# kwai/blaze

Measured on NVIDIA H100. Metric: rows/sec on TPC-DS q1 hash-agg+filter at 1/2/4/8 H100; HBM GB/s vs 3.35 TB/s, higher is better.
Workload: dtype int64

## Files before the change

blaze_b200/csrc/agg_device.cuh:

```cuda
#pragma once
#include <cuda_runtime.h>
#include <stdint.h>

#include "kernels.cuh"

namespace b200q {

constexpr unsigned TAG_EMPTY = 0, TAG_LOCKED = 1;
constexpr unsigned FLAG_SLOT_LOCK = 1u << 15;

__device__ __forceinline__ unsigned long long ld_relaxed_u64(const unsigned long long* p) {
  unsigned long long v; asm volatile("ld.relaxed.gpu.global.u64 %0, [%1];" : "=l"(v) : "l"(p) : "memory"); return v;
}
__device__ __forceinline__ ulonglong2 ld_relaxed_v2u64(const unsigned long long* p) {
  ulonglong2 v; asm volatile("ld.relaxed.gpu.global.v2.u64 {%0,%1}, [%2];" : "=l"(v.x), "=l"(v.y) : "l"(p) : "memory"); return v;
}
__device__ __forceinline__ void st_release_u32(unsigned* p, unsigned v) { asm volatile("st.release.gpu.global.u32 [%0], %1;" ::"l"(p), "r"(v) : "memory"); }
__device__ __forceinline__ void st_relaxed_u64(unsigned long long* p, unsigned long long v) { asm volatile("st.relaxed.gpu.global.u64 [%0], %1;" ::"l"(p), "l"(v) : "memory"); }
__device__ __forceinline__ void red_add_u64(unsigned long long* p, unsigned long long v) { asm volatile("red.global.add.u64 [%0], %1;" ::"l"(p), "l"(v) : "memory"); }
__device__ __forceinline__ void red_add_f64(unsigned long long* p, double v) { asm volatile("red.global.add.f64 [%0], %1;" ::"l"(p), "d"(v) : "memory"); }
__device__ __forceinline__ void red_min_s64(unsigned long long* p, long long v) { asm volatile("red.global.min.s64 [%0], %1;" ::"l"(p), "l"(v) : "memory"); }
__device__ __forceinline__ void red_max_s64(unsigned long long* p, long long v) { asm volatile("red.global.max.s64 [%0], %1;" ::"l"(p), "l"(v) : "memory"); }
constexpr uint64_t AGG_HASH_SEED = 0x9E3779B97F4A7C15ULL;
__device__ __forceinline__ uint64_t mix64(uint64_t x) { x ^= x >> 33; x *= 0xff51afd7ed558ccdULL; x ^= x >> 33; x *= 0xc4ceb9fe1a85ec53ULL; x ^= x >> 33; return x; }
__device__ __forceinline__ unsigned lanemask_lt() { unsigned m; asm("mov.u32 %0, %%lanemask_lt;" : "=r"(m)); return m; }

__device__ __forceinline__ uint64_t agg_hash2(uint64_t k0, uint64_t k1, uint32_t knull) {
  return mix64((AGG_HASH_SEED ^ k0) + k1 * 0xD6E8FEB86659FD93ULL + (uint64_t)knull * 0xA0761D6478BD642FULL);
}
__device__ __forceinline__ uint64_t agg_hash_words(const uint64_t* kw, int nkw, uint32_t knull) {
  if (nkw <= 2) return agg_hash2(nkw > 0 ? kw[0] : 0, nkw > 1 ? kw[1] : 0, knull);
  uint64_t x = AGG_HASH_SEED ^ kw[0];
  for (int i = 1; i < nkw; i++) x = x * 0xD6E8FEB86659FD93ULL + kw[i];
  return mix64(x + (uint64_t)knull * 0xA0761D6478BD642FULL);
}

__device__ __forceinline__ void slot_mark(unsigned long long* key_entry, unsigned flags_seen, int vbit) {
  if (vbit != 0xFF && !((flags_seen >> vbit) & 1)) atomicOr((unsigned*)key_entry + 1, 1u << vbit);
}

__device__ __forceinline__ uint64_t agg_first_slot(uint64_t h, uint64_t capacity) { return __umulhi((unsigned)(h >> 32), (unsigned)capacity); }
__device__ __forceinline__ unsigned agg_tag(uint64_t h) { return (unsigned)h | 0x80000000u; }
__device__ __forceinline__ uint64_t agg_next_slot(uint64_t s, uint64_t capacity) { return s + 1 == capacity ? 0 : s + 1; }
constexpr uint64_t AGG_NO_SLOT = ~0ULL;

__device__ __forceinline__ uint64_t agg_find_or_insert(const AggLayout& lay, const AggTable& tab, const uint64_t* kw, uint32_t knull,
                                                       uint64_t h, unsigned* flags_out, bool* inserted) {
  const unsigned tag = agg_tag(h);
  uint64_t s = agg_first_slot(h, tab.capacity);
  while (true) {
    unsigned long long* ke = tab.keys + s * (uint64_t)lay.kstride;
    const unsigned long long hdr = ld_relaxed_u64(ke);
    const unsigned t = (unsigned)hdr;
    unsigned flags = (unsigned)(hdr >> 32);
    if (t == tag) {
      asm volatile("fence.acq_rel.gpu;" ::: "memory");
      bool eq = (flags >> 16) == knull;
      for (int i = 0; eq && i < lay.nkw; i++) eq = ld_relaxed_u64(ke + 1 + i) == kw[i];
      if (eq) { *flags_out = flags; return s; }
    } else if (t == TAG_EMPTY) {
      if (ld_relaxed_u64(tab.counters) >= tab.max_groups) return AGG_NO_SLOT;
      if (atomicCAS((unsigned*)ke, TAG_EMPTY, TAG_LOCKED) == TAG_EMPTY) {
        for (int i = 0; i < lay.nkw; i++) ke[1 + i] = kw[i];
        unsigned long long* ae = tab.accs + s * (uint64_t)lay.astride;
        for (int i = 0; i < lay.astride; i++) ae[i] = lay.init[i];
        flags = lay.init_flags | (knull << 16);
        ((unsigned*)ke)[1] = flags;
        st_release_u32((unsigned*)ke, tag);
        *inserted = true;
        *flags_out = flags;
        return s;
      }
      continue;
    } else if (t == TAG_LOCKED) {
      continue;
    }
    s = agg_next_slot(s, tab.capacity);
  }
}

}
```

blaze_b200/csrc/capi.cu:

```cuda
#include <algorithm>
#include <cstdio>
#include <cstdlib>
#include <cstring>
#include <functional>
#include <mutex>

#include "lz4_frame.h"
#include "parquet_meta.h"
#include "runtime.h"

namespace b200q {

static thread_local std::string g_last_error;

static std::string format_of(const DType& t) {
  switch (t.id) {
    case T_BOOL: return "b"; case T_INT8: return "c"; case T_INT16: return "s"; case T_INT32: return "i"; case T_INT64: return "l";
    case T_FLOAT32: return "f"; case T_FLOAT64: return "g"; case T_DATE32: return "tdD"; case T_TIMESTAMP_US: return "tsu:";
    case T_DECIMAL128: return "d:" + std::to_string(t.precision) + "," + std::to_string(t.scale);
    case T_BINARY: return "z"; case T_UTF8: return "u"; default: return "n";
  }
}
DType type_of_format(const char* f) {
  DType d; std::string s(f ? f : "");
// ... 455 lines not shown
      hc.values = d2h((const uint8_t*)dc.values->ptr + first, (size_t)(ho[n] - first));
      if (first) for (int64_t i = 0; i <= n; i++) ho[i] -= first;
    } else if (dc.type.id == T_BOOL) hc.values = d2h(dc.values->ptr, (size_t)(n + 7) / 8);
    else if (dc.type.id != T_NULL) hc.values = d2h(dc.values->ptr, (size_t)n * dc.type.byte_width());
    hb.cols.push_back(hc);
  }
  B200Q_CUDA(cudaStreamSynchronize(cx.stream));
  return hb;
}

struct ArrayPriv {
  std::shared_ptr<HostBlock> block;
  std::vector<DevMemP> dev;
  std::vector<const void*> buffers;
  std::vector<ArrowArray> children; std::vector<ArrowArray*> child_ptrs;
};
static void release_array(ArrowArray* a) {
  if (!a || !a->release) return;
  auto* p = (ArrayPriv*)a->private_data;
  for (auto& c : p->children) if (c.release) c.release(&c);
  delete p; a->release = nullptr;
}
static int64_t count_nulls(const uint8_t* bits, int64_t off, int64_t n) {
  int64_t set = 0;
  for (int64_t i = 0; i < n; i++) set += (bits[(off + i) >> 3] >> ((off + i) & 7)) & 1;
  return n - set;
}
static void export_host_slice(const HostBatch& hb, int64_t off, int64_t len, ArrowArray* out) {
  auto* top = new ArrayPriv(); top->block = hb.block;
  memset(out, 0, sizeof(*out));
  out->length = len; out->null_count = 0; out->offset = 0; out->n_buffers = 1;
  top->buffers.push_back(nullptr); out->buffers = top->buffers.data();
  top->children.resize(hb.cols.size()); top->child_ptrs.resize(hb.cols.size());
  for (size_t i = 0; i < hb.cols.size(); i++) {
    const HostColumn& hc = hb.cols[i];
    auto* cp = new ArrayPriv(); cp->block = hb.block;
    ArrowArray& c = top->children[i]; memset(&c, 0, sizeof(c));
    c.length = len; c.offset = off;
    c.null_count = hc.validity ? count_nulls((const uint8_t*)hc.validity, off, len) : 0;
    if (hc.type.id == T_NULL) { c.null_count = len; c.n_buffers = 0; }
    else if (hc.type.is_varlen()) { cp->buffers = {hc.validity, hc.offsets, hc.values}; c.n_buffers = 3; }
    else { cp->buffers = {hc.validity, hc.values}; c.n_buffers = 2; }
    c.buffers = cp->buffers.data(); c.release = release_array; c.private_data = cp;
    top->child_ptrs[i] = &c;
  }
  out->n_children = (int64_t)hb.cols.size(); out->children = top->child_ptrs.data();
  out->release = release_array; out->private_data = top;
}
void export_device(DevBatch& db, int device, ArrowDeviceArray* out) {
  auto* top = new ArrayPriv();
  memset(out, 0, sizeof(*out));
  ArrowArray& a = out->array;
  a.length = db.num_rows; a.n_buffers = 1; top->buffers.push_back(nullptr); a.buffers = top->buffers.data();
  top->children.resize(db.cols.size()); top->child_ptrs.resize(db.cols.size());
  for (size_t i = 0; i < db.cols.size(); i++) {
    DevColumn& dc = db.cols[i];
    auto* cp = new ArrayPriv();
    ArrowArray& c = top->children[i]; memset(&c, 0, sizeof(c));
    c.length = db.num_rows; c.offset = dc.offset; c.null_count = dc.validity ? -1 : 0;
    const void* v = dc.validity ? dc.validity->ptr : nullptr;
    if (dc.validity) cp->dev.push_back(dc.validity);
    if (dc.values) cp->dev.push_back(dc.values);
    if (dc.offsets) cp->dev.push_back(dc.offsets);
    if (dc.type.id == T_NULL) { c.n_buffers = 0; c.null_count = db.num_rows; }
    else if (dc.type.is_varlen()) { cp->buffers = {v, dc.offsets->ptr, dc.values->ptr}; c.n_buffers = 3; }
    else { cp->buffers = {v, dc.values ? dc.values->ptr : nullptr}; c.n_buffers = 2; }
    c.buffers = cp->buffers.data(); c.release = release_array; c.private_data = cp;
    top->child_ptrs[i] = &c;
  }
  a.n_children = (int64_t)db.cols.size(); a.children = top->child_ptrs.data();
  a.release = release_array; a.private_data = top;
  out->device_id = device; out->device_type = ARROW_DEVICE_CUDA; out->sync_event = nullptr;
}

static void conf_defaults(b200q_conf* c) {
  memset(c, 0, sizeof(*c));
  c->struct_size = sizeof(b200q_conf);
  c->batch_size = 10000;
  c->suggested_batch_mem_size = 8388608;
  c->partial_agg_skipping_enable = 1;
  c->partial_agg_skipping_ratio = 0.999;
  c->partial_agg_skipping_min_rows = 20000;
  c->staging_rows = 1 << 20;
  c->agg_initial_groups = 1 << 19;
  c->max_launch_rows = 1 << 27;
  c->partial_state_columnar = 0;
  c->force_generic_kernels = 0;
  c->agg_dense_keys = 1;
  c->agg_hot_key_cache = 1;
}

}

#define B200Q_STR2(x) #x
#define B200Q_STR(x) B200Q_STR2(x)

extern "C" {

int32_t b200q_version(void) { return 100; }
const char* b200q_build_info(void) { return "blaze_b200 hot path: Filter/Project/HashAgg, sm_90a, CUDA " B200Q_STR(CUDART_VERSION); }
const char* b200q_last_error(void) { return g_last_error.c_str(); }
int32_t b200q_device_count(void) { int n = 0; if (cudaGetDeviceCount(&n) != cudaSuccess) { cudaGetLastError(); return 0; } return n; }

b200q_status b200q_conf_init(b200q_conf* conf) {
  if (!conf) return fail(B200Q_ERR_INVALID_ARG, "conf is null");
  conf_defaults(conf); return B200Q_OK;
}

b200q_status b200q_plan_explain(const uint8_t* plan, size_t plan_len, int32_t plan_kind, char* buf, size_t cap, size_t* needed) {
  return guarded(nullptr, [&] {
    PlanP p = decode_plan(plan, plan_len, plan_kind);
    std::string s = explain_plan(p);
    if (needed) *needed = s.size() + 1;
    if (buf && cap) { const size_t n = std::min(cap - 1, s.size()); memcpy(buf, s.data(), n); buf[n] = 0; }
  });
}

b200q_status b200q_op_create(const uint8_t* plan, size_t plan_len, int32_t plan_kind, const struct ArrowSchema* input_schema,
                             const b200q_conf* conf, int32_t device, b200q_op** out) {
  if (!out) return fail(B200Q_ERR_INVALID_ARG, "out is null");
  *out = nullptr;
  b200q_op* op = nullptr;
  b200q_status st = guarded(nullptr, [&] {
    PlanP p = decode_plan(plan, plan_len, plan_kind);
    int ndev = 0;
    if (cudaGetDeviceCount(&ndev) != cudaSuccess || ndev == 0) { cudaGetLastError(); throw ExecError(B200Q_ERR_NO_DEVICE, "no CUDA device is visible: the sm_90a kernels cannot run and there is no CPU fallback"); }
    if (device < 0 || device >= ndev) throw ExecError(B200Q_ERR_INVALID_ARG, "invalid device ordinal");
    op = new b200q_op();
    op->plan = p; op->cx.device = device;
    conf_defaults(&op->cx.conf);
    if (conf) { const size_t n = std::min<size_t>(conf->struct_size ? conf->struct_size : sizeof(b200q_conf), sizeof(b200q_conf)); memcpy(&op->cx.conf, conf, n); op->cx.conf.struct_size = sizeof(b200q_conf); }
    if (op->cx.conf.batch_size <= 0) op->cx.conf.batch_size = 10000;
    if (op->cx.conf.max_launch_rows <= 0) op->cx.conf.max_launch_rows = 1 << 27;
    if (op->cx.conf.agg_initial_groups <= 0) op->cx.conf.agg_initial_groups = 1 << 19;
    B200Q_CUDA(cudaSetDevice(device));
    {
      cudaMemPool_t pool; unsigned long long keep = ~0ULL;
      if (cudaDeviceGetDefaultMemPool(&pool, device) == cudaSuccess) cudaMemPoolSetAttribute(pool, cudaMemPoolAttrReleaseThreshold, &keep);
    }
    op->stream_ref = stream_ref_create(device);
    op->cx.stream = op->stream_ref->s;
    B200Q_CUDA(cudaEventCreate(&op->cx.ev0)); B200Q_CUDA(cudaEventCreate(&op->cx.ev1));
    build_pipeline(op);
    const PlanNode* leaf = op->plan.get();
    while (leaf->input) leaf = leaf->input.get();
    if (leaf->leaf_kind == "IpcReader") op->ipc = make_ipc_source(op->cx, op->in_schema, op->stages[0]->used_input_cols);
    if (input_schema) {
      if (input_schema->n_children != (int64_t)op->in_schema.fields.size()) throw PlanError(B200Q_ERR_INVALID_ARG, "input_schema does not match the plan leaf: column count");
      for (int64_t i = 0; i < input_schema->n_children; i++)
        if (type_of_format(input_schema->children[i]->format) != op->in_schema.fields[i].type)
          throw PlanError(B200Q_ERR_INVALID_ARG, "input_schema does not match the plan leaf: type of column " + std::to_string(i));
    }
  });
  if (st != B200Q_OK) { if (op) { op->stages.clear(); delete op; } return st; }
  *out = op;
  return B200Q_OK;
}

b200q_status b200q_op_input_schema(b200q_op* op, struct ArrowSchema* out) {
  if (!op || !out) return fail(B200Q_ERR_INVALID_ARG, "null argument");
  return guarded(nullptr, [&] { export_schema(op->in_schema, out); });
}
b200q_status b200q_op_output_schema(b200q_op* op, struct ArrowSchema* out) {
  if (!op || !out) return fail(B200Q_ERR_INVALID_ARG, "null argument");
  return guarded(nullptr, [&] { export_schema(op->out_schema, out); });
}

b200q_status b200q_op_push(b200q_op* op, struct ArrowArray* batch) {
  if (!op) return fail(B200Q_ERR_INVALID_ARG, "op is null");
  b200q_status st = guarded(op, [&] {
    if (op->finished) throw ExecError(B200Q_ERR_STATE, "push after finish");
    if (op->ipc) throw ExecError(B200Q_ERR_STATE, "an op whose leaf is an IpcReaderExecNode takes its input through b200q_op_push_ipc");
    B200Q_CUDA(cudaSetDevice(op->cx.device));
    validate_host_batch(op, batch);
    poll_pending(op, false);
    op->cx.m.input_rows += batch->length; op->cx.m.input_batches++;
    if (batch->length == 0) return;
    const std::vector<int>& used = op->stages[0]->used_input_cols;
    const int64_t srows = op->cx.conf.staging_rows;
    if (srows > 0 && batch->length < srows / 2) { staging_append(op, batch); return; }
    if (op->staging_ready) staging_flush(op);
    DevBatch db = import_direct(op, batch, used);
    PendingRelease pr; pr.arr = *batch; batch->release = nullptr;
    B200Q_CUDA(cudaEventCreateWithFlags(&pr.ev, cudaEventDisableTiming));
    B200Q_CUDA(cudaEventRecord(pr.ev, op->cx.stream));
    op->pending.push_back(pr);
    run_stages(op, db, 0);
  });
  if (batch && batch->release) batch->release(batch);
  return st;
}

b200q_status b200q_op_push_ipc(b200q_op* op, const uint8_t* data, size_t len) {
  if (!op) return fail(B200Q_ERR_INVALID_ARG, "op is null");
  return guarded(op, [&] {
    if (op->finished) throw ExecError(B200Q_ERR_STATE, "push after finish");
    if (!op->ipc) throw ExecError(B200Q_ERR_STATE, "push_ipc: the op's leaf is not an IpcReaderExecNode");
    if (!data && len) throw ExecError(B200Q_ERR_INVALID_ARG, "push_ipc: null data");
    B200Q_CUDA(cudaSetDevice(op->cx.device));
    poll_pending(op, false);
    op->ipc->push(op->cx, data, len, [&](DevBatch& b) { run_stages(op, b, 0); });
  });
}

b200q_status b200q_op_push_device(b200q_op* op, struct ArrowDeviceArray* dbatch) {
  if (!op) return fail(B200Q_ERR_INVALID_ARG, "op is null");
  b200q_status st = guarded(op, [&] {
    if (op->finished) throw ExecError(B200Q_ERR_STATE, "push after finish");
    if (op->ipc) throw ExecError(B200Q_ERR_STATE, "an op whose leaf is an IpcReaderExecNode takes its input through b200q_op_push_ipc");
    if (!dbatch) throw ExecError(B200Q_ERR_INVALID_ARG, "null batch");
    if (dbatch->device_type != ARROW_DEVICE_CUDA || dbatch->device_id != op->cx.device) throw ExecError(B200Q_ERR_INVALID_ARG, "push_device: batch is not on this op's CUDA device");
    B200Q_CUDA(cudaSetDevice(op->cx.device));
    ArrowArray* batch = &dbatch->array;
    validate_host_batch(op, batch);
    poll_pending(op, false);
    if (op->staging_ready) staging_flush(op);
    if (dbatch->sync_event) B200Q_CUDA(cudaStreamWaitEvent(op->cx.stream, *(cudaEvent_t*)dbatch->sync_event, 0));
    op->cx.m.input_rows += batch->length; op->cx.m.input_batches++;
    if (batch->length == 0) return;
    DevBatch db; db.num_rows = batch->length; db.cols.resize(op->in_schema.fields.size());
    for (size_t i = 0; i < db.cols.size(); i++) {
      const ArrowArray* c = batch->children[i]; DevColumn& dc = db.cols[i];
      dc.type = op->in_schema.fields[i].type; dc.offset = c->offset + batch->offset;
      const size_t huge = (size_t)1 << 60;
      if (c->n_buffers > 0 && c->buffers[0] && c->null_count != 0) dc.validity = DevMem::borrow(c->buffers[0], huge, nullptr);
      if (dc.type.is_varlen()) { dc.offsets = DevMem::borrow(c->buffers[1], huge, nullptr); dc.values = DevMem::borrow(c->buffers[2], huge, nullptr); }
      else if (c->n_buffers > 1 && c->buffers[1]) dc.values = DevMem::borrow(c->buffers[1], huge, nullptr);
    }
    PendingRelease pr; pr.arr = *batch;
    B200Q_CUDA(cudaEventCreateWithFlags(&pr.ev, cudaEventDisableTiming));
    batch->release = nullptr;
    op->pending.push_back(pr);
    const cudaEvent_t ev = pr.ev;
    try { run_stages(op, db, 0); } catch (...) { cudaEventRecord(ev, op->cx.stream); throw; }
    B200Q_CUDA(cudaEventRecord(ev, op->cx.stream));
  });
  if (dbatch && dbatch->array.release) dbatch->array.release(&dbatch->array);
  return st;
}

b200q_status b200q_op_finish(b200q_op* op) {
  if (!op) return fail(B200Q_ERR_INVALID_ARG, "op is null");
  return guarded(op, [&] {
    if (op->finished) return;
    B200Q_CUDA(cudaSetDevice(op->cx.device));
    {
      const PlanNode* leaf = op->plan.get();
      while (leaf->input) leaf = leaf->input.get();
      if (leaf->kind == N_LEAF && leaf->leaf_kind == "ParquetScan") {
        if (op->cx.m.input_batches) throw ExecError(B200Q_ERR_STATE, "an op whose leaf is a ParquetScanExecNode takes no pushed batches");
        run_parquet_scan(op->cx, *leaf, [&](DevBatch& b) { run_stages(op, b, 0); });
      }
    }
    if (op->ipc) op->ipc->flush(op->cx, [&](DevBatch& b) { run_stages(op, b, 0); });
    if (op->staging_ready) staging_flush(op);
    for (size_t i = 0; i < op->stages.size(); i++) {
      std::vector<DevBatch> outs;
      op->cx.cur_stage = (int)i;
      op->stages[i]->finish(op->cx, outs);
      for (auto& o : outs) {
        if (i + 1 < op->stages.size()) run_stages(op, o, i + 1);
        else { op->cx.m.output_rows += o.num_rows; op->out_queue.push_back(std::move(o)); }
      }
    }
    B200Q_CUDA(cudaStreamSynchronize(op->cx.stream));
    poll_pending(op, true);
    op->finished = true;
  });
}

b200q_status b200q_op_pull(b200q_op* op, struct ArrowArray* out, int32_t* has_batch) {
  if (!op || !out || !has_batch) return fail(B200Q_ERR_INVALID_ARG, "null argument");
  *has_batch = 0;
  return guarded(op, [&] {
    B200Q_CUDA(cudaSetDevice(op->cx.device));
    if (!op->has_cur_host) {
      if (op->out_queue.empty()) return;
      op->cur_host = to_host(op, op->out_queue.front());
      op->out_queue.pop_front();
      op->has_cur_host = true;
    }
    HostBatch& hb = op->cur_host;
    const int64_t len = std::min<int64_t>(op->cx.conf.batch_size, hb.num_rows - hb.cursor);
    export_host_slice(hb, hb.cursor, len, out);
    hb.cursor += len;
    if (hb.cursor >= hb.num_rows) { op->has_cur_host = false; op->cur_host = HostBatch(); }
    op->cx.m.output_batches++;
    *has_batch = 1;
  });
}

b200q_status b200q_op_pull_device(b200q_op* op, struct ArrowDeviceArray* out, int32_t* has_batch) {
  if (!op || !out || !has_batch) return fail(B200Q_ERR_INVALID_ARG, "null argument");
  *has_batch = 0;
  return guarded(op, [&] {
    if (op->has_cur_host) throw ExecError(B200Q_ERR_STATE, "pull_device while a host batch is partially pulled");
    if (op->out_queue.empty()) return;
    B200Q_CUDA(cudaSetDevice(op->cx.device));
    B200Q_CUDA(cudaStreamSynchronize(op->cx.stream));
    export_device(op->out_queue.front(), op->cx.device, out);
    op->out_queue.pop_front();
    op->cx.m.output_batches++;
    *has_batch = 1;
  });
}

b200q_status b200q_op_sync(b200q_op* op) {
// ... 143 lines not shown
```

blaze_b200/csrc/kernels_fast.cu:

```cuda
#include <algorithm>
#include <cstdlib>
#include <cuda_runtime.h>
#include <stdint.h>

#include "agg_device.cuh"
#include "kernels_fast.cuh"

namespace b200q {

constexpr int FA_BLOCK = 256;

__device__ __forceinline__ uint64_t make_evict_first_policy() {
  uint64_t pol; asm volatile("createpolicy.fractional.L2::evict_first.b64 %0, 1.0;" : "=l"(pol)); return pol;
}
__device__ __forceinline__ long long ld_stream_s64(const long long* p) {
  long long v; const uint64_t pol = make_evict_first_policy();
  asm volatile("ld.global.nc.L1::no_allocate.L2::cache_hint.s64 %0, [%1], %2;" : "=l"(v) : "l"(p), "l"(pol)); return v;
}
__device__ __forceinline__ bool col_valid(const DevCol& c, long long i) {
  if (!c.validity) return true;
  const unsigned long long bi = (unsigned long long)i + c.bit_offset;
  return (__ldg(c.validity + (bi >> 3)) >> (bi & 7)) & 1;
}
__device__ __forceinline__ long long col_load_int(const DevCol& c, int phys, long long i) {
// ... 191 lines not shown
#pragma unroll
    for (int u = 0; u < U; u++) {
      unsigned long long di;
      const bool in = dense_index<NK>(fs, k0[u], k1[u], di) && alive[u] && !(meta[u] & 3u);
      const unsigned pk = in ? ((unsigned)di | ((meta[u] & 0xCu) << 26)) : 0xFFFFFFFFu;
#pragma unroll
      for (int t = 0; t < G; t++) {
        const unsigned opk = __shfl_sync(0xffffffffu, pk, t, G);
        const unsigned long long ov0 = add0 ? __shfl_sync(0xffffffffu, v0[u], t, G) : 0ULL;
        const unsigned long long ov1 = add1 ? __shfl_sync(0xffffffffu, v1[u], t, G) : 0ULL;
        const bool live = opk != 0xFFFFFFFFu;
        unsigned long long val;
        switch (wkind) {
          case DW_ONE: val = 1; break;
          case DW_ADD0: val = ov0; break;
          case DW_ADD1: val = ov1; break;
          case DW_VALID0: val = (opk >> 28) & 1u; break;
          case DW_VALID1: val = (opk >> 29) & 1u; break;
          default: val = 0; break;
        }
        red_add_u64(live ? fs.dense_tab + (uint64_t)(opk & IDX_MASK) * G + q : sink, live ? val : 0ULL);
      }
      const bool fb = alive[u] && !in;
      if (__any_sync(0xffffffffu, fb)) {
        bool inserted = false;
        if (fb) {
          uint64_t kw[2] = {(uint64_t)k0[u], NK == 2 ? (uint64_t)k1[u] : 0ULL};
          const unsigned knull = meta[u] & 3u;
          unsigned fl = 0;
          const uint64_t si = agg_find_or_insert(lay, tab, kw, knull, agg_hash2(kw[0], kw[1], knull), &fl, &inserted);
          if (si == AGG_NO_SLOT) { const unsigned long long at = atomicAdd(tab.counters + 1, 1ULL); tab.deferred[at] = (uint32_t)((unit0 + u) * 32 + lane); }
          else {
            unsigned long long* const p = tab.accs + si * (uint64_t)lay.astride;
            unsigned long long* const ke = tab.keys + si * (uint64_t)lay.kstride;
            if (meta[u] & 4u) { red_add_u64(p + fs.acc[0].word, add0 ? v0[u] : 1ULL); slot_mark(ke, fl, fs.acc[0].vbit); }
            if (NACC == 2 && (meta[u] & 8u)) { red_add_u64(p + fs.acc[1].word, add1 ? v1[u] : 1ULL); slot_mark(ke, fl, fs.acc[1].vbit); }
          }
        }
        const unsigned bl = __ballot_sync(0xffffffffu, inserted);
        if (lane == 0 && bl) atomicAdd(tab.counters, (unsigned long long)__popc(bl));
      }
    }
  }
}

constexpr int HC_LINES = 1024;
template <int NACC, int NK, int G>
__global__ void __launch_bounds__(FA_BLOCK) agg_dense_hot_kernel(const ColTable cols, const FastSpec fs, const AggLayout lay, const AggTable tab,
                                                                 long long row_begin, long long n) {
  constexpr int U = 4;
  constexpr unsigned IDX_MASK = 0x0FFFFFFFu;
  __shared__ unsigned long long c_key[HC_LINES];
  __shared__ unsigned c_acc[HC_LINES * G * 2];
  for (int i = threadIdx.x; i < HC_LINES; i += FA_BLOCK) c_key[i] = 0;
  for (int i = threadIdx.x; i < HC_LINES * G * 2; i += FA_BLOCK) c_acc[i] = 0;
  __syncthreads();
  const unsigned lane = threadIdx.x & 31, q = lane & (G - 1);
  const long long gwarp = (long long)blockIdx.x * (FA_BLOCK / 32) + (threadIdx.x >> 5), nwarps = (long long)gridDim.x * (FA_BLOCK / 32);
  const long long nunits = (n + 31) / 32;
  const bool add0 = fs.acc[0].kind == FAST_ACC_ADD, add1 = NACC == 2 && fs.acc[1].kind == FAST_ACC_ADD;
  auto word_kind = [&](int m) {
    const int src = fs.dense_word_src[m];
    return src == -1 ? DW_ONE : src == -2 ? DW_ZERO : src >= 2 ? DW_ONE : src == 0 ? (add0 ? DW_ADD0 : DW_ONE) : (add1 ? DW_ADD1 : DW_ONE);
  };
  int wk[G];
#pragma unroll
  for (int m = 0; m < G; m++) wk[m] = word_kind(m);
  const int wkind = word_kind((int)q);
  unsigned long long* const sink = warp_sink(fs, gwarp, lane);

  for (long long unit0 = gwarp * U; unit0 < nunits; unit0 += nwarps * U) {
    long long k0[U], k1[U]; unsigned long long v0[U], v1[U]; bool alive[U];
#pragma unroll
    for (int u = 0; u < U; u++) {
      const long long rel = (unit0 + u) * 32 + lane, row = row_begin + rel;
      alive[u] = rel < n; k0[u] = 0; k1[u] = 0; v0[u] = 0; v1[u] = 0;
      if (!alive[u]) continue;
      k0[u] = ld_stream_vec((const long long*)cols.col[fs.key_col[0]].values + row, (i64xG<1>*)nullptr).v[0];
      if (NK == 2) k1[u] = ld_stream_vec((const long long*)cols.col[fs.key_col[1]].values + row, (i64xG<1>*)nullptr).v[0];
      if (add0) v0[u] = (unsigned long long)ld_stream_vec((const long long*)cols.col[fs.acc[0].col].values + row, (i64xG<1>*)nullptr).v[0];
      if (add1) v1[u] = (unsigned long long)ld_stream_vec((const long long*)cols.col[fs.acc[1].col].values + row, (i64xG<1>*)nullptr).v[0];
    }
    for (int f = 0; f < fs.nfilt; f++) {
      const long long* fcol = (const long long*)cols.col[fs.filt[f].col].values + row_begin;
#pragma unroll
      for (int u = 0; u < U; u++) {
        const long long rel = (unit0 + u) * 32 + lane;
        if (alive[u]) alive[u] = cmp_apply(fs.filt[f].op, ld_stream_vec(fcol + rel, (i64xG<1>*)nullptr).v[0], fs.filt[f].lit);
      }
    }
#pragma unroll
    for (int u = 0; u < U; u++) {
      unsigned long long di;
      const bool in = dense_index<NK>(fs, k0[u], k1[u], di) && alive[u];
      bool cached = false;
      if (in) {
        const unsigned line = (unsigned)((di * 0x9E3779B97F4A7C15ULL) >> 54);
        const unsigned long long mine = di + 1;
        unsigned long long cur = *(volatile unsigned long long*)&c_key[line];
        if (cur == 0) { cur = atomicCAS(&c_key[line], 0ULL, mine); if (cur == 0) cur = mine; }
        if (cur == mine) {
          cached = true;
          unsigned* const e = c_acc + line * (G * 2);
#pragma unroll
          for (int m = 0; m < G; m++) {
            if (wk[m] == DW_ONE) smem_add64(e + 2 * m, 1ULL);
            else if (wk[m] == DW_ADD0) smem_add64(e + 2 * m, v0[u]);
            else if (wk[m] == DW_ADD1) smem_add64(e + 2 * m, v1[u]);
          }
        }
      }
      const unsigned pk = (in && !cached) ? (unsigned)di : 0xFFFFFFFFu;
#pragma unroll
      for (int t = 0; t < G; t++) {
        const unsigned opk = __shfl_sync(0xffffffffu, pk, t, G);
        const unsigned long long ov0 = add0 ? __shfl_sync(0xffffffffu, v0[u], t, G) : 0ULL;
        const unsigned long long ov1 = add1 ? __shfl_sync(0xffffffffu, v1[u], t, G) : 0ULL;
        const bool live = opk != 0xFFFFFFFFu;
        const unsigned long long val = wkind == DW_ONE ? 1ULL : wkind == DW_ADD0 ? ov0 : wkind == DW_ADD1 ? ov1 : 0ULL;
        red_add_u64(live ? fs.dense_tab + (uint64_t)(opk & IDX_MASK) * G + q : sink, live ? val : 0ULL);
      }
      const bool fb = alive[u] && !in;
      if (__any_sync(0xffffffffu, fb)) {
        bool inserted = false;
        if (fb) {
          uint64_t kw[2] = {(uint64_t)k0[u], NK == 2 ? (uint64_t)k1[u] : 0ULL};
          unsigned fl = 0;
          const uint64_t si = agg_find_or_insert(lay, tab, kw, 0, agg_hash2(kw[0], kw[1], 0), &fl, &inserted);
          if (si == AGG_NO_SLOT) { const unsigned long long at = atomicAdd(tab.counters + 1, 1ULL); tab.deferred[at] = (uint32_t)((unit0 + u) * 32 + lane); }
          else {
            unsigned long long* const p = tab.accs + si * (uint64_t)lay.astride;
            unsigned long long* const ke = tab.keys + si * (uint64_t)lay.kstride;
            red_add_u64(p + fs.acc[0].word, add0 ? v0[u] : 1ULL); slot_mark(ke, fl, fs.acc[0].vbit);
            if (NACC == 2) { red_add_u64(p + fs.acc[1].word, add1 ? v1[u] : 1ULL); slot_mark(ke, fl, fs.acc[1].vbit); }
          }
        }
        const unsigned bl = __ballot_sync(0xffffffffu, inserted);
        if (lane == 0 && bl) atomicAdd(tab.counters, (unsigned long long)__popc(bl));
      }
    }
  }
  __syncthreads();
  for (int line = threadIdx.x; line < HC_LINES; line += FA_BLOCK) {
    const unsigned long long key = c_key[line];
    if (!key) continue;
#pragma unroll
    for (int m = 0; m < G; m++) {
      const unsigned long long val = (unsigned long long)c_acc[(line * G + m) * 2] | ((unsigned long long)c_acc[(line * G + m) * 2 + 1] << 32);
      if (val) red_add_u64(fs.dense_tab + (key - 1) * G + m, val);
    }
  }
}

__global__ void __launch_bounds__(256) key_skew_hist_kernel(const DevCol c0, const DevCol c1, int phys0, int phys1, int nkeys, long long n, unsigned* hist) {
  for (long long i = blockIdx.x * (long long)blockDim.x + threadIdx.x; i < n; i += (long long)gridDim.x * blockDim.x) {
    if (!col_valid(c0, i) || (nkeys == 2 && !col_valid(c1, i))) continue;
    const uint64_t h = agg_hash2((uint64_t)col_load_int(c0, phys0, i), nkeys == 2 ? (uint64_t)col_load_int(c1, phys1, i) : 0ULL, 0);
    atomicAdd(hist + (h >> 48), 1u);
  }
}
__global__ void __launch_bounds__(256) key_skew_max_kernel(unsigned* hist) {
  unsigned mx = 0;
  for (int i = blockIdx.x * blockDim.x + threadIdx.x; i < 65536; i += gridDim.x * blockDim.x) mx = max(mx, hist[i]);
#pragma unroll
  for (int d = 16; d > 0; d >>= 1) mx = max(mx, __shfl_xor_sync(0xffffffffu, mx, d));
  if ((threadIdx.x & 31) == 0) atomicMax(hist + 65536, mx);
}

constexpr int LH_BLOCK = 128, LH_U = 4, LH_QCAP = 32 * (LH_U + 1);
template <int NK, bool TYPED> struct LhQueue {
  unsigned long long k0[LH_QCAP]; unsigned long long k1[NK == 2 ? LH_QCAP : 1]; unsigned long long v0[LH_QCAP], v1[LH_QCAP];
  unsigned idx[LH_QCAP], tag[LH_QCAP], row[LH_QCAP];
  uint8_t meta[TYPED ? LH_QCAP : 1];
};
enum { LH_HIT = 0, LH_AGAIN = 1, LH_NEW = 2, LH_IDLE = 3 };
constexpr unsigned LH_META_PLAIN = 0xC;

template <int NK>
__device__ __forceinline__ int lh_eval(const AggTable& tab, int ks, unsigned cap, ulonglong2 hk, unsigned tag, unsigned knull, unsigned long long k0,
                                       unsigned long long k1, unsigned& idx, unsigned& flags) {
  const unsigned t = (unsigned)hk.x;
  if (t == tag) {
    bool hit = (unsigned)(hk.x >> 48) == knull && hk.y == k0;
    if (NK == 2 && hit) hit = ld_relaxed_u64(tab.keys + (uint64_t)idx * ks + 2) == k1;
    if (hit) { flags = (unsigned)(hk.x >> 32); return LH_HIT; }
  } else if (t == TAG_EMPTY) return LH_NEW;
  else if (t == TAG_LOCKED) return LH_AGAIN;
  idx = idx + 1 == cap ? 0 : idx + 1;
  return LH_AGAIN;
}

template <int NK, int NACC, bool TYPED>
__device__ __forceinline__ void lh_finish(const FastSpec& fs, const AggLayout& lay, const AggTable& tab, LhQueue<NK, TYPED>& q, int& count, unsigned lane,
                                          unsigned long long* sink, bool has_v1, int st, unsigned idx, unsigned flags, unsigned tag, unsigned meta,
                                          unsigned long long k0, unsigned long long k1, unsigned long long v0, unsigned long long v1, unsigned row) {
  constexpr unsigned NONE = 0xFFFFFFFFu;
  if (__any_sync(0xffffffffu, st == LH_NEW)) {
    bool inserted = false;
    if (st == LH_NEW) {
      uint64_t kw[2] = {k0, NK == 2 ? k1 : 0ULL};
      const unsigned knull = TYPED ? (meta & 3u) : 0u;
      const uint64_t si = agg_find_or_insert(lay, tab, kw, knull, agg_hash2(k0, NK == 2 ? k1 : 0ULL, knull), &flags, &inserted);
      if (si == AGG_NO_SLOT) { const unsigned long long at = atomicAdd(tab.counters + 1, 1ULL); tab.deferred[at] = row; st = LH_IDLE; }
      else { idx = (unsigned)si; st = LH_HIT; }
    }
    const unsigned b = __ballot_sync(0xffffffffu, inserted);
    if (lane == 0 && b) atomicAdd(tab.counters, (unsigned long long)__popc(b));
  }
  const bool odd = lane & 1;
  const int as = lay.astride, w0 = fs.acc[0].word, w1 = NACC == 2 ? fs.acc[1].word : 0;
  const unsigned mi = st == LH_HIT ? idx : NONE;
  unsigned long long* const mine = mi != NONE ? tab.accs + (uint64_t)mi * as + w0 : sink;
  const unsigned long long mv = mi != NONE ? v0 : 0ULL;
  if (NACC == 1) red_add_u64(mine, mv);
  else {
    const unsigned pi = __shfl_xor_sync(0xffffffffu, mi, 1);
    const unsigned long long pv1 = has_v1 ? __shfl_xor_sync(0xffffffffu, v1, 1) : 1ULL;
    unsigned long long* const theirs = pi != NONE ? tab.accs + (uint64_t)pi * as + w1 : sink;
    const unsigned long long tv = pi != NONE ? pv1 : 0ULL;
    red_add_u64(odd ? theirs : mine, odd ? tv : mv);
    red_add_u64(odd ? mine : theirs, odd ? mv : tv);
  }
  if (mi != NONE) {
    unsigned long long* ke = tab.keys + (uint64_t)mi * lay.kstride;
    if (!TYPED || (meta & 4u)) slot_mark(ke, flags, fs.acc[0].vbit);
    if (NACC == 2 && (!TYPED || (meta & 8u))) slot_mark(ke, flags, fs.acc[1].vbit);
  }
  const unsigned m = __ballot_sync(0xffffffffu, st == LH_AGAIN);
  if (m) {
    if (st == LH_AGAIN) {
      const int at = count + __popc(m & ((1u << lane) - 1));
      q.k0[at] = k0; if (NK == 2) q.k1[at] = k1; q.v0[at] = v0; q.v1[at] = v1; q.idx[at] = idx; q.tag[at] = tag; q.row[at] = row;
      if (TYPED) q.meta[at] = (uint8_t)meta;
    }
    count += __popc(m);
  }
}

template <int NK, int NACC, bool TYPED>
__device__ __forceinline__ void lh_drain(const FastSpec& fs, const AggLayout& lay, const AggTable& tab, LhQueue<NK, TYPED>& q, int& count, unsigned lane,
                                         unsigned long long* sink, bool has_v1) {
  const int nb = count < 32 ? count : 32;
  __syncwarp();
  count -= nb;
  const bool act = (int)lane < nb; const int e = count + (act ? lane : 0);
  const unsigned long long k0 = q.k0[e], k1 = NK == 2 ? q.k1[e] : 0ULL, v0 = q.v0[e], v1 = q.v1[e];
  unsigned idx = q.idx[e], flags = 0; const unsigned tag = q.tag[e], row = q.row[e], meta = TYPED ? q.meta[e] : LH_META_PLAIN;
  __syncwarp();
  int st = LH_IDLE;
  if (act) st = lh_eval<NK>(tab, lay.kstride, (unsigned)tab.capacity, ld_relaxed_v2u64(tab.keys + (uint64_t)idx * lay.kstride), tag, TYPED ? (meta & 3u) : 0u, k0, k1, idx, flags);
  lh_finish<NK, NACC, TYPED>(fs, lay, tab, q, count, lane, sink, has_v1, st, idx, flags, tag, meta, k0, k1, v0, v1, row);
}

template <int NK, int NACC, bool TYPED>
__global__ void __launch_bounds__(LH_BLOCK, TYPED ? 4 : 6) agg_lean_hash_kernel(const ColTable cols, const FastSpec fs, const AggLayout lay, const AggTable tab,
                                                                                long long row_begin, long long n) {
  constexpr int U = LH_U;
  __shared__ LhQueue<NK, TYPED> queues[LH_BLOCK / 32];
  LhQueue<NK, TYPED>& q = queues[threadIdx.x >> 5];
  int count = 0;
  const unsigned lane = threadIdx.x & 31;
  const long long gwarp = (long long)blockIdx.x * (LH_BLOCK / 32) + (threadIdx.x >> 5), nwarps = (long long)gridDim.x * (LH_BLOCK / 32);
  const long long nunits = (n + 31) / 32;
  const bool add0 = fs.acc[0].kind == FAST_ACC_ADD, add1 = NACC == 2 && fs.acc[1].kind == FAST_ACC_ADD;
  const long long* kcol0 = (const long long*)cols.col[fs.key_col[0]].values + row_begin;
  const long long* kcol1 = NK == 2 ? (const long long*)cols.col[fs.key_col[1]].values + row_begin : nullptr;
  const long long* vcol0 = add0 ? (const long long*)cols.col[fs.acc[0].col].values + row_begin : nullptr;
  const long long* vcol1 = add1 ? (const long long*)cols.col[fs.acc[1].col].values + row_begin : nullptr;
  unsigned long long* const sink = warp_sink(fs, gwarp, lane);
  const unsigned cap = (unsigned)tab.capacity; const int ks = lay.kstride;

  for (long long unit0 = gwarp * U; unit0 < nunits; unit0 += nwarps * U) {
    unsigned long long k0[U], k1[U], v0[U], v1[U]; bool alive[U]; unsigned meta[U];
#pragma unroll
    for (int u = 0; u < U; u++) {
      const long long rel = (unit0 + u) * 32 + lane;
      alive[u] = rel < n; meta[u] = LH_META_PLAIN;
      if (!TYPED) {
        k0[u] = alive[u] ? (unsigned long long)ld_stream_vec(kcol0 + rel, (i64xG<1>*)nullptr).v[0] : 0;
        k1[u] = (NK == 2 && alive[u]) ? (unsigned long long)ld_stream_vec(kcol1 + rel, (i64xG<1>*)nullptr).v[0] : 0;
        v0[u] = (vcol0 && alive[u]) ? (unsigned long long)ld_stream_vec(vcol0 + rel, (i64xG<1>*)nullptr).v[0] : 1ULL;
        v1[u] = (vcol1 && alive[u]) ? (unsigned long long)ld_stream_vec(vcol1 + rel, (i64xG<1>*)nullptr).v[0] : 1ULL;
      } else {
        k0[u] = 0; k1[u] = 0; v0[u] = 1; v1[u] = 1;
        if (alive[u]) {
          const long long row = row_begin + rel;
          { const DevCol& c = cols.col[fs.key_col[0]]; if (col_valid(c, row)) k0[u] = (unsigned long long)col_load_int(c, fs.key_phys[0], row); else meta[u] |= 1u; }
          if (NK == 2) { const DevCol& c = cols.col[fs.key_col[1]]; if (col_valid(c, row)) k1[u] = (unsigned long long)col_load_int(c, fs.key_phys[1], row); else meta[u] |= 2u; }
          if (fs.acc[0].col >= 0) {
            const DevCol& c = cols.col[fs.acc[0].col];
            if (!col_valid(c, row)) { meta[u] &= ~4u; v0[u] = 0; } else if (add0) v0[u] = (unsigned long long)col_load_int(c, fs.acc[0].phys, row);
          }
          if (NACC == 2 && fs.acc[1].col >= 0) {
            const DevCol& c = cols.col[fs.acc[1].col];
            if (!col_valid(c, row)) { meta[u] &= ~8u; v1[u] = 0; } else if (add1) v1[u] = (unsigned long long)col_load_int(c, fs.acc[1].phys, row);
          }
        }
      }
    }
    for (int f = 0; f < fs.nfilt; f++) {
      if (!TYPED) {
        const long long* fcol = (const long long*)cols.col[fs.filt[f].col].values + row_begin;
#pragma unroll
        for (int u = 0; u < U; u++) {
          const long long rel = (unit0 + u) * 32 + lane;
          const long long x = rel < n ? ld_stream_vec(fcol + rel, (i64xG<1>*)nullptr).v[0] : 0;
          alive[u] = alive[u] && cmp_apply(fs.filt[f].op, x, fs.filt[f].lit);
        }
      } else {
        const DevCol& c = cols.col[fs.filt[f].col];
#pragma unroll
        for (int u = 0; u < U; u++) {
          const long long row = row_begin + (unit0 + u) * 32 + lane;
          if (alive[u]) alive[u] = col_valid(c, row) && cmp_apply(fs.filt[f].op, col_load_int(c, fs.filt[f].phys, row), fs.filt[f].lit);
        }
      }
    }
    unsigned idx[U], tag[U]; ulonglong2 hk[U];
#pragma unroll
// ... 25 lines not shown
  for (unsigned i = threadIdx.x; i < 2 * nwords; i += FA_BLOCK) s_tab[i] = 0;
  __syncthreads();
  const unsigned lane = threadIdx.x & 31;
  const long long gwarp = (long long)blockIdx.x * (FA_BLOCK / 32) + (threadIdx.x >> 5), nwarps = (long long)gridDim.x * (FA_BLOCK / 32);
  const long long nunits = (n + 31) / 32;
  const bool add0 = fs.acc[0].kind == FAST_ACC_ADD, add1 = NACC == 2 && fs.acc[1].kind == FAST_ACC_ADD;

  for (long long unit0 = gwarp * U; unit0 < nunits; unit0 += nwarps * U) {
    long long k[U], k1[U]; unsigned long long v0[U], v1[U]; bool alive[U]; unsigned meta[U];
#pragma unroll
    for (int u = 0; u < U; u++) {
      const long long rel = (unit0 + u) * 32 + lane, row = row_begin + rel;
      alive[u] = rel < n; meta[u] = 0xC; k[u] = 0; k1[u] = 0; v0[u] = 1; v1[u] = 1;
      if (!alive[u]) continue;
      if (!TYPED) {
        k[u] = ld_stream_vec((const long long*)cols.col[fs.key_col[0]].values + row, (i64xG<1>*)nullptr).v[0];
        if (NK == 2) k1[u] = ld_stream_vec((const long long*)cols.col[fs.key_col[1]].values + row, (i64xG<1>*)nullptr).v[0];
        if (add0) v0[u] = (unsigned long long)ld_stream_vec((const long long*)cols.col[fs.acc[0].col].values + row, (i64xG<1>*)nullptr).v[0];
        if (add1) v1[u] = (unsigned long long)ld_stream_vec((const long long*)cols.col[fs.acc[1].col].values + row, (i64xG<1>*)nullptr).v[0];
      } else {
        { const DevCol& c = cols.col[fs.key_col[0]]; if (col_valid(c, row)) k[u] = col_load_int(c, fs.key_phys[0], row); else meta[u] |= 1u; }
        if (NK == 2) { const DevCol& c = cols.col[fs.key_col[1]]; if (col_valid(c, row)) k1[u] = col_load_int(c, fs.key_phys[1], row); else meta[u] |= 2u; }
        if (fs.acc[0].col >= 0) {
          const DevCol& c = cols.col[fs.acc[0].col];
          if (!col_valid(c, row)) { meta[u] &= ~4u; v0[u] = 0; } else if (add0) v0[u] = (unsigned long long)col_load_int(c, fs.acc[0].phys, row);
        }
        if (NACC == 2 && fs.acc[1].col >= 0) {
          const DevCol& c = cols.col[fs.acc[1].col];
          if (!col_valid(c, row)) { meta[u] &= ~8u; v1[u] = 0; } else if (add1) v1[u] = (unsigned long long)col_load_int(c, fs.acc[1].phys, row);
        }
      }
    }
    for (int f = 0; f < fs.nfilt; f++) {
      const DevCol& c = cols.col[fs.filt[f].col];
#pragma unroll
      for (int u = 0; u < U; u++) {
        const long long row = row_begin + (unit0 + u) * 32 + lane;
        if (!alive[u]) continue;
        if (!TYPED) alive[u] = cmp_apply(fs.filt[f].op, ld_stream_vec((const long long*)c.values + row, (i64xG<1>*)nullptr).v[0], fs.filt[f].lit);
        else alive[u] = col_valid(c, row) && cmp_apply(fs.filt[f].op, col_load_int(c, fs.filt[f].phys, row), fs.filt[f].lit);
      }
    }
#pragma unroll
    for (int u = 0; u < U; u++) {
      unsigned long long idx;
      const bool in = dense_index<NK>(fs, k[u], k1[u], idx) && alive[u] && !(meta[u] & 3u);
      if (in) {
        unsigned* const e = s_tab + 2 * (unsigned)idx * G;
#pragma unroll
        for (int m = 0; m < 4; m++) {
          if (m >= G) break;
          const int src = fs.dense_word_src[m];
          if (src == -1) smem_add64(e + 2 * m, 1ULL);
          else if (src == 0) { if (meta[u] & 4u) smem_add64(e + 2 * m, v0[u]); }
          else if (src == 1 && NACC == 2) { if (meta[u] & 8u) smem_add64(e + 2 * m, v1[u]); }
          else if (src >= 2) { if (meta[u] & (4u << (src - 2))) smem_add64(e + 2 * m, 1ULL); }
        }
      }
      const bool fb = alive[u] && !in;
      if (__any_sync(0xffffffffu, fb)) {
        bool inserted = false;
        if (fb) {
          uint64_t kw[2] = {(uint64_t)k[u], NK == 2 ? (uint64_t)k1[u] : 0ULL};
          const unsigned knull = meta[u] & 3u;
          unsigned fl = 0;
          const uint64_t si = agg_find_or_insert(lay, tab, kw, knull, agg_hash2(kw[0], kw[1], knull), &fl, &inserted);
          if (si == AGG_NO_SLOT) { const unsigned long long at = atomicAdd(tab.counters + 1, 1ULL); tab.deferred[at] = (uint32_t)((unit0 + u) * 32 + lane); }
          else {
            unsigned long long* const p = tab.accs + si * (uint64_t)lay.astride;
            unsigned long long* const ke = tab.keys + si * (uint64_t)lay.kstride;
            if (meta[u] & 4u) { red_add_u64(p + fs.acc[0].word, v0[u]); slot_mark(ke, fl, fs.acc[0].vbit); }
            if (NACC == 2 && (meta[u] & 8u)) { red_add_u64(p + fs.acc[1].word, v1[u]); slot_mark(ke, fl, fs.acc[1].vbit); }
          }
        }
        const unsigned b = __ballot_sync(0xffffffffu, inserted);
        if (lane == 0 && b) atomicAdd(tab.counters, (unsigned long long)__popc(b));
      }
    }
  }
  __syncthreads();
  for (unsigned w = threadIdx.x; w < nwords; w += FA_BLOCK) {
    const unsigned long long val = (unsigned long long)s_tab[2 * w] | ((unsigned long long)s_tab[2 * w + 1] << 32);
    if (val) red_add_u64(fs.dense_tab + w, val);
  }
}

static int fast_grid(int64_t ntiles) {
  int dev = 0, sms = 132; cudaGetDevice(&dev); cudaDeviceGetAttribute(&sms, cudaDevAttrMultiProcessorCount, dev);
  const int64_t cap = (int64_t)sms * 8;
  return (int)(ntiles < cap ? (ntiles < 1 ? 1 : ntiles) : cap);
}

int launch_agg_fast_update(const ColTable& cols, const FastSpec& fs, const AggLayout& lay, const AggTable& tab, int64_t row_begin, int64_t n, cudaStream_t s) {
  if (n <= 0) return 0;
  const int dg = fs.dense ? fs.dense_stride : 0;
  if (dg && fs.dense_cap * (unsigned long long)dg <= (unsigned long long)DS_MAX_WORDS) {
    const int g = (int)std::max<int64_t>(1, std::min<int64_t>((n + FA_BLOCK * 4 - 1) / (FA_BLOCK * 4), (int64_t)fast_grid(1 << 30) / 8 * 3));
#define B200Q_DS(NACC, TYPED, NK) agg_dense_smem_kernel<NACC, TYPED, NK><<<g, FA_BLOCK, 0, s>>>(cols, fs, lay, tab, row_begin, n)
    if (fs.nkeys == 1) {
      if (fs.lean) { if (fs.nacc == 2) B200Q_DS(2, false, 1); else B200Q_DS(1, false, 1); } else { if (fs.nacc == 2) B200Q_DS(2, true, 1); else B200Q_DS(1, true, 1); }
    } else {
      if (fs.lean) { if (fs.nacc == 2) B200Q_DS(2, false, 2); else B200Q_DS(1, false, 2); } else { if (fs.nacc == 2) B200Q_DS(2, true, 2); else B200Q_DS(1, true, 2); }
    }
#undef B200Q_DS
    return 1;
  }
  if (dg && fs.lean && fs.hot_cache) {
    const int g = fast_grid((n + 32 * 8 * 4 - 1) / (32 * 8 * 4));
#define B200Q_HC(NACC, NK, G) agg_dense_hot_kernel<NACC, NK, G><<<g, FA_BLOCK, 0, s>>>(cols, fs, lay, tab, row_begin, n)
    if (fs.nkeys == 1) {
      if (fs.nacc == 2) { if (dg == 2) B200Q_HC(2, 1, 2); else B200Q_HC(2, 1, 4); } else { if (dg == 2) B200Q_HC(1, 1, 2); else B200Q_HC(1, 1, 4); }
    } else {
      if (fs.nacc == 2) { if (dg == 2) B200Q_HC(2, 2, 2); else B200Q_HC(2, 2, 4); } else { if (dg == 2) B200Q_HC(1, 2, 2); else B200Q_HC(1, 2, 4); }
    }
#undef B200Q_HC
    return 1;
  }
  if (dg && fs.lean && fs.nkeys == 1 && fs.nfilt == 0) {
    const int u = dg == 2 ? 4 : 2;
    const int g = fast_grid((n + 32 * 8 * u - 1) / (32 * 8 * u));
#define B200Q_LD(NACC, G) agg_lean_dense_kernel<NACC, G, 1><<<g, FA_BLOCK, 0, s>>>(cols, fs, lay, tab, row_begin, n)
    if (fs.nacc == 2) { if (dg == 2) B200Q_LD(2, 2); else B200Q_LD(2, 4); } else { if (dg == 2) B200Q_LD(1, 2); else B200Q_LD(1, 4); }
#undef B200Q_LD
    return 1;
  }
  if (dg && fs.nfcol >= 0) {
    if (fs.filt_never) return 0;
    return launch_agg_tile_dense(cols, fs, lay, tab, row_begin, n, s);
  }
  if (dg) {
    const int g = fast_grid((n + 32 * 8 * 4 - 1) / (32 * 8 * 4));
#define B200Q_DR(NACC, NK, G) do { if (fs.lean) agg_dense_row_kernel<NACC, NK, G, false><<<g, FA_BLOCK, 0, s>>>(cols, fs, lay, tab, row_begin, n); \
                                   else agg_dense_row_kernel<NACC, NK, G, true><<<g, FA_BLOCK, 0, s>>>(cols, fs, lay, tab, row_begin, n); } while (0)
    if (fs.nkeys == 1) {
      if (fs.nacc == 2) { if (dg == 2) B200Q_DR(2, 1, 2); else B200Q_DR(2, 1, 4); } else { if (dg == 2) B200Q_DR(1, 1, 2); else B200Q_DR(1, 1, 4); }
    } else {
      if (fs.nacc == 2) { if (dg == 2) B200Q_DR(2, 2, 2); else B200Q_DR(2, 2, 4); } else { if (dg == 2) B200Q_DR(1, 2, 2); else B200Q_DR(1, 2, 4); }
    }
#undef B200Q_DR
    return 1;
  }
  if (!dg) {
    const int64_t tiles = (n + 32 * (LH_BLOCK / 32) * LH_U - 1) / (32 * (LH_BLOCK / 32) * LH_U);
    const int g = (int)std::max<int64_t>(1, std::min<int64_t>(tiles, (int64_t)fast_grid(1 << 30) / 8 * (fs.lean ? 6 : 4)));
#define B200Q_LH(NK, NACC, TYPED) agg_lean_hash_kernel<NK, NACC, TYPED><<<g, LH_BLOCK, 0, s>>>(cols, fs, lay, tab, row_begin, n)
    if (fs.lean) { if (fs.nkeys == 1) { if (fs.nacc == 2) B200Q_LH(1, 2, false); else B200Q_LH(1, 1, false); } else { if (fs.nacc == 2) B200Q_LH(2, 2, false); else B200Q_LH(2, 1, false); } }
    else { if (fs.nkeys == 1) { if (fs.nacc == 2) B200Q_LH(1, 2, true); else B200Q_LH(1, 1, true); } else { if (fs.nacc == 2) B200Q_LH(2, 2, true); else B200Q_LH(2, 1, true); } }
#undef B200Q_LH
    return 1;
  }
  return 0;
}

__global__ void __launch_bounds__(256) key_range_kernel(const DevCol col, int phys, long long n, long long* out ) {
  long long mn = INT64_MAX, mx = INT64_MIN; unsigned long long cnt = 0;
  for (long long i = blockIdx.x * (long long)blockDim.x + threadIdx.x; i < n; i += (long long)gridDim.x * blockDim.x) {
    if (!col_valid(col, i)) continue;
    const long long v = col_load_int(col, phys, i);
    mn = v < mn ? v : mn; mx = v > mx ? v : mx; cnt++;
  }
#pragma unroll
  for (int d = 16; d > 0; d >>= 1) {
    const long long a = __shfl_xor_sync(0xffffffffu, mn, d), b = __shfl_xor_sync(0xffffffffu, mx, d);
    mn = a < mn ? a : mn; mx = b > mx ? b : mx; cnt += __shfl_xor_sync(0xffffffffu, cnt, d);
  }
  if ((threadIdx.x & 31) == 0) { atomicMin(out, mn); atomicMax(out + 1, mx); atomicAdd((unsigned long long*)out + 2, cnt); }
}
int launch_key_skew_probe(const DevCol* key_cols, const uint8_t* phys, int nkeys, int64_t n, unsigned* d_hist, cudaStream_t s) {
  key_skew_hist_kernel<<<fast_grid((n + 2047) / 2048), 256, 0, s>>>(key_cols[0], key_cols[nkeys == 2 ? 1 : 0], phys[0], phys[nkeys == 2 ? 1 : 0], nkeys, n, d_hist);
  key_skew_max_kernel<<<32, 256, 0, s>>>(d_hist);
  return 2;
}
int launch_key_range(const DevCol& col, int phys, int64_t n, long long* d_out, cudaStream_t s) {
  key_range_kernel<<<fast_grid((n + 2047) / 2048), 256, 0, s>>>(col, phys, n, d_out);
  return 1;
}

__device__ __forceinline__ void dense_store(const EmitCol& c, unsigned long long at, uint64_t lo, bool valid) {
  if (c.valid_bytes) c.valid_bytes[at] = valid ? 1 : 0;
  switch (c.phys) {
    case PH_BOOL: ((uint8_t*)c.values)[at] = lo != 0; break;
    case PH_I8: ((int8_t*)c.values)[at] = (int8_t)lo; break;
    case PH_I16: ((int16_t*)c.values)[at] = (int16_t)lo; break;
    case PH_I32: ((int32_t*)c.values)[at] = (int32_t)lo; break;
    default: ((uint64_t*)c.values)[at] = lo; break;
  }
}
__global__ void __launch_bounds__(256) agg_emit_dense_kernel(const FastSpec fs, const EmitTable emit, const DenseEmitMap map, unsigned long long* out_count) {
  const unsigned lane = threadIdx.x & 31;
  const uint64_t stride = (uint64_t)gridDim.x * blockDim.x;
  const uint64_t rounds = (fs.dense_cap + stride - 1) / stride;
  for (uint64_t it = 0; it < rounds; it++) {
    const uint64_t i = it * stride + blockIdx.x * (uint64_t)blockDim.x + threadIdx.x;
    const uint64_t pe = fs.nkeys == 2 && fs.dense_key0_minor ? dense_entry2(fs, i / fs.dense_r1, i % fs.dense_r1) : i;
    const unsigned long long* e = fs.dense_tab + pe * fs.dense_stride;
    const bool occ = i < fs.dense_cap && e[fs.dense_presence_word] != 0;
    const unsigned m = __ballot_sync(0xffffffffu, occ);
    if (!m) continue;
    unsigned long long base = 0;
    if (lane == 0) base = atomicAdd(out_count, (unsigned long long)__popc(m));
    base = __shfl_sync(0xffffffffu, base, 0);
    if (!occ) continue;
    const unsigned long long at = base + __popc(m & lanemask_lt());
    for (int c = 0; c < emit.ncols; c++) {
      const EmitCol ec = emit.col[c];
      if (ec.kind == EMIT_KEY) {
        const long long kv = fs.nkeys == 1 ? fs.dense_base + (long long)i
                           : ec.key == 0 ? fs.dense_base + (long long)(i / fs.dense_r1) : fs.dense_base1 + (long long)(i % fs.dense_r1);
        dense_store(ec, at, (uint64_t)kv, true);
      }
      else {
        const int w = map.word[c], vw = map.valid_word[c];
        const bool valid = vw == 0xFF ? true : e[vw] != 0;
        dense_store(ec, at, valid ? e[w] : 0, valid);
      }
    }
  }
}
int launch_agg_emit_dense(const FastSpec& fs, const EmitTable& emit, const DenseEmitMap& map, unsigned long long* d_out_count, cudaStream_t s) {
  agg_emit_dense_kernel<<<fast_grid(((int64_t)fs.dense_cap + 255) / 256), 256, 0, s>>>(fs, emit, map, d_out_count);
  return 1;
}

__global__ void __launch_bounds__(256) dense_count_kernel(const FastSpec fs, unsigned long long* out) {
  unsigned long long c = 0;
  for (uint64_t i = blockIdx.x * (uint64_t)blockDim.x + threadIdx.x; i < fs.dense_cap; i += (uint64_t)gridDim.x * blockDim.x)
    c += fs.dense_tab[i * fs.dense_stride + fs.dense_presence_word] != 0;
#pragma unroll
  for (int d = 16; d > 0; d >>= 1) c += __shfl_xor_sync(0xffffffffu, c, d);
  if ((threadIdx.x & 31) == 0 && c) atomicAdd(out, c);
}
int launch_dense_count(const FastSpec& fs, unsigned long long* d_out, cudaStream_t s) {
  dense_count_kernel<<<fast_grid(((int64_t)fs.dense_cap + 255) / 256), 256, 0, s>>>(fs, d_out);
  return 1;
}

}
```

blaze_b200/csrc/kernels_fast.cuh:

```cuda
#pragma once
#include <cstddef>

#include "kernels.cuh"

namespace b200q {

enum FastAccKind : uint8_t { FAST_ACC_ADD = 0, FAST_ACC_COUNT = 1 };

struct FilterInterval { int8_t col; uint8_t phys; uint8_t _pad[6]; long long lo; unsigned long long span; };

struct FastSpec {
  int32_t nkeys, nacc, nfilt, dense;
  int32_t lean, hot_cache;
  int8_t key_col[2]; uint8_t key_phys[2];
  struct { uint8_t kind; int8_t col; uint8_t phys; uint8_t vbit; uint8_t word; uint8_t _pad[3]; } acc[2];
  struct { int8_t col; uint8_t phys; uint8_t op; uint8_t _pad[5]; long long lit; } filt[4];
  int32_t nfcol;
  int32_t filt_never;
  FilterInterval frange[2];
  long long dense_base;
  unsigned long long dense_cap;
  long long dense_base1;
  unsigned long long dense_r1, dense_cap0;
  unsigned long long* dense_tab;
  int8_t dense_stride;
  int8_t dense_word_src[4];
  uint8_t dense_presence_word;
  uint8_t dense_key0_minor;
  uint8_t _pad1;
  unsigned long long* sink;
};
constexpr int FAST_SINK_WARPS = 4096;

struct DenseEmitMap { uint8_t word[EMIT_MAX_COLS]; uint8_t valid_word[EMIT_MAX_COLS]; };

__device__ __forceinline__ unsigned long long dense_entry2(const FastSpec& fs, unsigned long long d0, unsigned long long d1) {
  return fs.dense_key0_minor ? d1 * fs.dense_cap0 + d0 : d0 * fs.dense_r1 + d1;
}
template <int NK>
__device__ __forceinline__ bool dense_index_of(const FastSpec& fs, long long k0, long long k1, unsigned long long& idx) {
  const unsigned long long d0 = (unsigned long long)(k0 - fs.dense_base);
  if (NK == 1) { idx = d0; return d0 < fs.dense_cap; }
  const unsigned long long d1 = (unsigned long long)(k1 - fs.dense_base1);
  idx = dense_entry2(fs, d0, d1);
  return d0 < fs.dense_cap0 && d1 < fs.dense_r1;
}

enum TileFlavour : uint8_t { TF_ADD_U64 = 0, TF_ADD_F64 = 1, TF_MIN_S64 = 2 };
__host__ __device__ constexpr unsigned long long tile_identity(int flavour) {
  return flavour == TF_MIN_S64 ? 0x7FFFFFFFFFFFFFFFULL : flavour == TF_ADD_F64 ? 0x8000000000000000ULL : 0ULL;
}
enum TileArgCvt : uint8_t { TC_NONE = 0, TC_I2F = 1 , TC_ORDER = 2  };
enum TileRecon : uint8_t { TR_COPY = 0 , TR_NOT = 1 ,
                           TR_F2I = 2 , TR_DEC3 = 3  };
struct TileWord {
  uint8_t srcsel;
  uint8_t sh;
  uint8_t gate;
  uint8_t _pad[5];
  unsigned long long msk, inv, cst;
};
struct TileAggSpec {
  int32_t nkeys, nargs, nfcol, filt_never, nacc, G, flavour, arg_is_dec;
  int8_t key_col[2]; uint8_t key_phys[2];
  int8_t arg_col[2]; uint8_t arg_phys[2]; uint8_t arg_cvt[2]; uint8_t arg_values[2];
  FilterInterval frange[2];
  long long dense_base, dense_base1;
  unsigned long long dense_cap, dense_r1, dense_cap0;
  unsigned long long* dense_tab;
  unsigned long long* sink;
  unsigned long long dec_mul;
  TileWord word[8];
  uint8_t presence_word, dec_word , _pad2[6];
  struct { int8_t arg; uint8_t recon; uint8_t w0; uint8_t valid_word; uint8_t lay_acc; uint8_t _pad[3]; } acc[4];
};
static_assert(sizeof(FastSpec) == 232 && offsetof(FastSpec, frange) == 120, "FastSpec layout");
static_assert(sizeof(TileAggSpec) == 456 && offsetof(TileAggSpec, frange) == 48, "TileAggSpec layout");

int launch_agg_tile_wide(const ColTable& cols, const TileAggSpec& ts, const AggLayout& lay, const AggTable& tab, int64_t row_begin, int64_t n, cudaStream_t s);
int launch_tile_wide_init(const TileAggSpec& ts, cudaStream_t s);
int launch_tile_wide_count(const TileAggSpec& ts, unsigned long long* d_out, cudaStream_t s);
int launch_tile_wide_normalise(const TileAggSpec& ts, cudaStream_t s);
int launch_tile_wide_emit(const TileAggSpec& ts, const AggLayout& lay, const EmitTable& emit, unsigned long long* d_out_count, cudaStream_t s);

int launch_agg_tile_dense(const ColTable& cols, const FastSpec& fs, const AggLayout& lay, const AggTable& tab, int64_t row_begin, int64_t n, cudaStream_t s);
int launch_agg_fast_update(const ColTable& cols, const FastSpec& fs, const AggLayout& lay, const AggTable& tab, int64_t row_begin, int64_t n, cudaStream_t s);
int launch_key_skew_probe(const DevCol* key_cols, const uint8_t* phys, int nkeys, int64_t n, unsigned* d_hist , cudaStream_t s);
int launch_key_range(const DevCol& col, int phys, int64_t n, long long* d_out, cudaStream_t s);
int launch_agg_emit_dense(const FastSpec& fs, const EmitTable& emit, const DenseEmitMap& map, unsigned long long* d_out_count, cudaStream_t s);
int launch_dense_count(const FastSpec& fs, unsigned long long* d_out, cudaStream_t s);

}
```

blaze_b200/csrc/kernels_tile.cu:

```cuda
#include <cuda_runtime.h>
#include <stdint.h>

#include <algorithm>

#include "agg_device.cuh"
#include "emit_device.cuh"
#include "kernels_fast.cuh"

namespace b200q {

constexpr int TL_BLOCK = 256, TL_WARPS = TL_BLOCK / 32, TL_ROWS = 128;

__device__ __forceinline__ uint64_t tl_policy_evict_first() {
  uint64_t pol; asm volatile("createpolicy.fractional.L2::evict_first.b64 %0, 1.0;" : "=l"(pol)); return pol;
}
__device__ __forceinline__ void tl_ld_b64(const long long* p, unsigned on, uint64_t pol, long long& v) {
  asm volatile("{\n\t.reg .pred q;\n\tsetp.ne.u32 q, %2, 0;\n\t@q ld.global.nc.L1::no_allocate.L2::cache_hint.b64 %0, [%1], %3;\n\t}"
               : "+l"(v) : "l"(p), "r"(on), "l"(pol));
}
__device__ __forceinline__ void tl_ld_v2b64(const long long* p, unsigned on, uint64_t pol, long long& a, long long& b) {
  asm volatile("{\n\t.reg .pred q;\n\tsetp.ne.u32 q, %3, 0;\n\t@q ld.global.nc.L1::no_allocate.L2::cache_hint.v2.b64 {%0,%1}, [%2], %4;\n\t}"
               : "+l"(a), "+l"(b) : "l"(p), "r"(on), "l"(pol));
}
__device__ __forceinline__ void tl_ld_b32(const int* p, unsigned on, uint64_t pol, int& v) {
// ... 227 lines not shown
  const bool a16 = ((uintptr_t)c.values & 15) == 0;
#pragma unroll
  for (int j = 0; j < 4; j++) {
    lo[j] = 0; hi[j] = 0;
    if (a16) tl_ld_v2b64(p + 64 * j, (ld >> j) & 1u, pol, lo[j], hi[j]);
    else { tl_ld_b64(p + 64 * j, (ld >> j) & 1u, pol, lo[j]); tl_ld_b64(p + 64 * j + 1, (ld >> j) & 1u, pol, hi[j]); }
  }
}

__device__ __forceinline__ unsigned long long tw_convert(long long v, int cvt) {
  if (cvt == TC_I2F) return f64_bits(__ll2double_rn(v));
  if (cvt == TC_ORDER) return (unsigned long long)total_order_key((uint64_t)v);
  return (unsigned long long)v;
}

__device__ __forceinline__ void tw_slot_update(const AggLayout& lay, const TileAggSpec& ts, unsigned long long* ke, unsigned long long* ae, unsigned flags,
                                               unsigned long long x0, unsigned long long x1, bool valid0, bool valid1) {
  for (int a = 0; a < ts.nacc; a++) {
    const AccOp op = lay.acc[ts.acc[a].lay_acc];
    const int arg = ts.acc[a].arg;
    const bool valid = arg < 0 ? true : (arg == 0 ? valid0 : valid1);
    if (!valid) continue;
    const unsigned long long x = arg == 1 ? x1 : x0;
    unsigned long long* w = ae + op.word;
    switch (op.kind) {
      case ACC_ADD_I64: red_add_u64(w, x); break;
      case ACC_ADD_F64: red_add_f64(w, as_f64(x)); break;
      case ACC_ADD_DEC: { const unsigned long long old = atomicAdd(w, x0); red_add_u64(w + 1, x1 + ((old + x0) < old ? 1ULL : 0ULL)); break; }
      case ACC_COUNT: red_add_u64(w, 1ULL); break;
      case ACC_MIN_I64: case ACC_MIN_F64: red_min_s64(w, (long long)x); break;
      default: red_max_s64(w, (long long)x); break;
    }
    slot_mark(ke, flags, op.vbit);
  }
}

template <int NK, int NF, int G, int FLAV>
__global__ void __launch_bounds__(TL_BLOCK, TW_MIN_CTAS(NK, NF)) agg_tile_wide_kernel(const ColTable cols, const TileAggSpec ts, const AggLayout lay, const AggTable tab, long long row_begin, long long n) {
  constexpr unsigned IDX_MASK = 0x0FFFFFFFu, ALWAYS = 1u << 30, FULL = 0xffffffffu;
  __shared__ TileQueue queues[TL_WARPS];
  TileQueue& q = queues[threadIdx.x >> 5];
  const unsigned lane = threadIdx.x & 31, qw = lane & (G - 1);
  const long long gwarp = (long long)blockIdx.x * TL_WARPS + (threadIdx.x >> 5), nwarps = (long long)gridDim.x * TL_WARPS;
  const long long ntiles = (n + TL_ROWS - 1) / TL_ROWS;
  const TileWord tw = ts.word[qw];
  const bool use1 = tw.srcsel == 1, use_c = tw.srcsel == 2;
  const unsigned long long noop = tw_noop<FLAV>();
  unsigned long long* const sink = ts.sink + ((gwarp & (FAST_SINK_WARPS - 1)) << 2) + (lane & 3);
  const uint64_t pol = tl_policy_evict_first();
  const bool dec = ts.arg_is_dec != 0;

  long long f[NF > 0 ? NF : 1][4]; unsigned fv[NF > 0 ? NF : 1];
  tl_load_filters<NF>(cols, ts.frange, row_begin, gwarp * TL_ROWS + lane, n, pol, f, fv);
  for (long long tile = gwarp; tile < ntiles; tile += nwarps) {
    const long long rel0 = tile * TL_ROWS + lane, row0 = row_begin + rel0;
    const unsigned alive = tl_pass<NF>(ts.frange, f, fv, tl_rows_in(rel0, n));
    long long k0[4], k1[4], a0[4], a1[4]; unsigned kv0, kv1 = 0xF, av0 = 0xF, av1 = 0xF;
    tl_column<NF>(cols, ts.frange, f, fv, ts.key_col[0], ts.key_phys[0], row0, alive, true, pol, k0, kv0);
    if (NK == 2) tl_column<NF>(cols, ts.frange, f, fv, ts.key_col[1], ts.key_phys[1], row0, alive, true, pol, k1, kv1);
    else { k1[0] = k1[1] = k1[2] = k1[3] = 0; }
    a0[0] = a0[1] = a0[2] = a0[3] = 0; a1[0] = a1[1] = a1[2] = a1[3] = 0;
    if (dec) {
      tl_load_dec(cols.col[ts.arg_col[0]], row0, alive, pol, a0, a1, av0); av1 = av0;
      if (ts.dec_mul != 1) {
#pragma unroll
        for (int j = 0; j < 4; j++) { const i128_t v = mk128((uint64_t)a0[j], (uint64_t)a1[j]) * (i128_t)ts.dec_mul; a0[j] = (long long)lo64(v); a1[j] = (long long)hi64(v); }
      }
    }
    else {
      if (ts.nargs > 0) tl_column<NF>(cols, ts.frange, f, fv, ts.arg_col[0], ts.arg_phys[0], row0, alive, ts.arg_values[0] != 0, pol, a0, av0);
      if (ts.nargs > 1) tl_column<NF>(cols, ts.frange, f, fv, ts.arg_col[1], ts.arg_phys[1], row0, alive, ts.arg_values[1] != 0, pol, a1, av1);
    }
    tl_load_filters<NF>(cols, ts.frange, row_begin, rel0 + nwarps * TL_ROWS, n, pol, f, fv);
    const unsigned knull = (~kv0 | (NK == 2 ? ~kv1 : 0u)) & 0xFu;
    int total = 0; unsigned fb = 0;
#pragma unroll
    for (int j = 0; j < 4; j++) {
      const unsigned long long d0 = (unsigned long long)(k0[j] - ts.dense_base), d1 = (unsigned long long)(k1[j] - ts.dense_base1);
      const unsigned long long di = NK == 1 ? d0 : d0 * ts.dense_r1 + d1;
      const bool inr = NK == 1 ? d0 < ts.dense_cap : (d0 < ts.dense_cap0 && d1 < ts.dense_r1);
      const bool live = (alive >> j) & 1u;
      const bool in = inr && live && !((knull >> j) & 1u);
      fb |= (unsigned)(live && !in) << j;
      const unsigned m = __ballot_sync(FULL, in);
      if (in) {
        const int at = total + __popc(m & lanemask_lt());
        q.idx[at] = (unsigned)di | (((av0 >> j) & 1u) << 28) | (((av1 >> j) & 1u) << 29) | ALWAYS;
        q.v0[at] = dec ? (unsigned long long)a0[j] : tw_convert(a0[j], ts.arg_cvt[0]);
        q.v1[at] = dec ? (unsigned long long)a1[j] : tw_convert(a1[j], ts.arg_cvt[1]);
      }
      total += __popc(m);
    }
    __syncwarp();
    for (int e0 = 0; e0 < total; e0 += 32 / G) {
      const int e = e0 + (int)(lane / G);
      const bool live = e < total;
      const int er = live ? e : 0;
      const unsigned pk = q.idx[er];
      const unsigned long long x = use1 ? q.v1[er] : q.v0[er];
      unsigned long long val = use_c ? tw.cst : (((x >> tw.sh) & tw.msk) ^ tw.inv);
      const bool on = live && ((pk >> tw.gate) & 1u);
      val = on ? val : noop;
      tw_red<FLAV>(live ? ts.dense_tab + (uint64_t)(pk & IDX_MASK) * G + qw : sink, val);
    }
    __syncwarp();
    if (__any_sync(FULL, fb != 0)) {
#pragma unroll
      for (int j = 0; j < 4; j++) {
        bool inserted = false;
        if ((fb >> j) & 1u) {
          const unsigned kn = ((~kv0 >> j) & 1u) | (NK == 2 ? (((~kv1 >> j) & 1u) << 1) : 0u);
          uint64_t kw[2] = {(kn & 1u) ? 0ULL : (uint64_t)k0[j], (NK == 2 && !(kn & 2u)) ? (uint64_t)k1[j] : 0ULL};
          unsigned fl = 0;
          const uint64_t si = agg_find_or_insert(lay, tab, kw, kn, agg_hash2(kw[0], kw[1], kn), &fl, &inserted);
          if (si == AGG_NO_SLOT) { const unsigned long long at = atomicAdd(tab.counters + 1, 1ULL); tab.deferred[at] = (uint32_t)(rel0 + 32 * j); }
          else tw_slot_update(lay, ts, tab.keys + si * (uint64_t)lay.kstride, tab.accs + si * (uint64_t)lay.astride, fl,
                              dec ? (unsigned long long)a0[j] : tw_convert(a0[j], ts.arg_cvt[0]), dec ? (unsigned long long)a1[j] : tw_convert(a1[j], ts.arg_cvt[1]),
                              (av0 >> j) & 1u, (av1 >> j) & 1u);
        }
        const unsigned bl = __ballot_sync(FULL, inserted);
        if (lane == 0 && bl) atomicAdd(tab.counters, (unsigned long long)__popc(bl));
      }
    }
  }
}

int launch_agg_tile_wide(const ColTable& cols, const TileAggSpec& ts, const AggLayout& lay, const AggTable& tab, int64_t row_begin, int64_t n, cudaStream_t s) {
  if (n <= 0 || ts.filt_never) return 0;
  const int64_t units = ((n + TL_ROWS - 1) / TL_ROWS + TL_WARPS - 1) / TL_WARPS;
#define B200Q_TW(NK, NF, G_, FL) do { auto k_ = agg_tile_wide_kernel<NK, NF, G_, FL>; k_<<<tile_grid(k_, units), TL_BLOCK, 0, s>>>(cols, ts, lay, tab, row_begin, n); } while (0)
#define B200Q_TW_FL(NK, NF, G_) do { if (ts.flavour == TF_ADD_U64) B200Q_TW(NK, NF, G_, TF_ADD_U64); else if (ts.flavour == TF_ADD_F64) B200Q_TW(NK, NF, G_, TF_ADD_F64); else B200Q_TW(NK, NF, G_, TF_MIN_S64); } while (0)
#define B200Q_TW_G(NK, NF) do { if (ts.G == 2) B200Q_TW_FL(NK, NF, 2); else if (ts.G == 4) B200Q_TW_FL(NK, NF, 4); else B200Q_TW_FL(NK, NF, 8); } while (0)
#define B200Q_TW_NF(NK) do { if (ts.nfcol == 0) B200Q_TW_G(NK, 0); else if (ts.nfcol == 1) B200Q_TW_G(NK, 1); else B200Q_TW_G(NK, 2); } while (0)
  if (ts.nkeys == 1) B200Q_TW_NF(1); else B200Q_TW_NF(2);
#undef B200Q_TW_NF
#undef B200Q_TW_G
#undef B200Q_TW_FL
#undef B200Q_TW
  return 1;
}

__global__ void __launch_bounds__(256) tile_wide_fill_kernel(unsigned long long* tab, unsigned long long nwords, unsigned long long v) {
  for (unsigned long long i = blockIdx.x * (unsigned long long)blockDim.x + threadIdx.x; i < nwords; i += (unsigned long long)gridDim.x * blockDim.x) tab[i] = v;
}
int launch_tile_wide_init(const TileAggSpec& ts, cudaStream_t s) {
  const unsigned long long nwords = ts.dense_cap * (unsigned long long)ts.G;
  tile_wide_fill_kernel<<<tile_grid(tile_wide_fill_kernel, (int64_t)((nwords + 8191) / 8192)), 256, 0, s>>>(ts.dense_tab, nwords, tile_identity(ts.flavour));
  return 1;
}
__device__ __forceinline__ bool tw_marked(const TileAggSpec& ts, unsigned long long w) {
  return ts.flavour == TF_MIN_S64 ? w == 0 : ts.flavour == TF_ADD_F64 ? as_f64(w) != 0.0 : w != 0;
}
__device__ __forceinline__ bool tw_present(const TileAggSpec& ts, const unsigned long long* e) { return tw_marked(ts, e[ts.presence_word]); }
__global__ void __launch_bounds__(256) tile_wide_count_kernel(const TileAggSpec ts, unsigned long long* out) {
  unsigned long long c = 0;
  for (uint64_t i = blockIdx.x * (uint64_t)blockDim.x + threadIdx.x; i < ts.dense_cap; i += (uint64_t)gridDim.x * blockDim.x) c += tw_present(ts, ts.dense_tab + i * ts.G);
#pragma unroll
  for (int d = 16; d > 0; d >>= 1) c += __shfl_xor_sync(0xffffffffu, c, d);
  if ((threadIdx.x & 31) == 0 && c) atomicAdd(out, c);
}
int launch_tile_wide_count(const TileAggSpec& ts, unsigned long long* d_out, cudaStream_t s) {
  tile_wide_count_kernel<<<tile_grid(tile_wide_count_kernel, ((int64_t)ts.dense_cap + 16383) / 16384), 256, 0, s>>>(ts, d_out);
  return 1;
}
__global__ void __launch_bounds__(256) tile_wide_normalise_kernel(const TileAggSpec ts) {
  for (uint64_t i = blockIdx.x * (uint64_t)blockDim.x + threadIdx.x; i < ts.dense_cap; i += (uint64_t)gridDim.x * blockDim.x) {
    unsigned long long* e = ts.dense_tab + i * ts.G + ts.dec_word;
    unsigned long long w0 = e[0], w1 = e[1], w2 = e[2];
    w1 += w0 >> 32; w0 &= 0xFFFFFFFFULL; w2 += w1 >> 32; w1 &= 0xFFFFFFFFULL;
    e[0] = w0; e[1] = w1; e[2] = w2;
  }
}
int launch_tile_wide_normalise(const TileAggSpec& ts, cudaStream_t s) {
  if (ts.dec_word == 0xFF) return 0;
  tile_wide_normalise_kernel<<<tile_grid(tile_wide_normalise_kernel, ((int64_t)ts.dense_cap + 16383) / 16384), 256, 0, s>>>(ts);
  return 1;
}
__global__ void __launch_bounds__(256) tile_wide_emit_kernel(const TileAggSpec ts, const AggLayout lay, const EmitTable emit, unsigned long long* out_count) {
  const unsigned lane = threadIdx.x & 31;
  const uint64_t stride = (uint64_t)gridDim.x * blockDim.x;
  const uint64_t rounds = (ts.dense_cap + stride - 1) / stride;
  for (uint64_t it = 0; it < rounds; it++) {
    const uint64_t i = it * stride + blockIdx.x * (uint64_t)blockDim.x + threadIdx.x;
    const unsigned long long* e = ts.dense_tab + i * ts.G;
    const bool occ = i < ts.dense_cap && tw_present(ts, e);
    const unsigned m = __ballot_sync(0xffffffffu, occ);
    if (!m) continue;
    unsigned long long base = 0;
    if (lane == 0) base = atomicAdd(out_count, (unsigned long long)__popc(m));
    base = __shfl_sync(0xffffffffu, base, 0);
    if (!occ) continue;
    const unsigned long long at = base + __popc(m & lanemask_lt());
    unsigned long long ke[4] = {0, 0, 0, 0}, slot[16];
    ke[lay.key_word[0]] = (unsigned long long)(ts.nkeys == 1 ? ts.dense_base + (long long)i : ts.dense_base + (long long)(i / ts.dense_r1));
    if (ts.nkeys == 2) ke[lay.key_word[1]] = (unsigned long long)(ts.dense_base1 + (long long)(i % ts.dense_r1));
#pragma unroll
    for (int w = 0; w < 16; w++) slot[w] = 0;
    unsigned flags = 0;
    for (int a = 0; a < ts.nacc; a++) {
      const AccOp op = lay.acc[ts.acc[a].lay_acc];
      const unsigned long long d = e[ts.acc[a].w0];
      switch (ts.acc[a].recon) {
        case TR_COPY: slot[op.word] = d; break;
        case TR_NOT: slot[op.word] = ~d; break;
        case TR_F2I: slot[op.word] = (unsigned long long)__double2ll_rn(as_f64(d)); break;
        default: {
          const unsigned long long w0 = d, w1 = e[ts.acc[a].w0 + 1], w2 = e[ts.acc[a].w0 + 2];
          const unsigned long long c1 = w1 + (w0 >> 32);
          slot[op.word] = (w0 & 0xFFFFFFFFULL) | (c1 << 32); slot[op.word + 1] = w2 + (c1 >> 32);
          break;
        }
      }
      const uint8_t vw = ts.acc[a].valid_word;
      const bool valid = vw == 0xFF ? true : tw_marked(ts, e[vw]);
      if (op.vbit != 0xFF && valid) flags |= 1u << op.vbit;
    }
    emit_row_columns(emit, at, ke, slot, flags);
  }
}
int launch_tile_wide_emit(const TileAggSpec& ts, const AggLayout& lay, const EmitTable& emit, unsigned long long* d_out_count, cudaStream_t s) {
  tile_wide_emit_kernel<<<tile_grid(tile_wide_emit_kernel, ((int64_t)ts.dense_cap + 16383) / 16384), 256, 0, s>>>(ts, lay, emit, d_out_count);
  return 1;
}

}
```

blaze_b200/csrc/stages.cu:

```cuda
#include <algorithm>
#include <chrono>
#include <cstdlib>
#include <cstring>
#include <mutex>
#include <unordered_map>

#include "runtime.h"
#include "kernels_fast.cuh"

namespace b200q {

static std::mutex g_stream_mu;
static std::unordered_map<cudaStream_t, std::weak_ptr<StreamRef>> g_streams;

StreamRef::~StreamRef() {
  { std::lock_guard<std::mutex> l(g_stream_mu); g_streams.erase(s); }
  if (s) { cudaSetDevice(device); cudaStreamSynchronize(s); cudaStreamDestroy(s); }
}
std::shared_ptr<StreamRef> stream_ref_create(int device) {
  auto r = std::make_shared<StreamRef>(); r->device = device;
  B200Q_CUDA(cudaStreamCreateWithFlags(&r->s, cudaStreamNonBlocking));
  std::lock_guard<std::mutex> l(g_stream_mu); g_streams[r->s] = r;
  return r;
}
std::shared_ptr<StreamRef> stream_ref_lookup(cudaStream_t s) {
  std::lock_guard<std::mutex> l(g_stream_mu);
  auto it = g_streams.find(s);
  return it == g_streams.end() ? nullptr : it->second.lock();
}

DevMem::~DevMem() {
  if (owned && ptr) {
    if (stream_keep) { cudaSetDevice(stream_keep->device); cudaFreeAsync(ptr, stream_keep->s); }
    else cudaFree(ptr);
  }
}
DevMemP DevMem::alloc(size_t bytes, cudaStream_t s, bool zero) {
  auto m = std::make_shared<DevMem>();
  m->bytes = bytes; m->stream = s; m->owned = true; m->stream_keep = stream_ref_lookup(s);
  if (bytes == 0) bytes = 16;
  {
    const cudaError_t e = cudaMallocAsync(&m->ptr, bytes, s);
    if (e == cudaErrorMemoryAllocation) {
      cudaGetLastError(); m->ptr = nullptr; m->owned = false;
      throw ExecError(B200Q_ERR_UNSUPPORTED, "out of HBM: a device allocation of " + std::to_string(bytes) + " bytes failed; this task must fall back to the host path");
    }
    B200Q_CUDA(e);
  }
  if (zero) B200Q_CUDA(cudaMemsetAsync(m->ptr, 0, bytes, s));
  return m;
}
DevMemP DevMem::borrow(const void* p, size_t bytes, std::shared_ptr<void> owner) {
  auto m = std::make_shared<DevMem>();
  m->ptr = const_cast<void*>(p); m->bytes = bytes; m->owned = false; m->owner = std::move(owner);
  return m;
}

static inline size_t bitmap_bytes(int64_t n) { return (size_t)((n + 31) / 32) * 4; }

DevCol dev_col_of(const DevColumn& c) {
  DevCol d{};
  const int w = c.type.byte_width();
  d.values = c.values ? (const uint8_t*)c.values->ptr + (size_t)c.offset * (size_t)w : nullptr;
  if (c.type.is_varlen()) d.offsets = c.offsets ? (const int32_t*)c.offsets->ptr + c.offset : nullptr;
  d.validity = c.validity ? (const uint8_t*)c.validity->ptr : nullptr;
  d.bit_offset = (uint32_t)c.offset;
  if (c.offset > 0xFFFFFFFFLL) throw ExecError(B200Q_ERR_UNSUPPORTED, "column offset beyond 2^32 rows");
  return d;
}

static DevMemP upload_program(const CompiledProgram& cp, cudaStream_t s) {
  DevMemP d = DevMem::alloc(sizeof(VmProgram), s);
  const VmProgram p = relocated_program(cp, d->ptr);
  B200Q_CUDA(cudaMemcpyAsync(d->ptr, &p, sizeof(VmProgram), cudaMemcpyHostToDevice, s));
  B200Q_CUDA(cudaStreamSynchronize(s));
  return d;
}

static void check_device_error_flags(int flags) {
  if (flags & 1) throw ExecError(B200Q_ERR_EXECUTION, "Arrow error: Divide by zero error");
  if (flags & 2) throw ExecError(B200Q_ERR_EXECUTION, "Arrow error: Arithmetic overflow");
  if (flags & 4) throw ExecError(B200Q_ERR_EXECUTION, "corrupted accumulator row in the Binary agg buffer column");
}

class FilterProjectStage : public Stage {
  CompiledProgram cp_;
  DevMemP d_prog_;
  bool has_filters_;
  bool identity_ = false;
  bool lean_possible_ = false;
  LeanFpSpec lean_{};
  std::vector<int> out_src_, vm_out_;
  bool varlen_ = false;
  int sel_out_ = -1;

  int slot_of(int col_index) const { for (size_t i = 0; i < cp_.used_cols.size(); i++) if (cp_.used_cols[i] == col_index) return (int)i; return -1; }
  static bool is_i64(const DType& t) { return t.id == T_INT64 || t.id == T_TIMESTAMP_US; }

  void detect_lean(const std::vector<ExprP>& filters, const std::vector<ExprP>& outs) {
    lean_possible_ = false;
    if (filters.size() > 4 || outs.size() > 8 || outs.empty() || cp_.used_cols.empty() || cp_.used_cols.size() > 4) return;
    LeanFpSpec sp{}; sp.nfilt = (int)filters.size(); sp.nout = (int)outs.size();
    for (size_t f = 0; f < filters.size(); f++) {
      const ExprP& p = filters[f];
      if (p->kind != E_BINARY || p->op < OP_EQ || p->op > OP_GE) return;
      ExprP l = p->children[0], r = p->children[1]; int op = p->op - OP_EQ;
      if (l->kind == E_LITERAL && r->kind == E_COLUMN) { std::swap(l, r); static const int flip[] = {CMP_EQ, CMP_NE, CMP_GT, CMP_GE, CMP_LT, CMP_LE}; op = flip[op]; }
      if (l->kind != E_COLUMN || r->kind != E_LITERAL || r->lit_null || !is_i64(l->type) || !is_i64(r->type)) return;
      const int s = slot_of(l->col_index); if (s < 0 || s > 127) return;
      sp.filt[f].col = (int8_t)s; sp.filt[f].op = (uint8_t)op; sp.filt[f].lit = (long long)r->lit_lo;
    }
    for (size_t o = 0; o < outs.size(); o++) {
      const ExprP& e = outs[o];
      if (!is_i64(e->type)) return;
      if (e->kind == E_COLUMN) { const int s = slot_of(e->col_index); if (s < 0 || s > 127) return; sp.out[o].kind = 0; sp.out[o].a = (int8_t)s; sp.out[o].b = -1; continue; }
      if (e->kind != E_BINARY || (e->op != OP_PLUS && e->op != OP_MINUS && e->op != OP_MUL)) return;
      const ExprP &l = e->children[0], &r = e->children[1];
      if (l->kind != E_COLUMN || !is_i64(l->type)) return;
      const int sa = slot_of(l->col_index); if (sa < 0 || sa > 127) return;
      sp.out[o].kind = (uint8_t)(e->op == OP_PLUS ? 1 : e->op == OP_MINUS ? 2 : 3); sp.out[o].a = (int8_t)sa;
      if (r->kind == E_COLUMN && is_i64(r->type)) { const int sb = slot_of(r->col_index); if (sb < 0 || sb > 127) return; sp.out[o].b = (int8_t)sb; }
      else if (r->kind == E_LITERAL && !r->lit_null && is_i64(r->type)) { sp.out[o].b = -1; sp.out[o].lit = (long long)r->lit_lo; }
      else return;
    }
    lean_ = sp; lean_possible_ = true;
  }

 public:
  FilterProjectStage(OpContext& cx, const SchemaDef& in, const std::vector<ExprP>& filters, const std::vector<ExprP>& outs, const SchemaDef& out) {
    in_schema = in; out_schema = out;
    has_filters_ = !filters.empty();
    identity_ = !has_filters_ && outs.size() == in.fields.size();
    for (size_t i = 0; identity_ && i < outs.size(); i++) identity_ = outs[i]->kind == E_COLUMN && outs[i]->col_index == (int)i && outs[i]->type == in.fields[i].type;
    std::vector<ExprP> vm_outs;
    for (const ExprP& o : outs) {
      ExprP e = o;
      while ((e->kind == E_TRY_CAST || e->kind == E_CAST) && e->children[0]->type == e->type) e = e->children[0];
      if (!e->type.is_varlen()) { out_src_.push_back(-1); vm_out_.push_back((int)vm_outs.size()); vm_outs.push_back(o); continue; }
      if (e->kind != E_COLUMN)
        throw PlanError(B200Q_ERR_UNSUPPORTED, "ProjectExec: " + explain_expr(o) + " produces a " + e->type.str() + " value; only " + e->type.str() + " column references are on the hot path");
      out_src_.push_back(e->col_index); vm_out_.push_back(-1);
    }
    varlen_ = vm_outs.size() != outs.size();
    if (varlen_ && has_filters_) sel_out_ = (int)vm_outs.size();
    cp_ = compile_program(filters, vm_outs, has_filters_, sel_out_);
    used_input_cols = cp_.used_cols;
    for (int c : out_src_) if (c >= 0 && std::find(used_input_cols.begin(), used_input_cols.end(), c) == used_input_cols.end()) used_input_cols.push_back(c);
    if (!cx.conf.force_generic_kernels && !varlen_ && !cp_.has_strings) detect_lean(filters, outs);
    d_prog_ = upload_program(cp_, cx.stream);
  }

  void push(OpContext& cx, DevBatch& in, std::vector<DevBatch>& outs) override {
    const int64_t n = in.num_rows;
    if (n == 0) return;
    if (n > 0x7FFFFFFFLL) throw ExecError(B200Q_ERR_UNSUPPORTED, "batches above 2^31-1 rows must be split by the caller");
    if (identity_) {
      bool plain = true;
      auto ours = [](const DevMemP& m) { return !m || m->owned || m->owner; };
      for (auto& c : in.cols) plain = plain && c.offset == 0 && ours(c.values) && ours(c.validity) && ours(c.offsets);
      if (plain) { outs.push_back(in); return; }
    }
    ColTable ct{};
    for (size_t i = 0; i < cp_.used_cols.size(); i++) ct.col[i] = dev_col_of(in.cols[cp_.used_cols[i]]);
    OutTable ot{};
    DevBatch ob;
    for (size_t i = 0; i < cp_.outs.size(); i++) {
      const OutDesc& od = cp_.outs[i];
      DevColumn c; c.type = od.type;
      const bool is_bool = od.type.id == T_BOOL;
      c.values = is_bool ? DevMem::alloc(bitmap_bytes(n), cx.stream, true) : DevMem::alloc((size_t)n * od.type.byte_width(), cx.stream);
      if (od.nullable) c.validity = DevMem::alloc(bitmap_bytes(n), cx.stream, true);
      ot.values[i] = c.values->ptr; ot.validity[i] = c.validity ? (uint32_t*)c.validity->ptr : nullptr; ot.phys[i] = phys_of(od.type);
      ob.cols.push_back(c);
    }
    DevMemP sel;
    if (sel_out_ >= 0) { sel = DevMem::alloc((size_t)n * 4, cx.stream); ot.values[sel_out_] = sel->ptr; ot.validity[sel_out_] = nullptr; ot.phys[sel_out_] = PH_SEL; }
    bool lean = lean_possible_;
    for (size_t i = 0; lean && i < cp_.used_cols.size(); i++) lean = ct.col[i].validity == nullptr;
    DevMemP scratch = DevMem::alloc(32, cx.stream, true);
    DevMemP status;
    B200Q_CUDA(cudaEventRecord(cx.ev0, cx.stream));
    if (lean) {
      for (auto& c : ob.cols) if (c.validity) B200Q_CUDA(cudaMemsetAsync(c.validity->ptr, 0xFF, c.validity->bytes, cx.stream));
      if (has_filters_) status = DevMem::alloc((size_t)filter_project_lean_scratch_bytes(n), cx.stream, true);
      long long* outp[8]; for (size_t i = 0; i < cp_.outs.size(); i++) outp[i] = (long long*)ot.values[i];
      cx.m.launches += launch_filter_project_lean(ct, (int)cp_.used_cols.size(), lean_, outp, n, status ? status->ptr : nullptr, (unsigned long long*)scratch->ptr, cx.stream);
      cx.m.fast_launches++;
    } else {
      if (has_filters_) status = DevMem::alloc((size_t)filter_project_num_tiles(n) * 8, cx.stream, true);
      cx.m.launches += launch_filter_project((const VmProgram*)d_prog_->ptr, ct, ot, (int)cp_.outs.size(), n, has_filters_,
                                             status ? (unsigned long long*)status->ptr : nullptr, (unsigned long long*)scratch->ptr, cx.stream);
    }
    B200Q_CUDA(cudaEventRecord(cx.ev1, cx.stream));
    B200Q_CUDA(cudaGetLastError());
    unsigned long long h[4];
    B200Q_CUDA(cudaMemcpyAsync(h, scratch->ptr, 32, cudaMemcpyDeviceToHost, cx.stream));
    B200Q_CUDA(cudaStreamSynchronize(cx.stream));
    { float ms = 0; B200Q_CUDA(cudaEventElapsedTime(&ms, cx.ev0, cx.ev1)); cx.m.gpu_ms += ms; if (cx.cur_stage == 0) { cx.m.hot_ms += ms; cx.m.hot_rows += n; cx.m.hot_launches++; } }
    check_device_error_flags((int)h[2]);
    ob.num_rows = (int64_t)h[1];
    if (ob.num_rows == 0) return;
    if (!varlen_) { outs.push_back(std::move(ob)); return; }
    DevBatch res; res.num_rows = ob.num_rows;
    for (size_t i = 0; i < out_src_.size(); i++) res.cols.push_back(out_src_[i] < 0 ? ob.cols[(size_t)vm_out_[i]] : DevColumn());
    gather_varlen(cx, in, sel ? (const uint32_t*)sel->ptr : nullptr, res);
    outs.push_back(std::move(res));
  }

  void gather_varlen(OpContext& cx, const DevBatch& in, const uint32_t* sel, DevBatch& res) {
    const int64_t m = res.num_rows;
    auto ours = [](const DevMemP& p) { return !p || p->owned || p->owner; };
    struct Job { size_t out; DevCol src; };
    std::vector<Job> jobs;
    for (size_t i = 0; i < out_src_.size(); i++) {
      if (out_src_[i] < 0) continue;
      const DevColumn& c = in.cols[(size_t)out_src_[i]];
      if (!sel && c.offset == 0 && ours(c.values) && ours(c.offsets) && ours(c.validity)) { res.cols[i] = c; continue; }
      jobs.push_back(Job{i, dev_col_of(c)});
    }
    if (jobs.empty()) return;
    const size_t nj = jobs.size();
    DevMemP totals = DevMem::alloc(nj * 8, cx.stream, true);
    std::vector<DevMemP> keep;
    for (size_t j = 0; j < nj; j++) {
      DevColumn& o = res.cols[jobs[j].out];
      const DevColumn& c = in.cols[(size_t)out_src_[jobs[j].out]];
      o.type = c.type;
      o.offsets = DevMem::alloc((size_t)(m + 1) * 4, cx.stream);
      if (c.validity && out_schema.fields[jobs[j].out].nullable) o.validity = DevMem::alloc(bitmap_bytes(m), cx.stream);
      DevMemP lengths = DevMem::alloc((size_t)m * 4 + 16, cx.stream), sums = DevMem::alloc((size_t)scan_num_blocks(m) * 4 + 16, cx.stream);
      cx.m.launches += launch_varlen_lengths(jobs[j].src, sel, m, (int32_t*)lengths->ptr, o.validity ? (uint32_t*)o.validity->ptr : nullptr,
                                             (unsigned long long*)totals->ptr + j, cx.stream);
      cx.m.launches += launch_exclusive_scan_i32((const int32_t*)lengths->ptr, (int32_t*)o.offsets->ptr, m, (int32_t*)sums->ptr, cx.stream);
      keep.push_back(lengths); keep.push_back(sums);
    }
    std::vector<unsigned long long> bytes(nj);
    B200Q_CUDA(cudaMemcpyAsync(bytes.data(), totals->ptr, nj * 8, cudaMemcpyDeviceToHost, cx.stream));
    B200Q_CUDA(cudaStreamSynchronize(cx.stream));
    for (size_t j = 0; j < nj; j++) {
      DevColumn& o = res.cols[jobs[j].out];
      if (bytes[j] > 0x7FFFFFFFULL) throw ExecError(B200Q_ERR_UNSUPPORTED, "a " + o.type.str() + " output column of one batch exceeds 2 GiB (32-bit Arrow offsets); push smaller batches");
      o.values = DevMem::alloc((size_t)bytes[j], cx.stream);
      cx.m.launches += launch_varlen_copy(jobs[j].src, sel, m, (const int32_t*)o.offsets->ptr, (uint8_t*)o.values->ptr, cx.stream);
    }
    B200Q_CUDA(cudaGetLastError());
  }
  void finish(OpContext&, std::vector<DevBatch>&) override {}
};

std::unique_ptr<Stage> make_filter_project_stage(OpContext& cx, const SchemaDef& in_schema, const std::vector<ExprP>& filters,
                                                 const std::vector<ExprP>& outs, const SchemaDef& out_schema) {
  return std::unique_ptr<Stage>(new FilterProjectStage(cx, in_schema, filters, outs, out_schema));
}

class ExpandStage : public Stage {
  std::vector<std::unique_ptr<FilterProjectStage>> sets_;
 public:
  ExpandStage(OpContext& cx, const SchemaDef& in, const std::vector<ExprP>& filters, const std::vector<std::vector<ExprP>>& projections, const SchemaDef& out) {
    in_schema = in; out_schema = out;
    for (auto& p : projections) {
      sets_.emplace_back(new FilterProjectStage(cx, in, filters, p, out));
      for (int c : sets_.back()->used_input_cols) if (std::find(used_input_cols.begin(), used_input_cols.end(), c) == used_input_cols.end()) used_input_cols.push_back(c);
    }
    std::sort(used_input_cols.begin(), used_input_cols.end());
  }
  void push(OpContext& cx, DevBatch& in, std::vector<DevBatch>& outs) override { for (auto& s : sets_) s->push(cx, in, outs); }
  void finish(OpContext&, std::vector<DevBatch>&) override {}
};

std::unique_ptr<Stage> make_expand_stage(OpContext& cx, const SchemaDef& in_schema, const std::vector<ExprP>& filters,
                                         const std::vector<std::vector<ExprP>>& projections, const SchemaDef& out_schema) {
  return std::unique_ptr<Stage>(new ExpandStage(cx, in_schema, filters, projections, out_schema));
}

static uint64_t host_mix64(uint64_t x) { x ^= x >> 33; x *= 0xff51afd7ed558ccdULL; x ^= x >> 33; x *= 0xc4ceb9fe1a85ec53ULL; x ^= x >> 33; return x; }

StateCols state_columns_of(const AggDef& a) {
  StateCols s; DType i64; i64.id = T_INT64;
  const uint8_t value_kind = a.data_type.id == T_BOOL ? FZ_BOOL : FZ_PRIM;
  switch (a.fn) {
    case AGG_COUNT: s.fields.push_back(FieldDef{a.field_name, i64, false}); s.frozen = {FZ_COUNT}; break;
    case AGG_AVG:
      s.fields.push_back(FieldDef{a.field_name + "#sum", a.data_type, true});
      s.fields.push_back(FieldDef{a.field_name + "#count", i64, false});
      s.frozen = {FZ_PRIM, FZ_COUNT};
      break;
    case AGG_FIRST: {
      DType i8; i8.id = T_INT8;
      s.fields.push_back(FieldDef{a.field_name, a.data_type, true});
      s.fields.push_back(FieldDef{a.field_name + "#flag", i8, false});
      s.frozen = {value_kind, FZ_BOOL};
      break;
    }
    default: s.fields.push_back(FieldDef{a.field_name, a.data_type, true}); s.frozen = {value_kind}; break;
  }
  return s;
}

static bool cast_may_fail(const DType& f, const DType& t) {
  if (f == t) return false;
  auto ii = [](const DType& d) { return d.is_integer() || d.id == T_DATE32 || d.id == T_TIMESTAMP_US || d.id == T_BOOL; };
  if (ii(f) && ii(t)) return t.int_bits() < f.int_bits();
  if (ii(f) && t.is_float()) return false;
  if (f.is_float() && (t.is_float() || t.is_integer() || t.id == T_BOOL)) return false;
  return true;
}
static bool can_be_null(const ExprP& e) {
  switch (e->kind) {
    case E_COLUMN: return e->nullable;
    case E_LITERAL: return e->lit_null || e->type.id == T_NULL;
    case E_BINARY:
      if (e->op == OP_AND || e->op == OP_OR) return e->nullable;
      return can_be_null(e->children[0]) || can_be_null(e->children[1]);
    case E_IS_NULL: case E_IS_NOT_NULL: return false;
    case E_NOT: case E_NEGATIVE: return can_be_null(e->children[0]);
    case E_CAST: case E_TRY_CAST: return can_be_null(e->children[0]) || cast_may_fail(e->children[0]->type, e->type);
    default: return true;
  }
}

static bool same_expr(const ExprP& a, const ExprP& b) {
  if (a == b) return true;
  if (a->kind != b->kind || a->type != b->type || a->children.size() != b->children.size()) return false;
  if (a->kind == E_COLUMN) return a->col_index == b->col_index;
  if (a->kind == E_LITERAL) return a->lit_null == b->lit_null && a->lit_lo == b->lit_lo && a->lit_hi == b->lit_hi && a->lit_str == b->lit_str;
  if (a->kind == E_STR_MATCH && (a->str_match != b->str_match || a->lit_str != b->lit_str)) return false;
  if (a->kind == E_BINARY && a->op != b->op) return false;
  if (a->kind == E_SCALAR_FN && a->name != b->name) return false;
  if (a->kind == E_IN_LIST && a->negated != b->negated) return false;
  if (a->kind == E_CASE && (a->case_has_base != b->case_has_base || a->case_has_else != b->case_has_else)) return false;
  for (size_t i = 0; i < a->children.size(); i++) if (!same_expr(a->children[i], b->children[i])) return false;
  return true;
}
static ExprP strip_noop_casts(ExprP e) {
  while ((e->kind == E_CAST || e->kind == E_TRY_CAST) && !cast_may_fail(e->children[0]->type, e->type)) {
    const DType &f = e->children[0]->type, &t = e->type;
    const bool same_repr = (f == t) || (f.is_intlike() && t.is_intlike());
    if (!same_repr) break;
    e = e->children[0];
  }
  return e;
}

static bool is_null_literal(ExprP e) {
  while (e->kind == E_CAST || e->kind == E_TRY_CAST) e = e->children[0];
  return e->kind == E_LITERAL && (e->lit_null || e->type.id == T_NULL);
}
static bool const_key(const ExprP& e0, bool& null, uint64_t& lo, uint64_t& hi) {
  if (is_null_literal(e0)) { null = true; lo = hi = 0; return true; }
  const ExprP e = strip_noop_casts(e0);
  if (e->kind != E_LITERAL || !(e->type.is_intlike() || e->type.is_decimal())) return false;
  null = false; lo = e->lit_lo; hi = e->lit_hi;
  return true;
}

class PinnedSlots {
  std::mutex mu_; std::vector<unsigned long long*> free_; 
 public:
  unsigned long long* get() {
    std::lock_guard<std::mutex> l(mu_);
    if (free_.empty()) {
      unsigned long long* page = nullptr;
      B200Q_CUDA(cudaMallocHost((void**)&page, 4096));
      for (int i = 0; i < 4096 / 32; i++) free_.push_back(page + i * 4);
    }
    unsigned long long* p = free_.back(); free_.pop_back(); return p;
  }
  void put(unsigned long long* p) { std::lock_guard<std::mutex> l(mu_); free_.push_back(p); }
};
static PinnedSlots& pinned_slots() { static PinnedSlots* p = new PinnedSlots(); return *p; }

class AggStage : public Stage {
  PlanNode node_;
  std::vector<ExprP> filters_;
  std::vector<ExprP> vm_outs_;
  CompiledProgram cp_;
  DevMemP d_prog_;
  AggLayout lay_{};
  bool merge_mode_ = false, columnar_ = false, final_ = false;
  int n_in_ = 0;
  std::vector<FieldDef> merge_state_fields_;
  std::vector<uint8_t> merge_state_kinds_;
  uint64_t rows_pushed_ = 0;
  int first_state_col_ = 0;
  int nsets_ = 1;
  std::vector<AggSetDesc> sets_;
  DevMemP d_sets_;

  DevMemP keys_, accs_, counters_, deferred_[2];
  uint64_t capacity_ = 0;
  int64_t deferred_cap_ = 0;
  int64_t ngroups_ = 0;

  bool fast_ok_ = false, dense_possible_ = false, dense_decided_ = false;
  bool acc_arg_nullable_[2] = {true, true};
  FastSpec fs_{};
  DenseEmitMap dmap_{};
  DevMemP dense_tab_, sink_;
  bool wide_possible_ = false;
  TileAggSpec ws_{};
  int64_t wide_rows_since_norm_ = 0;

  struct EmitSpec { EmitCol ec; FieldDef field; bool frozen_count = false, frozen_bool = false; };
  std::vector<EmitSpec> emit_;
  std::vector<FrozenField> frozen_fields_;

  int add_out(const ExprP& e) {
    ExprP s = strip_noop_casts(e);
    for (size_t i = 0; i < vm_outs_.size(); i++) if (same_expr(vm_outs_[i], s)) return (int)i;
    if (nsets_ > 1 && (int)vm_outs_.size() >= VM_MAX_OUT)
      throw PlanError(B200Q_ERR_UNSUPPORTED, "ExpandExec below AggExec: the grouping sets need more than " + std::to_string(VM_MAX_OUT) + " distinct key and argument expressions (VM_MAX_OUT)");
    vm_outs_.push_back(s);
    return (int)vm_outs_.size() - 1;
  }

  static uint8_t frozen_width(const DType& t) { return (uint8_t)t.byte_width(); }

 public:
  AggStage(OpContext& cx, const SchemaDef& in, const std::vector<ExprP>& filters, const PlanNode& agg,
           const std::vector<ExprP>& group_exprs, const std::vector<std::vector<ExprP>>& agg_args, const std::vector<AggSetExprs>& sets) : node_(agg), filters_(filters) {
    in_schema = in; out_schema = agg.schema;
    n_in_ = (int)in.fields.size();
    merge_mode_ = agg.need_partial_merge; final_ = agg.need_final_merge;
    columnar_ = cx.conf.partial_state_columnar != 0;
    if (agg.exec_mode != 0 && !agg.group_exprs.empty()) {
    }
    if ((int)group_exprs.size() > AGG_MAX_KEYS) throw PlanError(B200Q_ERR_UNSUPPORTED, "more than 8 grouping columns");
    if (merge_mode_ && !filters.empty()) throw PlanError(B200Q_ERR_UNSUPPORTED, "Filter fused below a merge-mode aggregate");
    const bool multi = sets.size() > 1;
    if (multi) {
      if ((int)sets.size() > AGG_MAX_SETS)
        throw PlanError(B200Q_ERR_UNSUPPORTED, "ExpandExec below AggExec: " + std::to_string(sets.size()) + " projections exceed the limit of " + std::to_string(AGG_MAX_SETS) + " grouping sets (AGG_MAX_SETS)");
      if (merge_mode_) throw PlanError(B200Q_ERR_UNSUPPORTED, "ExpandExec fused below a merge-mode aggregate");
      nsets_ = (int)sets.size();
      sets_.resize(nsets_);
      for (auto& d : sets_) { memset(&d, 0, sizeof(d)); memset(d.acc_arg, AGG_NO_ARG, sizeof(d.acc_arg)); }
    }

    for (auto& a : agg.aggs)
      if (a.mode != MODE_PARTIAL) {
        const StateCols sc = state_columns_of(a);
        for (size_t k = 0; k < sc.fields.size(); k++) { merge_state_fields_.push_back(sc.fields[k]); merge_state_kinds_.push_back(sc.frozen[k]); }
      }
    if (merge_mode_) {
      if (columnar_) {
        first_state_col_ = n_in_ - (int)merge_state_fields_.size();
        if (first_state_col_ < (int)0) throw PlanError(B200Q_ERR_INVALID_PLAN, "columnar partial state: input has too few columns");
        for (size_t k = 0; k < merge_state_fields_.size(); k++)
          if (in.fields[first_state_col_ + k].type != merge_state_fields_[k].type)
            throw PlanError(B200Q_ERR_INVALID_PLAN, "columnar partial state: column " + in.fields[first_state_col_ + k].name + " has type " +
                                                        in.fields[first_state_col_ + k].type.str() + ", expected " + merge_state_fields_[k].type.str());
      } else {
        first_state_col_ = n_in_;
        if (in.fields.empty() || in.fields.back().type.id != T_BINARY)
          throw PlanError(B200Q_ERR_INVALID_PLAN, "merge-mode aggregate: the last input column must be the Binary agg buffer column (agg_ctx.rs:280)");
      }
    }

    lay_.nkeys = (int)group_exprs.size();
    int word = 1;
    for (int k = 0; k < lay_.nkeys; k++) {
      const ExprP& g = group_exprs[k];
      if (!multi) {
        lay_.key_out[k] = (uint8_t)add_out(g);
        if (lay_.key_out[k] != k) throw PlanError(B200Q_ERR_UNSUPPORTED, "duplicate grouping expressions");
      } else lay_.key_out[k] = AGG_KEY_CONST;
      lay_.key_word[k] = (uint8_t)word; lay_.key_nwords[k] = g->type.is_decimal() ? 2 : 1;
      word += lay_.key_nwords[k];
    }
    for (int s = 0; multi && s < nsets_; s++)
      for (int k = 0; k < lay_.nkeys; k++) {
        AggSetDesc& d = sets_[s];
        bool null = false; uint64_t lo = 0, hi = 0;
        if (const_key(sets[s].group_exprs[k], null, lo, hi)) {
          d.key_out[k] = AGG_KEY_CONST;
          if (null) d.key_null |= 1u << k;
          else { d.key_const[lay_.key_word[k] - 1] = lo; if (lay_.key_nwords[k] == 2) d.key_const[lay_.key_word[k]] = hi; }
        } else d.key_out[k] = (uint8_t)add_out(sets[s].group_exprs[k]);
      }
    lay_.nkw = word - 1;
    const int key_entry_words = word;
    word = 0;
    for (int i = 0; i < AGG_MAX_SLOT_WORDS; i++) lay_.init[i] = 0;
    lay_.init_flags = 0;
    int vbits = 0, state_k = 0;
    auto new_vbit = [&]() { if (vbits >= 15) throw PlanError(B200Q_ERR_UNSUPPORTED, "too many nullable accumulators in one aggregate"); return (uint8_t)vbits++; };
    auto state_col_expr = [&](const FieldDef& f) {
      auto e = std::make_shared<Expr>(); e->kind = E_COLUMN; e->col_index = first_state_col_ + state_k++; e->name = f.name; e->type = f.type; e->nullable = f.nullable;
      return ExprP(e);
    };
    auto add_acc = [&](AccKind kind, int nwords, uint8_t vbit, const std::vector<int>& args, uint64_t init_lo, uint64_t init_hi) {
      if (lay_.nacc >= AGG_MAX_ACC) throw PlanError(B200Q_ERR_UNSUPPORTED, "too many accumulators in one aggregate");
      if (word + nwords > AGG_MAX_SLOT_WORDS) throw PlanError(B200Q_ERR_UNSUPPORTED, "aggregate state too wide for one table slot");
      AccOp& a = lay_.acc[lay_.nacc++];
      a.kind = kind; a.word = (uint8_t)word; a.vbit = vbit; a.nargs = (uint8_t)args.size();
      for (size_t i = 0; i < args.size() && i < 4; i++) a.arg_out[i] = (uint8_t)args[i];
      lay_.init[word] = init_lo; if (nwords == 2) lay_.init[word + 1] = init_hi;
      const int w = word; word += nwords; return w;
    };
    int first_oword[2] = {-1, -1}, first_flag_out = -1;
    auto new_oword = [&]() {
      if (word + 1 > AGG_MAX_SLOT_WORDS) throw PlanError(B200Q_ERR_UNSUPPORTED, "aggregate state too wide for one table slot");
      lay_.init[word] = ~0ULL; return word++;
    };

    for (int k = 0; k < lay_.nkeys; k++) {
      EmitSpec es{}; es.ec.kind = EMIT_KEY; es.ec.phys = phys_of(group_exprs[k]->type); es.ec.word = lay_.key_word[k]; es.ec.key = (uint8_t)k; es.ec.vbit = 0xFF;
      es.field = agg.schema.fields[k];
      emit_.push_back(es);
    }

    for (size_t ai = 0; ai < agg.aggs.size(); ai++) {
      const AggDef& a = agg.aggs[ai];
      const bool partial = a.mode == MODE_PARTIAL;
      const DType& dt = a.data_type;
      if ((a.fn == AGG_MIN || a.fn == AGG_MAX) && dt.id == T_BOOL) throw PlanError(B200Q_ERR_UNSUPPORTED, "min/max over boolean is not on the hot path");
      int sum_word = -1, cnt_word = -1; uint8_t sum_vbit = 0xFF;
      if (a.fn == AGG_FIRST || a.fn == AGG_FIRST_IGNORES_NULL) {
        const bool ign = a.fn == AGG_FIRST_IGNORES_NULL;
        const StateCols sc = state_columns_of(a);
        std::vector<int> args;
        bool value_nullable = true;
        std::vector<int> set_o(nsets_, -1);
        if (partial && !multi) { args.push_back(add_out(agg_args[ai][0])); value_nullable = can_be_null(agg_args[ai][0]); }
        else if (partial) {
          value_nullable = false;
          for (int s = 0; s < nsets_; s++) {
            const ExprP& e = sets[s].agg_args[ai][0];
            if (is_null_literal(e)) { value_nullable = true; continue; }
            set_o[s] = add_out(e); value_nullable = value_nullable || can_be_null(e);
          }
          int o = 0; for (int s = nsets_ - 1; s >= 0; s--) if (set_o[s] >= 0) o = set_o[s];
          args.push_back(o);
        } else {
          args.push_back(add_out(state_col_expr(sc.fields[0])));
          if (!ign) {
            const ExprP flag = state_col_expr(sc.fields[1]);
            if (first_flag_out < 0) first_flag_out = add_out(flag);
            args.push_back(first_flag_out);
          }
        }
        const uint8_t vbit = (!ign && value_nullable) ? new_vbit() : (uint8_t)0xFF;
        const int nwords = dt.is_decimal() ? 2 : 1;
        const int vw = add_acc(ign ? ACC_FIRST_VALID : ACC_FIRST, nwords, vbit, args, 0, 0);
        AccOp& op = lay_.acc[lay_.nacc - 1];
        op.nwords = (uint8_t)nwords;
        int ow;
        if (!ign) { if (first_oword[partial] < 0) first_oword[partial] = new_oword(); ow = first_oword[partial]; }
        else ow = new_oword();
        op.oword = (uint8_t)ow;
        for (int s = 0; multi && s < nsets_; s++) {
          if (set_o[s] >= 0) sets_[s].acc_arg[lay_.nacc - 1][0] = (uint8_t)set_o[s];
          else if (ign) sets_[s].acc_skip |= 1u << (lay_.nacc - 1);
        }
        auto first_spec = [&](const FieldDef& f, EmitKind kind) {
          EmitSpec es{}; es.ec.kind = kind; es.ec.phys = phys_of(f.type); es.ec.word = (uint8_t)vw; es.ec.word2 = (uint8_t)ow; es.ec.vbit = vbit; es.field = f; return es;
        };
        if (final_) emit_.push_back(first_spec(agg.schema.fields[lay_.nkeys + ai], EMIT_FIRST_VALUE));
        else {
          emit_.push_back(first_spec(sc.fields[0], EMIT_FIRST_VALUE)); emit_.back().frozen_bool = sc.frozen[0] == FZ_BOOL;
          if (!ign) { emit_.push_back(first_spec(sc.fields[1], EMIT_FIRST_FLAG)); emit_.back().frozen_bool = true; }
        }
        continue;
      }
      if (a.fn != AGG_COUNT) {
        ExprP arg;
        if (partial) { arg = agg_args[ai][0]; }
        else { arg = state_col_expr(state_columns_of(a).fields[0]); }
        std::vector<int> set_o(nsets_, -1);
        bool set_nullable = false;
        for (int s = 0; multi && s < nsets_; s++) {
          const ExprP& e = sets[s].agg_args[ai][0];
          if (is_null_literal(e)) { set_nullable = true; continue; }
          set_o[s] = add_out(e); set_nullable = set_nullable || can_be_null(e);
        }
        int o = 0;
        if (!multi) o = add_out(arg);
        else for (int s = nsets_ - 1; s >= 0; s--) if (set_o[s] >= 0) o = set_o[s];
        const bool nullable_arg = (multi ? set_nullable : can_be_null(arg)) || lay_.nkeys == 0;
        const uint8_t vbit = nullable_arg ? new_vbit() : (uint8_t)0xFF;
        AccKind kind; int nwords = 1; uint64_t ilo = 0, ihi = 0;
        if (a.fn == AGG_SUM || a.fn == AGG_AVG) {
          if (dt.is_decimal()) { kind = ACC_ADD_DEC; nwords = 2; }
          else if (dt.id == T_FLOAT64) { kind = ACC_ADD_F64; ilo = 0x8000000000000000ULL; }
          else if (dt.is_integer()) kind = ACC_ADD_I64;
          else throw PlanError(B200Q_ERR_UNSUPPORTED, "sum/avg accumulating at " + dt.str() + " is not on the hot path");
        } else {
          const bool mn = a.fn == AGG_MIN;
          if (dt.is_decimal()) { kind = mn ? ACC_MIN_DEC : ACC_MAX_DEC; nwords = 2; ilo = mn ? ~0ULL : 0ULL; ihi = mn ? 0x7FFFFFFFFFFFFFFFULL : 0x8000000000000000ULL; }
          else if (dt.is_float()) { kind = mn ? ACC_MIN_F64 : ACC_MAX_F64; ilo = mn ? 0x7FFFFFFFFFFFFFFFULL : 0x8000000000000000ULL; }
          else if (dt.is_intlike()) { kind = mn ? ACC_MIN_I64 : ACC_MAX_I64; ilo = mn ? 0x7FFFFFFFFFFFFFFFULL : 0x8000000000000000ULL; }
          else throw PlanError(B200Q_ERR_UNSUPPORTED, "min/max over " + dt.str() + " is not on the hot path");
        }
        sum_word = add_acc(kind, nwords, vbit, {o}, ilo, ihi); sum_vbit = vbit;
        for (int s = 0; multi && s < nsets_; s++) {
          if (set_o[s] < 0) sets_[s].acc_skip |= 1u << (lay_.nacc - 1);
          else sets_[s].acc_arg[lay_.nacc - 1][0] = (uint8_t)set_o[s];
        }
      }
      if (a.fn == AGG_COUNT || a.fn == AGG_AVG) {
        if (multi) {
          std::vector<std::vector<int>> set_args(nsets_);
          std::vector<bool> skip(nsets_, false);
          for (int s = 0; s < nsets_; s++) {
            const auto& srcs = a.fn == AGG_AVG ? std::vector<ExprP>{sets[s].agg_args[ai][0]} : sets[s].agg_args[ai];
            for (auto& e : srcs) {
              if (is_null_literal(e)) skip[s] = true;
              else if (can_be_null(e)) set_args[s].push_back(add_out(e));
            }
            if (set_args[s].size() > 4) throw PlanError(B200Q_ERR_UNSUPPORTED, "count over more than 4 nullable arguments");
          }
          cnt_word = add_acc(ACC_COUNT, 1, 0xFF, set_args[0], 0, 0);
          for (int s = 0; s < nsets_; s++) {
            if (skip[s]) { sets_[s].acc_skip |= 1u << (lay_.nacc - 1); continue; }
            for (size_t i = 0; i < set_args[s].size(); i++) sets_[s].acc_arg[lay_.nacc - 1][i] = (uint8_t)set_args[s][i];
          }
        } else if (partial) {
          std::vector<int> args;
          const auto& srcs = a.fn == AGG_AVG ? std::vector<ExprP>{agg_args[ai][0]} : agg_args[ai];
          for (auto& e : srcs) if (can_be_null(e)) args.push_back(add_out(e));
          if (args.size() > 4) throw PlanError(B200Q_ERR_UNSUPPORTED, "count over more than 4 nullable arguments");
          cnt_word = add_acc(ACC_COUNT, 1, 0xFF, args, 0, 0);
        } else {
          const auto sc = state_columns_of(a);
          const int o = add_out(state_col_expr(sc.fields.back()));
          cnt_word = add_acc(ACC_ADD_I64, 1, 0xFF, {o}, 0, 0);
        }
      }
      auto value_spec = [&](const FieldDef& f, int w, uint8_t vbit, bool order_key) {
        EmitSpec es{}; es.ec.kind = EMIT_ACC_VALUE; es.ec.phys = phys_of(f.type); es.ec.word = (uint8_t)w; es.ec.vbit = vbit; es.ec.is_order_key = order_key; es.field = f; return es;
      };
      const bool order_key = (a.fn == AGG_MIN || a.fn == AGG_MAX) && dt.is_float();
      if (final_) {
        const FieldDef& of = agg.schema.fields[lay_.nkeys + ai];
        if (a.fn == AGG_COUNT) emit_.push_back(value_spec(of, cnt_word, 0xFF, false));
        else if (a.fn == AGG_AVG) {
          EmitSpec es{}; es.field = of; es.ec.word = (uint8_t)sum_word; es.ec.word2 = (uint8_t)cnt_word; es.ec.vbit = sum_vbit;
          if (dt.is_decimal()) { es.ec.kind = EMIT_AVG_DEC; es.ec.phys = PH_DEC128; }
          else { es.ec.kind = EMIT_AVG_F64; es.ec.phys = PH_F64; es.ec.sum_is_f64 = dt.id == T_FLOAT64; }
          emit_.push_back(es);
        } else emit_.push_back(value_spec(of, sum_word, sum_vbit, order_key));
      } else {
        const auto sc = state_columns_of(a);
        if (a.fn == AGG_COUNT) { emit_.push_back(value_spec(sc.fields[0], cnt_word, 0xFF, false)); emit_.back().frozen_count = true; }
        else {
          emit_.push_back(value_spec(sc.fields[0], sum_word, sum_vbit, order_key));
          if (a.fn == AGG_AVG) { emit_.push_back(value_spec(sc.fields[1], cnt_word, 0xFF, false)); emit_.back().frozen_count = true; }
        }
      }
    }
    if (lay_.nkeys == 0 && lay_.nacc == 0) throw PlanError(B200Q_ERR_UNSUPPORTED, "aggregate without groupings and aggregates");
    auto stride_of = [](int words) { return words <= 1 ? 1 : words <= 2 ? 2 : words <= 4 ? 4 : (words + 3) & ~3; };
    lay_.kstride = std::max(2, stride_of(key_entry_words));
    lay_.astride = stride_of(std::max(word, 1));
    if (lay_.kstride > AGG_MAX_SLOT_WORDS || lay_.astride > AGG_MAX_SLOT_WORDS) throw PlanError(B200Q_ERR_UNSUPPORTED, "aggregate state too wide for one table slot");

    if (!final_ && columnar_) {
      out_schema.fields.resize(lay_.nkeys);
      for (size_t i = lay_.nkeys; i < emit_.size(); i++) out_schema.fields.push_back(emit_[i].field);
    }

    cp_ = compile_program(filters_, vm_outs_, false);
    lay_.nouts = (int)cp_.outs.size();
    int ow = 0;
    for (size_t i = 0; i < cp_.outs.size(); i++) { lay_.out_word[i] = (uint8_t)ow; ow += cp_.outs[i].slots; }
    if (ow > AGG_MAX_ROW_WORDS) {
      if (multi) throw PlanError(B200Q_ERR_UNSUPPORTED, "ExpandExec below AggExec: the grouping sets need " + std::to_string(ow) + " key/argument words per row, more than " + std::to_string(AGG_MAX_ROW_WORDS) + " (AGG_MAX_ROW_WORDS)");
      throw PlanError(B200Q_ERR_UNSUPPORTED, "too many key/argument words per row");
    }
    for (int c : cp_.used_cols) if (c < n_in_) used_input_cols.push_back(c);
    if (merge_mode_ && !columnar_) used_input_cols.push_back(n_in_ - 1);
    std::sort(used_input_cols.begin(), used_input_cols.end());
    used_input_cols.erase(std::unique(used_input_cols.begin(), used_input_cols.end()), used_input_cols.end());
    d_prog_ = upload_program(cp_, cx.stream);
    if (multi) {
      d_sets_ = DevMem::alloc(sizeof(AggSetDesc) * sets_.size(), cx.stream);
      B200Q_CUDA(cudaMemcpyAsync(d_sets_->ptr, sets_.data(), sizeof(AggSetDesc) * sets_.size(), cudaMemcpyHostToDevice, cx.stream));
    }

    if (!cp_.has_strings && !multi) {
      detect_fast(cx);
      if (!fast_ok_) detect_wide(cx);
    }

    if (!final_) {
      for (size_t i = lay_.nkeys; i < emit_.size(); i++) {
        FrozenField f{}; const FieldDef& fd = emit_[i].field;
        f.kind = emit_[i].frozen_count ? FZ_COUNT : emit_[i].frozen_bool ? FZ_BOOL : FZ_PRIM; f.width = frozen_width(fd.type); f.phys = phys_of(fd.type);
        frozen_fields_.push_back(f);
      }
    }

    capacity_ = std::max<uint64_t>(1ULL << 20, (uint64_t)((double)std::max<int64_t>(cx.conf.agg_initial_groups, 1) * AGG_SLOTS_PER_GROUP));
    if (capacity_ >= (1ULL << 32)) throw PlanError(B200Q_ERR_UNSUPPORTED, "agg_initial_groups too large");
    alloc_table(cx, capacity_, keys_, accs_, counters_);
    if (lay_.nkeys == 0) seed_global_group(cx);
    B200Q_CUDA(cudaStreamSynchronize(cx.stream));
    cx.m.table_capacity = (int64_t)capacity_;
  }


  int prog_col_slot(int col_index) const {
    for (size_t i = 0; i < cp_.used_cols.size(); i++) if (cp_.used_cols[i] == col_index) return (int)i;
    return -1;
  }
  static bool int_phys(const DType& t) { return t.is_intlike(); }
  bool has_first() const { for (int j = 0; j < lay_.nacc; j++) if (acc_is_first(lay_.acc[j].kind)) return true; return false; }

  bool parse_keys_and_conjuncts(FastSpec& fs) const {
    if (lay_.nkeys < 1 || lay_.nkeys > 2 || filters_.size() > 4) return false;
    fs.nkeys = lay_.nkeys; fs.nfilt = (int)filters_.size();
    for (int k = 0; k < lay_.nkeys; k++) {
      const ExprP& e = vm_outs_[lay_.key_out[k]];
      if (e->kind != E_COLUMN || !int_phys(e->type) || lay_.key_nwords[k] != 1) return false;
      const int s = prog_col_slot(e->col_index); if (s < 0 || s > 127) return false;
      fs.key_col[k] = (int8_t)s; fs.key_phys[k] = phys_of(e->type);
    }
    for (size_t f = 0; f < filters_.size(); f++) {
      const ExprP& p = filters_[f];
      if (p->kind != E_BINARY || p->op < OP_EQ || p->op > OP_GE) return false;
      ExprP l = strip_noop_casts(p->children[0]), r = strip_noop_casts(p->children[1]);
      int op = p->op - OP_EQ;
      if (l->kind == E_LITERAL && r->kind == E_COLUMN) { std::swap(l, r); static const int flip[] = {CMP_EQ, CMP_NE, CMP_GT, CMP_GE, CMP_LT, CMP_LE}; op = flip[op]; }
      if (l->kind != E_COLUMN || r->kind != E_LITERAL || r->lit_null || !int_phys(l->type) || !int_phys(r->type)) return false;
      const int s = prog_col_slot(l->col_index); if (s < 0 || s > 127) return false;
      fs.filt[f].col = (int8_t)s; fs.filt[f].phys = phys_of(l->type); fs.filt[f].op = (uint8_t)op; fs.filt[f].lit = (long long)r->lit_lo;
    }
    merge_conjuncts(fs);
    return true;
  }

  void detect_fast(OpContext& cx) {
    fast_ok_ = false;
    if (cx.conf.force_generic_kernels || has_first()) return;
    if (lay_.nacc < 1 || lay_.nacc > 2) return;
    FastSpec fs{};
    if (!parse_keys_and_conjuncts(fs)) return;
    fs.nacc = lay_.nacc;
    for (int j = 0; j < lay_.nacc; j++) {
      const AccOp& a = lay_.acc[j];
      fs.acc[j].vbit = a.vbit; fs.acc[j].word = a.word; fs.acc[j].col = -1; fs.acc[j].phys = PH_I64;
      if (a.kind == ACC_ADD_I64) {
        const ExprP& e = vm_outs_[a.arg_out[0]];
        if (e->kind != E_COLUMN || !int_phys(e->type)) return;
        const int s = prog_col_slot(e->col_index); if (s < 0 || s > 127) return;
        fs.acc[j].kind = FAST_ACC_ADD; fs.acc[j].col = (int8_t)s; fs.acc[j].phys = phys_of(e->type);
        acc_arg_nullable_[j] = e->nullable;
      } else if (a.kind == ACC_COUNT && a.nargs <= 1) {
        fs.acc[j].kind = FAST_ACC_COUNT;
        if (a.nargs == 1) {
          const ExprP& e = vm_outs_[a.arg_out[0]];
          if (e->kind != E_COLUMN || !(e->type.is_intlike() || e->type.is_float() || e->type.is_decimal())) return;
          const int s = prog_col_slot(e->col_index); if (s < 0 || s > 127) return;
          fs.acc[j].col = (int8_t)s; fs.acc[j].phys = phys_of(e->type);
        }
      } else return;
    }
    if (lay_.nacc == 2 && lay_.acc[0].word / 4 != lay_.acc[1].word / 4) return;
    sink_ = DevMem::alloc((size_t)FAST_SINK_WARPS * 32, cx.stream, true);
    fs.sink = (unsigned long long*)sink_->ptr;
    fs_ = fs; fast_ok_ = true;
    dense_possible_ = cx.conf.agg_dense_keys != 0;
    if (dense_possible_) {
      for (size_t c = 0; c < emit_.size(); c++) {
        const EmitCol& ec = emit_[c].ec;
        if (ec.kind == EMIT_KEY) continue;
        bool found = false; for (int i = 0; i < lay_.nacc; i++) found |= fs_.acc[i].word == ec.word;
        if (ec.kind != EMIT_ACC_VALUE || ec.is_order_key || !found) { dense_possible_ = false; break; }
      }
    }
    if (dense_possible_) dense_possible_ = dense_layout();
  }

  static void merge_conjuncts(FastSpec& fs) {
    fs.nfcol = 0; fs.filt_never = 0;
    long long lo[2] = {INT64_MIN, INT64_MIN}, hi[2] = {INT64_MAX, INT64_MAX}; bool never = false;
    for (int f = 0; f < fs.nfilt; f++) {
      int c = -1;
      for (int i = 0; i < fs.nfcol; i++) if (fs.frange[i].col == fs.filt[f].col) c = i;
      if (c < 0) { if (fs.nfcol == 2) { fs.nfcol = -1; return; } c = fs.nfcol++; fs.frange[c].col = fs.filt[f].col; fs.frange[c].phys = fs.filt[f].phys; }
      const long long lit = fs.filt[f].lit;
      switch (fs.filt[f].op) {
        case CMP_EQ: lo[c] = std::max(lo[c], lit); hi[c] = std::min(hi[c], lit); break;
        case CMP_LT: if (lit == INT64_MIN) never = true; else hi[c] = std::min(hi[c], lit - 1); break;
        case CMP_LE: hi[c] = std::min(hi[c], lit); break;
        case CMP_GT: if (lit == INT64_MAX) never = true; else lo[c] = std::max(lo[c], lit + 1); break;
        case CMP_GE: lo[c] = std::max(lo[c], lit); break;
        default: fs.nfcol = -1; return;
      }
    }
    for (int c = 0; c < fs.nfcol; c++) {
      if (lo[c] > hi[c]) never = true;
      fs.frange[c].lo = lo[c]; fs.frange[c].span = (unsigned long long)hi[c] - (unsigned long long)lo[c];
    }
    fs.filt_never = never ? 1 : 0;
  }

  void detect_wide(OpContext& cx) {
    wide_possible_ = false;
    if (cx.conf.force_generic_kernels || !cx.conf.agg_dense_keys || has_first()) return;
    if (lay_.nacc < 1 || lay_.nacc > 4) return;
    TileAggSpec ts{};
    {
      FastSpec fs{};
      if (!parse_keys_and_conjuncts(fs) || fs.nfcol < 0) return;
      ts.nkeys = fs.nkeys; ts.nfcol = fs.nfcol; ts.filt_never = fs.filt_never;
      for (int k = 0; k < 2; k++) { ts.key_col[k] = fs.key_col[k]; ts.key_phys[k] = fs.key_phys[k]; ts.frange[k] = fs.frange[k]; }
    }
    ts.nacc = lay_.nacc; ts.dec_word = 0xFF;
    bool any_f64 = false, any_min = false, any_int = false;
    for (int j = 0; j < lay_.nacc; j++) {
      switch (lay_.acc[j].kind) {
        case ACC_ADD_F64: any_f64 = true; break;
        case ACC_MIN_I64: case ACC_MAX_I64: case ACC_MIN_F64: case ACC_MAX_F64: any_min = true; break;
        case ACC_ADD_I64: case ACC_ADD_DEC: any_int = true; break;
        case ACC_COUNT: break;
        default: return;
      }
    }
    if ((int)any_f64 + (int)any_min + (int)any_int > 1) return;
    ts.flavour = any_f64 ? TF_ADD_F64 : any_min ? TF_MIN_S64 : TF_ADD_U64;
    const unsigned long long ONE = ts.flavour == TF_ADD_F64 ? 0x3FF0000000000000ULL : ts.flavour == TF_MIN_S64 ? 0ULL : 1ULL;
    const unsigned long long NOOP = tile_identity(ts.flavour);
    struct ArgInfo { int col_index; int cvt; bool nullable; bool values; };
    std::vector<ArgInfo> args; std::vector<ExprP> arg_cols;
    unsigned long long dec_mul = 1; bool dec_mul_seen = false;
    auto arg_of = [&](const ExprP& e0, int want_cvt, bool values, bool dec) -> int {
      ExprP e = strip_noop_casts(e0); int cvt = TC_NONE;
      const bool nullable = can_be_null(e0);
      if ((e->kind == E_CAST || e->kind == E_TRY_CAST)) {
        const ExprP& c = e->children[0];
        if (c->kind == E_COLUMN && c->type.is_intlike() && e->type.id == T_FLOAT64) { cvt = TC_I2F; e = c; }
        else if (c->kind == E_COLUMN && c->type.is_decimal() && e->type.is_decimal() && e->type.scale >= c->type.scale && e->type.scale - c->type.scale <= 18 &&
                 (int)e->type.precision - (int)c->type.precision >= (int)e->type.scale - (int)c->type.scale) {
          unsigned long long mul = 1; for (int i = c->type.scale; i < e->type.scale; i++) mul *= 10ULL;
          if (dec_mul_seen && dec_mul != mul) return -1;
          dec_mul = mul; dec_mul_seen = true; e = c;
        }
        else return -1;
      }
      if (e->kind != E_COLUMN) return -1;
      if (!values) { for (size_t i = 0; i < args.size(); i++) if (args[i].col_index == e->col_index) { args[i].nullable = args[i].nullable || nullable; return (int)i; } }
      if (values) {
        if (dec) { if (!e->type.is_decimal()) return -1; }
        else if (want_cvt == TC_ORDER) { if (e->type.id != T_FLOAT64 || cvt != TC_NONE) return -1; cvt = TC_ORDER; }
        else if (ts.flavour == TF_ADD_F64) { if (!(e->type.id == T_FLOAT64 && cvt == TC_NONE) && cvt != TC_I2F) return -1; }
        else if (!e->type.is_intlike() || cvt != TC_NONE) return -1;
      }
      for (size_t i = 0; i < args.size(); i++)
        if (args[i].col_index == e->col_index && (!values || !args[i].values || args[i].cvt == cvt)) { args[i].nullable = args[i].nullable || nullable; if (values && !args[i].values) { args[i].values = true; args[i].cvt = cvt; } return (int)i; }
      if (args.size() == 2) return -1;
      args.push_back(ArgInfo{e->col_index, cvt, nullable, values}); arg_cols.push_back(e);
      return (int)args.size() - 1;
    };
    int acc_arg[4] = {-1, -1, -1, -1};
    for (int j = 0; j < lay_.nacc; j++) {
      const AccOp& a = lay_.acc[j];
      if (a.kind == ACC_COUNT) { if (a.nargs > 1) return; if (a.nargs == 1) { acc_arg[j] = arg_of(vm_outs_[a.arg_out[0]], TC_NONE, false, false); if (acc_arg[j] < 0) return; } continue; }
      const bool dec = a.kind == ACC_ADD_DEC, order = a.kind == ACC_MIN_F64 || a.kind == ACC_MAX_F64;
      acc_arg[j] = arg_of(vm_outs_[a.arg_out[0]], order ? TC_ORDER : TC_NONE, true, dec);
      if (acc_arg[j] < 0) return;
      if (dec) { if ((ts.arg_is_dec && acc_arg[j] != 0) || acc_arg[j] != 0) return; ts.arg_is_dec = 1; }
    }
    if (ts.arg_is_dec && args.size() > 1) return;
    ts.nargs = (int)args.size(); ts.dec_mul = dec_mul;
    for (size_t i = 0; i < args.size(); i++) {
      const int s = prog_col_slot(args[i].col_index); if (s < 0 || s > 127) return;
      const DType& t = arg_cols[i]->type;
      if (args[i].values && !ts.arg_is_dec && !(t.is_intlike() || t.id == T_FLOAT64)) return;
      ts.arg_col[i] = (int8_t)s; ts.arg_phys[i] = t.id == T_FLOAT64 ? (uint8_t)PH_I64 : phys_of(t); ts.arg_cvt[i] = (uint8_t)args[i].cvt; ts.arg_values[i] = args[i].values ? 1 : 0;
    }
    int w = 0;
    auto constant_word = [&](unsigned long long cst, int gate) { TileWord tw{}; tw.srcsel = 2; tw.gate = (uint8_t)gate; tw.cst = cst; return tw; };
    ts.presence_word = 0; ts.word[w++] = constant_word(ONE, 30);
    int valid_word[2] = {-1, -1};
    for (size_t i = 0; i < args.size(); i++) if (args[i].nullable) { valid_word[i] = w; ts.word[w++] = constant_word(ONE, 28 + (int)i); }
    for (int j = 0; j < lay_.nacc; j++) {
      const AccOp& a = lay_.acc[j]; const int arg = acc_arg[j];
      auto& out = ts.acc[j]; out.arg = (int8_t)arg; out.lay_acc = (uint8_t)j; out.valid_word = 0xFF; out.recon = TR_COPY;
      if (a.kind == ACC_COUNT) {
        if (ts.flavour == TF_MIN_S64) return;
        out.w0 = (uint8_t)(arg >= 0 && valid_word[arg] >= 0 ? valid_word[arg] : 0);
        out.recon = ts.flavour == TF_ADD_F64 ? TR_F2I : TR_COPY;
        continue;
      }
      if (a.vbit != 0xFF) { if (valid_word[arg] < 0) return; out.valid_word = (uint8_t)valid_word[arg]; }
      if (w + (a.kind == ACC_ADD_DEC ? 3 : 1) > 8) return;
      out.w0 = (uint8_t)w;
      TileWord tw{}; tw.srcsel = (uint8_t)arg; tw.gate = (uint8_t)(28 + arg); tw.msk = ~0ULL;
      if (a.kind == ACC_ADD_DEC) {
        ts.dec_word = (uint8_t)w; out.recon = TR_DEC3;
        TileWord lo = tw; lo.srcsel = 0; lo.msk = 0xFFFFFFFFULL; ts.word[w++] = lo;
        TileWord mid = lo; mid.sh = 32; ts.word[w++] = mid;
        TileWord hi = tw; hi.srcsel = 1; ts.word[w++] = hi;
      } else {
        if (a.kind == ACC_MAX_I64 || a.kind == ACC_MAX_F64) { tw.inv = ~0ULL; out.recon = TR_NOT; }
        ts.word[w++] = tw;
      }
    }
    if (w > 8) return;
    ts.G = w <= 2 ? 2 : w <= 4 ? 4 : 8;
    for (; w < ts.G; w++) ts.word[w] = constant_word(NOOP, 30);
    sink_ = DevMem::alloc((size_t)FAST_SINK_WARPS * 32, cx.stream);
    { std::vector<unsigned long long> fill((size_t)FAST_SINK_WARPS * 4, NOOP); B200Q_CUDA(cudaMemcpyAsync(sink_->ptr, fill.data(), fill.size() * 8, cudaMemcpyHostToDevice, cx.stream)); B200Q_CUDA(cudaStreamSynchronize(cx.stream)); }
    ts.sink = (unsigned long long*)sink_->ptr;
    ws_ = ts; wide_possible_ = true;
  }

  struct DenseRange { long long base[2] = {0, 0}; uint64_t span[2] = {1, 1}; uint64_t entries = 1; bool hot = false; };
  bool dense_range(OpContext& cx, const ColTable& ct, int64_t n, int nkeys, const int8_t* key_col, const uint8_t* key_phys, int entry_words,
                   bool probe_skew, DenseRange& dr) {
    const int64_t sample = std::min<int64_t>(n, 1 << 22);
    DevMemP d = DevMem::alloc(64, cx.stream);
    { const long long init[8] = {INT64_MAX, INT64_MIN, 0, INT64_MAX, INT64_MIN, 0, 0, 0};
      B200Q_CUDA(cudaMemcpyAsync(d->ptr, init, 64, cudaMemcpyHostToDevice, cx.stream)); }
    for (int k = 0; k < nkeys; k++) cx.m.launches += launch_key_range(ct.col[key_col[k]], key_phys[k], sample, (long long*)d->ptr + 3 * k, cx.stream);
    DevMemP hist;
    if (probe_skew) {
      hist = DevMem::alloc((65536 + 1) * 4, cx.stream, true);
      DevCol kc[2] = {ct.col[key_col[0]], ct.col[key_col[nkeys == 2 ? 1 : 0]]};
      cx.m.launches += launch_key_skew_probe(kc, key_phys, nkeys, sample, (unsigned*)hist->ptr, cx.stream);
    }
    long long hr[6] = {0}; unsigned mx = 0;
    B200Q_CUDA(cudaMemcpyAsync(hr, d->ptr, 48, cudaMemcpyDeviceToHost, cx.stream));
    if (probe_skew) B200Q_CUDA(cudaMemcpyAsync(&mx, (unsigned*)hist->ptr + 65536, 4, cudaMemcpyDeviceToHost, cx.stream));
    B200Q_CUDA(cudaStreamSynchronize(cx.stream));
    long long nonnull = 0;
    for (int k = 0; k < nkeys; k++) {
      const long long* h = hr + 3 * k;
      if (h[2] <= 0 || h[1] < h[0]) return false;
      const unsigned __int128 range = (unsigned __int128)((__int128)h[1] - (__int128)h[0]) + 1;
      if (range > ((uint64_t)1 << 26)) return false;
      const uint64_t r = (uint64_t)range, margin = r / 8 + std::min<uint64_t>(64, r / 2 + 1);
      dr.base[k] = h[0] > INT64_MIN + (long long)margin ? h[0] - (long long)margin : INT64_MIN;
      dr.span[k] = r + 2 * margin;
      nonnull = std::max(nonnull, h[2]);
    }
    const unsigned __int128 entries = (unsigned __int128)dr.span[0] * dr.span[1];
    const uint64_t budget = 8 * (uint64_t)std::max<int64_t>(std::max<int64_t>(nonnull, cx.conf.agg_initial_groups), 1 << 16);
    if (entries > budget || entries > ((uint64_t)1 << 26)) return false;
    if (cx.conf.agg_max_table_bytes > 0 && entries * entry_words * 8 > (unsigned __int128)cx.conf.agg_max_table_bytes) return false;
    dr.entries = (uint64_t)entries;
    dr.hot = probe_skew && dr.entries * entry_words > 4096 && (uint64_t)mx * 256 > (uint64_t)sample;
    return true;
  }

  void decide_wide(OpContext& cx, const ColTable& ct, int64_t n) {
    dense_decided_ = true;
    if (!wide_possible_ || n == 0) { wide_possible_ = false; return; }
    DenseRange dr;
    if (!dense_range(cx, ct, n, ws_.nkeys, ws_.key_col, ws_.key_phys, ws_.G, false, dr)) { wide_possible_ = false; return; }
    ws_.dense_base = dr.base[0]; ws_.dense_cap0 = dr.span[0]; ws_.dense_base1 = dr.base[1]; ws_.dense_r1 = dr.span[1]; ws_.dense_cap = dr.entries;
    dense_tab_ = DevMem::alloc((size_t)ws_.dense_cap * ws_.G * 8, cx.stream);
    ws_.dense_tab = (unsigned long long*)dense_tab_->ptr;
    cx.m.launches += launch_tile_wide_init(ws_, cx.stream);
  }

  bool dense_layout() {
    int star = -1;
    for (int j = 0; j < lay_.nacc; j++) if (fs_.acc[j].kind == FAST_ACC_COUNT && fs_.acc[j].col < 0) star = j;
    int word_of_acc[2] = {0, 0}, valid_word_of_acc[2] = {0xFF, 0xFF}, w = 0;
    for (int i = 0; i < 4; i++) fs_.dense_word_src[i] = -2;
    int8_t src[8]; for (int i = 0; i < 8; i++) src[i] = -2;
    if (star < 0) src[w++] = -1;
    for (int j = 0; j < lay_.nacc; j++) { word_of_acc[j] = w; src[w++] = (int8_t)j; }
    for (int j = 0; j < lay_.nacc; j++) {
      if (fs_.acc[j].kind != FAST_ACC_ADD || fs_.acc[j].vbit == 0xFF) continue;
      for (int i = 0; i < lay_.nacc; i++) if (i != j && fs_.acc[i].kind == FAST_ACC_COUNT && fs_.acc[i].col == fs_.acc[j].col) valid_word_of_acc[j] = word_of_acc[i];
      if (valid_word_of_acc[j] == 0xFF && !acc_arg_nullable_[j]) valid_word_of_acc[j] = star >= 0 ? word_of_acc[star] : 0;
      if (valid_word_of_acc[j] == 0xFF) { valid_word_of_acc[j] = w; src[w++] = (int8_t)(2 + j); }
    }
    if (w > 4) return false;
    fs_.dense_stride = w <= 2 ? 2 : 4;
    for (int i = 0; i < 4; i++) fs_.dense_word_src[i] = src[i];
    fs_.dense_presence_word = (uint8_t)(star >= 0 ? word_of_acc[star] : 0);
    for (size_t c = 0; c < emit_.size(); c++) {
      dmap_.word[c] = 0; dmap_.valid_word[c] = 0xFF;
      const EmitCol& ec = emit_[c].ec;
      if (ec.kind == EMIT_KEY) continue;
      int j = 0; for (int i = 0; i < lay_.nacc; i++) if (fs_.acc[i].word == ec.word) j = i;
      dmap_.word[c] = (uint8_t)word_of_acc[j];
      if (ec.vbit != 0xFF) dmap_.valid_word[c] = (uint8_t)valid_word_of_acc[j];
    }
    return true;
  }

  void decide_dense(OpContext& cx, const ColTable& ct, int64_t n) {
    dense_decided_ = true;
    if (!fast_ok_ || !dense_possible_ || n == 0) return;
    DenseRange dr;
    if (!dense_range(cx, ct, n, fs_.nkeys, fs_.key_col, fs_.key_phys, fs_.dense_stride, cx.conf.agg_hot_key_cache != 0, dr)) return;
    fs_.dense_base = dr.base[0]; fs_.dense_cap0 = dr.span[0];
    fs_.dense_base1 = dr.base[1]; fs_.dense_r1 = dr.span[1];
    fs_.dense_cap = dr.entries;
    fs_.dense_key0_minor = fs_.nkeys == 2 && dr.span[1] < dr.span[0];
    dense_tab_ = DevMem::alloc((size_t)fs_.dense_cap * fs_.dense_stride * 8, cx.stream, true);
    fs_.dense_tab = (unsigned long long*)dense_tab_->ptr;
    fs_.dense = 1;
    fs_.hot_cache = dr.hot ? 1 : 0;
  }

  bool lean_ok(const ColTable& ct, int64_t begin) const {
    if (begin % 4) return false;
    auto ok = [&](int slot, uint8_t phys) {
      const DevCol& c = ct.col[slot];
      return phys == PH_I64 && c.validity == nullptr && ((uintptr_t)c.values & 31) == 0;
    };
    for (int k = 0; k < fs_.nkeys; k++) if (!ok(fs_.key_col[k], fs_.key_phys[k])) return false;
    for (int j = 0; j < fs_.nacc; j++) {
      if (fs_.acc[j].col < 0) continue;
      if (fs_.acc[j].kind == FAST_ACC_ADD) { if (!ok(fs_.acc[j].col, fs_.acc[j].phys)) return false; }
      else if (ct.col[fs_.acc[j].col].validity != nullptr) return false;
    }
    for (int f = 0; f < fs_.nfilt; f++) if (!ok(fs_.filt[f].col, fs_.filt[f].phys)) return false;
    return true;
  }

  int launch_update(OpContext& cx, const ColTable& ct, const AggTable& t, int64_t begin, int64_t m, const uint32_t* list) {
    if (nsets_ > 1) return launch_agg_update_sets((const VmProgram*)d_prog_->ptr, ct, lay_, t, begin, m, list, (const AggSetDesc*)d_sets_->ptr, nsets_, rows_pushed_, cx.stream);
    if (wide_possible_ && ws_.dense_tab && !list) {
      cx.m.fast_launches++;
      if (ws_.dec_word != 0xFF) {
        if (wide_rows_since_norm_ + m > (1LL << 31)) { cx.m.launches += launch_tile_wide_normalise(ws_, cx.stream); wide_rows_since_norm_ = 0; }
        wide_rows_since_norm_ += m;
      }
      return launch_agg_tile_wide(ct, ws_, lay_, t, begin, m, cx.stream);
    }
    if (fast_ok_ && !list) {
      cx.m.fast_launches++;
      FastSpec fs = fs_;
      fs.lean = lean_ok(ct, begin) ? 1 : 0;
      return launch_agg_fast_update(ct, fs, lay_, t, begin, m, cx.stream);
    }
    return launch_agg_update((const VmProgram*)d_prog_->ptr, ct, lay_, t, begin, m, list, rows_pushed_, cx.stream);
  }

  void check_table_budget(OpContext& cx, unsigned __int128 bytes, const char* what) const {
    const int64_t budget = cx.conf.agg_max_table_bytes;
    if (budget > 0 && bytes > (unsigned __int128)budget)
      throw ExecError(B200Q_ERR_UNSUPPORTED, std::string("aggregate ") + what + " of " + std::to_string((unsigned long long)bytes) + " bytes exceeds the HBM budget (agg_max_table_bytes = " +
                                                 std::to_string(budget) + "): the table cannot spill on the GPU, fall back to the host path (agg_table.rs:540-588)");
  }
  void alloc_table(OpContext& cx, uint64_t cap, DevMemP& keys, DevMemP& accs, DevMemP& counters) {
    check_table_budget(cx, (unsigned __int128)cap * (lay_.kstride + lay_.astride) * 8, "hash table");
    keys = DevMem::alloc((size_t)cap * lay_.kstride * 8, cx.stream, true);
    accs = DevMem::alloc((size_t)cap * lay_.astride * 8, cx.stream);
    counters = DevMem::alloc(64, cx.stream, true);
  }

  void seed_global_group(OpContext& cx) {
    const uint64_t h = host_mix64(0x9E3779B97F4A7C15ULL);
    const uint64_t s = ((h >> 32) * (uint64_t)(uint32_t)capacity_) >> 32;
    const uint32_t tag2 = (uint32_t)h | 0x80000000u;
    std::vector<uint64_t> kimg(lay_.kstride, 0), aimg(lay_.astride, 0);
    for (int i = 0; i < lay_.astride; i++) aimg[i] = lay_.init[i];
    kimg[0] = (uint64_t)tag2 | ((uint64_t)lay_.init_flags << 32);
    B200Q_CUDA(cudaMemcpyAsync((uint8_t*)keys_->ptr + s * lay_.kstride * 8, kimg.data(), kimg.size() * 8, cudaMemcpyHostToDevice, cx.stream));
    B200Q_CUDA(cudaMemcpyAsync((uint8_t*)accs_->ptr + s * lay_.astride * 8, aimg.data(), aimg.size() * 8, cudaMemcpyHostToDevice, cx.stream));
    const unsigned long long one = 1;
    B200Q_CUDA(cudaMemcpyAsync(counters_->ptr, &one, 8, cudaMemcpyHostToDevice, cx.stream));
    B200Q_CUDA(cudaStreamSynchronize(cx.stream));
  }

  static constexpr double AGG_SLOTS_PER_GROUP = 3.0, AGG_LOAD_LIMIT = 0.5;
  static uint64_t load_limit(uint64_t cap) {
    const uint64_t lim = (uint64_t)((double)cap * AGG_LOAD_LIMIT);
    return cap > (1ULL << 19) ? std::min<uint64_t>(lim, cap - (1ULL << 19)) : lim;
  }

  AggTable table_view(int deferred_idx) const {
    AggTable t{};
    t.keys = (unsigned long long*)keys_->ptr; t.accs = (unsigned long long*)accs_->ptr; t.capacity = capacity_; t.max_groups = load_limit(capacity_);
    t.counters = (unsigned long long*)counters_->ptr;
    t.deferred = deferred_[deferred_idx] ? (uint32_t*)deferred_[deferred_idx]->ptr : nullptr;
    return t;
  }

  void grow(OpContext& cx, uint64_t min_groups) {
    uint64_t cap = capacity_;
    do cap <<= 1; while (load_limit(cap) < min_groups);
    if (cap >= (1ULL << 32)) throw ExecError(B200Q_ERR_UNSUPPORTED, "aggregate hash table beyond 2^32 slots");
    DevMemP nkeys, naccs, ncounters;
    alloc_table(cx, cap, nkeys, naccs, ncounters);
    AggTable oldt = table_view(0);
    AggTable newt{}; newt.keys = (unsigned long long*)nkeys->ptr; newt.accs = (unsigned long long*)naccs->ptr; newt.capacity = cap; newt.max_groups = load_limit(cap); newt.counters = (unsigned long long*)ncounters->ptr;
    cx.m.launches += launch_agg_rehash(lay_, oldt, newt, cx.stream);
    B200Q_CUDA(cudaGetLastError());
    keys_ = nkeys; accs_ = naccs; counters_ = ncounters; capacity_ = cap;
    cx.m.grow_count++; cx.m.table_capacity = (int64_t)cap;
  }

  void read_counters(OpContext& cx, unsigned long long (&h)[3]) {
    B200Q_CUDA(cudaMemcpyAsync(h, counters_->ptr, 24, cudaMemcpyDeviceToHost, cx.stream));
    B200Q_CUDA(cudaStreamSynchronize(cx.stream));
    check_device_error_flags((int)h[2]);
    ngroups_ = (int64_t)h[0];
    cx.m.num_groups = ngroups_;
  }

  struct Snap { unsigned long long* h = nullptr; cudaEvent_t ready = nullptr, k0 = nullptr, k1 = nullptr; };
  Snap snap_[2];
 public:
  ~AggStage() override { for (auto& s : snap_) { if (s.h) pinned_slots().put(s.h); if (s.ready) cudaEventDestroy(s.ready); if (s.k0) cudaEventDestroy(s.k0); if (s.k1) cudaEventDestroy(s.k1); } }
  void ensure_snaps() {
    if (snap_[0].h) return;
    for (auto& s : snap_) {
      s.h = pinned_slots().get();
      B200Q_CUDA(cudaEventCreateWithFlags(&s.ready, cudaEventDisableTiming)); B200Q_CUDA(cudaEventCreate(&s.k0)); B200Q_CUDA(cudaEventCreate(&s.k1));
    }
  }
  void account(OpContext& cx, const Snap& s, int64_t rows) {
    float ms = 0; B200Q_CUDA(cudaEventElapsedTime(&ms, s.k0, s.k1));
    cx.m.gpu_ms += ms; if (cx.cur_stage == 0) { cx.m.hot_ms += ms; cx.m.hot_rows += rows; cx.m.hot_launches++; }
  }
  void replay(OpContext& cx, const ColTable& ct, int64_t begin, const uint32_t* list, uint64_t ndef, bool grow_first) {
    if (!deferred_[1] || deferred_[1]->bytes < (size_t)deferred_cap_ * 4) deferred_[1] = DevMem::alloc((size_t)deferred_cap_ * 4, cx.stream);
    int wr = list == (const uint32_t*)deferred_[0]->ptr ? 1 : 0;
    while (ndef > 0) {
      if (grow_first) grow(cx, (uint64_t)ngroups_ + ndef);
      grow_first = true;
      B200Q_CUDA(cudaMemsetAsync((uint8_t*)counters_->ptr + 8, 0, 8, cx.stream));
      cx.m.launches += launch_update(cx, ct, table_view(wr), begin, (int64_t)ndef, list);
      B200Q_CUDA(cudaGetLastError());
      unsigned long long h[3];
      read_counters(cx, h);
      ndef = h[1]; list = (const uint32_t*)deferred_[wr]->ptr; wr ^= 1;
    }
  }

  void update_rows(OpContext& cx, const ColTable& ct, int64_t n) {
    int64_t chunk = std::max<int64_t>(1 << 16, std::min<int64_t>(cx.conf.max_launch_rows, 0x7FFFFFFFLL));
    if (nsets_ > 1) chunk = std::max<int64_t>(1 << 16, chunk / nsets_);
    static const bool dbg = getenv("B200Q_AGG_TIMING") != nullptr;
    auto hnow = [] { return std::chrono::duration<double, std::milli>(std::chrono::steady_clock::now().time_since_epoch()).count(); };
    const double tA = hnow();
    ensure_snaps();
    const double tB = hnow();
    const int64_t m_max = std::min(chunk, n);
    if (deferred_cap_ < 2 * m_max * nsets_) {
      deferred_cap_ = 2 * m_max * nsets_;
      deferred_[0] = DevMem::alloc((size_t)deferred_cap_ * 4, cx.stream);
      deferred_[1] = nullptr;
    }
    const double tC = hnow(); double t_launch = 0, t_settle = 0;
    int64_t prev_begin = 0, prev_m = 0; bool have_prev = false;
    int idx = 0;
    auto settle = [&](int pi, int64_t pb, int64_t pm, bool cur_in_flight, int64_t cb, int64_t cm) -> bool {
      Snap& sp = snap_[pi];
      B200Q_CUDA(cudaEventSynchronize(sp.ready));
      account(cx, sp, pm);
      check_device_error_flags((int)sp.h[2]);
      ngroups_ = (int64_t)sp.h[0]; cx.m.num_groups = ngroups_;
      const uint64_t d_prev = sp.h[1];
      if (d_prev == 0) return false;
      uint64_t d_cur = 0; DevMemP list_cur;
      if (cur_in_flight) {
        Snap& sc = snap_[pi ^ 1];
        B200Q_CUDA(cudaEventSynchronize(sc.ready));
        account(cx, sc, cm);
        check_device_error_flags((int)sc.h[2]);
        ngroups_ = (int64_t)sc.h[0]; cx.m.num_groups = ngroups_;
        d_cur = sc.h[1] - d_prev;
        if (d_cur) { list_cur = DevMem::alloc((size_t)d_cur * 4, cx.stream); B200Q_CUDA(cudaMemcpyAsync(list_cur->ptr, (const uint32_t*)deferred_[0]->ptr + d_prev, (size_t)d_cur * 4, cudaMemcpyDeviceToDevice, cx.stream)); }
      }
      replay(cx, ct, pb, (const uint32_t*)deferred_[0]->ptr, d_prev, true);
      if (d_cur) replay(cx, ct, cb, (const uint32_t*)list_cur->ptr, d_cur, false);
      return true;
    };
    for (int64_t begin = 0; begin < n; begin += chunk, idx++) {
      const int64_t m = std::min(chunk, n - begin);
      Snap& s = snap_[idx & 1];
      const double tl = hnow();
      B200Q_CUDA(cudaEventRecord(s.k0, cx.stream));
      cx.m.launches += launch_update(cx, ct, table_view(0), begin, m, nullptr);
      B200Q_CUDA(cudaEventRecord(s.k1, cx.stream));
      B200Q_CUDA(cudaGetLastError());
      B200Q_CUDA(cudaMemcpyAsync(s.h, counters_->ptr, 24, cudaMemcpyDeviceToHost, cx.stream));
      B200Q_CUDA(cudaEventRecord(s.ready, cx.stream));
      const double ts = hnow(); t_launch += ts - tl;
      const bool slow = have_prev && settle((idx & 1) ^ 1, prev_begin, prev_m, true, begin, m);
      t_settle += hnow() - ts;
      if (slow) { have_prev = false; continue; }
      prev_begin = begin; prev_m = m; have_prev = true;
    }
    const double tD = hnow();
    if (have_prev) settle((idx & 1) ^ 1, prev_begin, prev_m, false, 0, 0);
    if (dbg) fprintf(stderr, "update_rows: snaps %.3f ms, deferred buffers %.3f ms, launches %.3f ms, settles %.3f ms, last settle %.3f ms (%d chunks)\n", tB - tA, tC - tB, t_launch, t_settle, hnow() - tD, idx);
  }

  void push(OpContext& cx, DevBatch& in, std::vector<DevBatch>&) override {
    const int64_t n = in.num_rows;
    if (n == 0) return;
    ColTable ct{};
    std::vector<DevColumn> state_cols;
    if (merge_mode_ && !columnar_) unfreeze(cx, in, state_cols);
    for (size_t i = 0; i < cp_.used_cols.size(); i++) {
      const int c = cp_.used_cols[i];
      ct.col[i] = dev_col_of(c < n_in_ ? in.cols[c] : state_cols[c - n_in_]);
    }
    if (!dense_decided_) { if (wide_possible_) decide_wide(cx, ct, n); else decide_dense(cx, ct, n); }
    update_rows(cx, ct, n);
    rows_pushed_ += (uint64_t)n;
  }

  void unfreeze(OpContext& cx, DevBatch& in, std::vector<DevColumn>& state_cols) {
    const int64_t n = in.num_rows;
    const DevColumn& bc = in.cols.back();
    if (!bc.offsets || !bc.values) throw ExecError(B200Q_ERR_INVALID_ARG, "agg buffer column without offsets/data");
    FrozenTable ft{}; ft.nfields = (int)merge_state_fields_.size();
    if (ft.nfields > FROZEN_MAX_FIELDS) throw ExecError(B200Q_ERR_UNSUPPORTED, "too many accumulator fields");
    std::vector<DevMemP> valid_bytes(ft.nfields);
    std::vector<DevMemP> bool_bytes(ft.nfields);
    for (int k = 0; k < ft.nfields; k++) {
      const FieldDef& f = merge_state_fields_[k];
      DevColumn c; c.type = f.type;
      FrozenField& ff = ft.f[k];
      ff.kind = merge_state_kinds_[k]; ff.width = frozen_width(f.type); ff.phys = phys_of(f.type);
      if (f.type.id == T_BOOL) { bool_bytes[k] = DevMem::alloc((size_t)n, cx.stream); ff.values = bool_bytes[k]->ptr; c.values = DevMem::alloc(bitmap_bytes(n), cx.stream); }
      else { c.values = DevMem::alloc((size_t)n * f.type.byte_width(), cx.stream); ff.values = c.values->ptr; }
      if (f.nullable) { valid_bytes[k] = DevMem::alloc((size_t)n, cx.stream); ff.valid = (const uint8_t*)valid_bytes[k]->ptr; c.validity = DevMem::alloc(bitmap_bytes(n), cx.stream); }
      state_cols.push_back(c);
    }
    int* d_err = (int*)((unsigned long long*)counters_->ptr + 2);
    cx.m.launches += launch_frozen_read(ft, n, (const int32_t*)bc.offsets->ptr, bc.offset, (const uint8_t*)bc.values->ptr, d_err, cx.stream);
    for (int k = 0; k < ft.nfields; k++) {
      if (valid_bytes[k]) cx.m.launches += launch_pack_valid((const uint8_t*)valid_bytes[k]->ptr, (uint32_t*)state_cols[k].validity->ptr, n, cx.stream);
      if (bool_bytes[k]) cx.m.launches += launch_pack_valid((const uint8_t*)bool_bytes[k]->ptr, (uint32_t*)state_cols[k].values->ptr, n, cx.stream);
    }
    B200Q_CUDA(cudaGetLastError());
  }

  void finish(OpContext& cx, std::vector<DevBatch>& outs) override {
    const bool wide = wide_possible_ && ws_.dense_tab;
    ensure_snaps();
    unsigned long long* hs = snap_[0].h;
    DevMemP dc;
    if (fs_.dense || wide) {
      dc = DevMem::alloc(8, cx.stream, true);
      if (wide) cx.m.launches += launch_tile_wide_normalise(ws_, cx.stream);
      cx.m.launches += fs_.dense ? launch_dense_count(fs_, (unsigned long long*)dc->ptr, cx.stream) : launch_tile_wide_count(ws_, (unsigned long long*)dc->ptr, cx.stream);
      B200Q_CUDA(cudaMemcpyAsync(hs + 3, dc->ptr, 8, cudaMemcpyDeviceToHost, cx.stream));
    } else hs[3] = 0;
    B200Q_CUDA(cudaMemcpyAsync(hs, counters_->ptr, 24, cudaMemcpyDeviceToHost, cx.stream));
    B200Q_CUDA(cudaStreamSynchronize(cx.stream));
    check_device_error_flags((int)hs[2]);
    ngroups_ = (int64_t)hs[0];
    const int64_t g = ngroups_ + (int64_t)hs[3];
    cx.m.num_groups = g;
    if (g == 0) return;
    EmitTable et{}; et.ncols = (int)emit_.size();
    if (et.ncols > EMIT_MAX_COLS) throw ExecError(B200Q_ERR_UNSUPPORTED, "too many output columns");
    DevBatch ob; ob.num_rows = g;
    std::vector<DevMemP> valid_bytes(emit_.size()), bool_bytes(emit_.size());
    for (size_t i = 0; i < emit_.size(); i++) {
      EmitCol ec = emit_[i].ec; const FieldDef& f = emit_[i].field;
      DevColumn c; c.type = f.type;
      if (f.type.id == T_BOOL) { bool_bytes[i] = DevMem::alloc((size_t)g, cx.stream); ec.values = bool_bytes[i]->ptr; c.values = DevMem::alloc(bitmap_bytes(g), cx.stream); }
      else { c.values = DevMem::alloc((size_t)g * f.type.byte_width(), cx.stream); ec.values = c.values->ptr; }
      if (f.nullable) { valid_bytes[i] = DevMem::alloc((size_t)g, cx.stream); ec.valid_bytes = (uint8_t*)valid_bytes[i]->ptr; c.validity = DevMem::alloc(bitmap_bytes(g), cx.stream); }
      et.col[i] = ec;
      ob.cols.push_back(c);
    }
    DevMemP out_count = DevMem::alloc(8, cx.stream, true);
    cx.m.launches += launch_agg_emit(lay_, table_view(0), et, (unsigned long long*)out_count->ptr, cx.stream);
    if (fs_.dense) cx.m.launches += launch_agg_emit_dense(fs_, et, dmap_, (unsigned long long*)out_count->ptr, cx.stream);
    if (wide) cx.m.launches += launch_tile_wide_emit(ws_, lay_, et, (unsigned long long*)out_count->ptr, cx.stream);
    for (size_t i = 0; i < emit_.size(); i++) {
      if (valid_bytes[i]) cx.m.launches += launch_pack_valid((const uint8_t*)valid_bytes[i]->ptr, (uint32_t*)ob.cols[i].validity->ptr, g, cx.stream);
      if (bool_bytes[i]) cx.m.launches += launch_pack_valid((const uint8_t*)bool_bytes[i]->ptr, (uint32_t*)ob.cols[i].values->ptr, g, cx.stream);
    }
    B200Q_CUDA(cudaGetLastError());
    if (!final_ && !columnar_) {
      FrozenTable ft{}; ft.nfields = (int)frozen_fields_.size();
      for (int k = 0; k < ft.nfields; k++) {
        ft.f[k] = frozen_fields_[k];
        ft.f[k].values = bool_bytes[lay_.nkeys + k] ? bool_bytes[lay_.nkeys + k]->ptr : ob.cols[lay_.nkeys + k].values->ptr;
        ft.f[k].valid = valid_bytes[lay_.nkeys + k] ? (const uint8_t*)valid_bytes[lay_.nkeys + k]->ptr : nullptr;
      }
      DevMemP lengths = DevMem::alloc((size_t)g * 4, cx.stream);
      DevMemP offsets = DevMem::alloc((size_t)(g + 1) * 4, cx.stream);
      DevMemP block_sums = DevMem::alloc((size_t)scan_num_blocks(g) * 4 + 16, cx.stream);
      cx.m.launches += launch_frozen_lengths(ft, g, (int32_t*)lengths->ptr, cx.stream);
      cx.m.launches += launch_exclusive_scan_i32((const int32_t*)lengths->ptr, (int32_t*)offsets->ptr, g, (int32_t*)block_sums->ptr, cx.stream);
      int32_t total = 0;
      B200Q_CUDA(cudaMemcpyAsync(&total, (int32_t*)offsets->ptr + g, 4, cudaMemcpyDeviceToHost, cx.stream));
      B200Q_CUDA(cudaStreamSynchronize(cx.stream));
      if (total < 0) throw ExecError(B200Q_ERR_UNSUPPORTED, "frozen accumulator column exceeds 2 GiB; emit in smaller batches");
      DevMemP data = DevMem::alloc((size_t)total, cx.stream);
      cx.m.launches += launch_frozen_write(ft, g, (const int32_t*)offsets->ptr, (uint8_t*)data->ptr, cx.stream);
      B200Q_CUDA(cudaGetLastError());
      DevColumn bc; bc.type.id = T_BINARY; bc.values = data; bc.offsets = offsets;
      ob.cols.resize(lay_.nkeys);
      ob.cols.push_back(bc);
    }
    B200Q_CUDA(cudaStreamSynchronize(cx.stream));
    outs.push_back(std::move(ob));
  }
};

std::unique_ptr<Stage> make_agg_stage(OpContext& cx, const SchemaDef& in_schema, const std::vector<ExprP>& filters, const PlanNode& agg,
                                      const std::vector<ExprP>& group_exprs, const std::vector<std::vector<ExprP>>& agg_args,
                                      const std::vector<AggSetExprs>& sets) {
  return std::unique_ptr<Stage>(new AggStage(cx, in_schema, filters, agg, group_exprs, agg_args, sets));
}

}
```

Baseline: 81.67 billion.

## Cut host syncs, kernel launches and eager table allocation in aggregation setup

Several overhead cuts at once. The per-key range and skew-histogram kernels merge into one key-stats kernel. The synchronous program upload now uses pinned staging with no stream sync, and the hashed table is allocated lazily only when the dense or wide path is not chosen. The separate dense and wide count kernels are removed: finish sizes outputs from an upper bound and reads the true count after emit. The dense emit now does one atomic per block instead of one per warp. This trades fewer syncs and launches for over-allocated output buffers and extra __syncthreads in emit.

```diff
diff --git a/blaze_b200/csrc/agg_device.cuh b/blaze_b200/csrc/agg_device.cuh
--- a/blaze_b200/csrc/agg_device.cuh
+++ b/blaze_b200/csrc/agg_device.cuh
@@ -46,6 +46,7 @@
 
 __device__ __forceinline__ uint64_t agg_find_or_insert(const AggLayout& lay, const AggTable& tab, const uint64_t* kw, uint32_t knull,
                                                        uint64_t h, unsigned* flags_out, bool* inserted) {
+  if (tab.capacity == 0) return AGG_NO_SLOT;
   const unsigned tag = agg_tag(h);
   uint64_t s = agg_first_slot(h, tab.capacity);
   while (true) {
diff --git a/blaze_b200/csrc/capi.cu b/blaze_b200/csrc/capi.cu
--- a/blaze_b200/csrc/capi.cu
+++ b/blaze_b200/csrc/capi.cu
@@ -631,7 +631,13 @@
           throw PlanError(B200Q_ERR_INVALID_ARG, "input_schema does not match the plan leaf: type of column " + std::to_string(i));
     }
   });
-  if (st != B200Q_OK) { if (op) { op->stages.clear(); delete op; } return st; }
+  if (st != B200Q_OK) {
+    if (op) {
+      if (op->cx.stream) cudaStreamSynchronize(op->cx.stream);
+      op->stages.clear(); delete op;
+    }
+    return st;
+  }
   *out = op;
   return B200Q_OK;
 }
diff --git a/blaze_b200/csrc/kernels_fast.cu b/blaze_b200/csrc/kernels_fast.cu
--- a/blaze_b200/csrc/kernels_fast.cu
+++ b/blaze_b200/csrc/kernels_fast.cu
@@ -367,19 +367,35 @@
   }
 }
 
-__global__ void __launch_bounds__(256) key_skew_hist_kernel(const DevCol c0, const DevCol c1, int phys0, int phys1, int nkeys, long long n, unsigned* hist) {
+__global__ void __launch_bounds__(256) key_stats_kernel(const DevCol c0, const DevCol c1, int phys0, int phys1, int nkeys, long long n, int skew,
+                                                        unsigned long long* out, unsigned* hist) {
+  constexpr unsigned long long SIGN = 0x8000000000000000ULL;
+  unsigned long long mn[2] = {0, 0}, mx[2] = {0, 0}, cnt[2] = {0, 0};
   for (long long i = blockIdx.x * (long long)blockDim.x + threadIdx.x; i < n; i += (long long)gridDim.x * blockDim.x) {
-    if (!col_valid(c0, i) || (nkeys == 2 && !col_valid(c1, i))) continue;
-    const uint64_t h = agg_hash2((uint64_t)col_load_int(c0, phys0, i), nkeys == 2 ? (uint64_t)col_load_int(c1, phys1, i) : 0ULL, 0);
-    atomicAdd(hist + (h >> 48), 1u);
-  }
-}
-__global__ void __launch_bounds__(256) key_skew_max_kernel(unsigned* hist) {
+    const bool v0 = col_valid(c0, i), v1 = nkeys == 2 && col_valid(c1, i);
+    long long a = 0, b = 0;
+    if (v0) { a = col_load_int(c0, phys0, i); const unsigned long long e = (unsigned long long)a ^ SIGN; mn[0] = max(mn[0], ~e); mx[0] = max(mx[0], e); cnt[0]++; }
+    if (v1) { b = col_load_int(c1, phys1, i); const unsigned long long e = (unsigned long long)b ^ SIGN; mn[1] = max(mn[1], ~e); mx[1] = max(mx[1], e); cnt[1]++; }
+    if (skew && v0 && (nkeys == 1 || v1)) atomicAdd(hist + (agg_hash2((uint64_t)a, (uint64_t)b, 0) >> 48), 1u);
+  }
+#pragma unroll
+  for (int d = 16; d > 0; d >>= 1) {
+#pragma unroll
+    for (int k = 0; k < 2; k++) {
+      mn[k] = max(mn[k], __shfl_xor_sync(0xffffffffu, mn[k], d)); mx[k] = max(mx[k], __shfl_xor_sync(0xffffffffu, mx[k], d));
+      cnt[k] += __shfl_xor_sync(0xffffffffu, cnt[k], d);
+    }
+  }
+  if ((threadIdx.x & 31) == 0) {
+    for (int k = 0; k < nkeys; k++) if (cnt[k]) { atomicMax(out + 3 * k, mn[k]); atomicMax(out + 3 * k + 1, mx[k]); atomicAdd(out + 3 * k + 2, cnt[k]); }
+  }
+}
+__global__ void __launch_bounds__(256) key_skew_max_kernel(const unsigned* hist, unsigned long long* out) {
   unsigned mx = 0;
   for (int i = blockIdx.x * blockDim.x + threadIdx.x; i < 65536; i += gridDim.x * blockDim.x) mx = max(mx, hist[i]);
 #pragma unroll
   for (int d = 16; d > 0; d >>= 1) mx = max(mx, __shfl_xor_sync(0xffffffffu, mx, d));
-  if ((threadIdx.x & 31) == 0) atomicMax(hist + 65536, mx);
+  if ((threadIdx.x & 31) == 0 && mx) atomicMax(out, (unsigned long long)mx);
 }
 
 constexpr int LH_BLOCK = 128, LH_U = 4, LH_QCAP = 32 * (LH_U + 1);
@@ -711,28 +727,12 @@
   return 0;
 }
 
-__global__ void __launch_bounds__(256) key_range_kernel(const DevCol col, int phys, long long n, long long* out ) {
-  long long mn = INT64_MAX, mx = INT64_MIN; unsigned long long cnt = 0;
-  for (long long i = blockIdx.x * (long long)blockDim.x + threadIdx.x; i < n; i += (long long)gridDim.x * blockDim.x) {
-    if (!col_valid(col, i)) continue;
-    const long long v = col_load_int(col, phys, i);
-    mn = v < mn ? v : mn; mx = v > mx ? v : mx; cnt++;
-  }
-#pragma unroll
-  for (int d = 16; d > 0; d >>= 1) {
-    const long long a = __shfl_xor_sync(0xffffffffu, mn, d), b = __shfl_xor_sync(0xffffffffu, mx, d);
-    mn = a < mn ? a : mn; mx = b > mx ? b : mx; cnt += __shfl_xor_sync(0xffffffffu, cnt, d);
-  }
-  if ((threadIdx.x & 31) == 0) { atomicMin(out, mn); atomicMax(out + 1, mx); atomicAdd((unsigned long long*)out + 2, cnt); }
-}
-int launch_key_skew_probe(const DevCol* key_cols, const uint8_t* phys, int nkeys, int64_t n, unsigned* d_hist, cudaStream_t s) {
-  key_skew_hist_kernel<<<fast_grid((n + 2047) / 2048), 256, 0, s>>>(key_cols[0], key_cols[nkeys == 2 ? 1 : 0], phys[0], phys[nkeys == 2 ? 1 : 0], nkeys, n, d_hist);
-  key_skew_max_kernel<<<32, 256, 0, s>>>(d_hist);
+int launch_key_stats(const DevCol* key_cols, const uint8_t* phys, int nkeys, int64_t n, bool skew, unsigned long long* d_out, unsigned* d_hist, cudaStream_t s) {
+  const int k1 = nkeys == 2 ? 1 : 0;
+  key_stats_kernel<<<fast_grid((n + 2047) / 2048), 256, 0, s>>>(key_cols[0], key_cols[k1], phys[0], phys[k1], nkeys, n, skew ? 1 : 0, d_out, d_hist);
+  if (!skew) return 1;
+  key_skew_max_kernel<<<32, 256, 0, s>>>(d_hist, d_out + 6);
   return 2;
-}
-int launch_key_range(const DevCol& col, int phys, int64_t n, long long* d_out, cudaStream_t s) {
-  key_range_kernel<<<fast_grid((n + 2047) / 2048), 256, 0, s>>>(col, phys, n, d_out);
-  return 1;
 }
 
 __device__ __forceinline__ void dense_store(const EmitCol& c, unsigned long long at, uint64_t lo, bool valid) {
@@ -746,7 +746,9 @@
   }
 }
 __global__ void __launch_bounds__(256) agg_emit_dense_kernel(const FastSpec fs, const EmitTable emit, const DenseEmitMap map, unsigned long long* out_count) {
-  const unsigned lane = threadIdx.x & 31;
+  __shared__ unsigned s_cnt[8];
+  __shared__ unsigned long long s_base;
+  const unsigned lane = threadIdx.x & 31, warp = threadIdx.x >> 5;
   const uint64_t stride = (uint64_t)gridDim.x * blockDim.x;
   const uint64_t rounds = (fs.dense_cap + stride - 1) / stride;
   for (uint64_t it = 0; it < rounds; it++) {
@@ -755,10 +757,17 @@
     const unsigned long long* e = fs.dense_tab + pe * fs.dense_stride;
     const bool occ = i < fs.dense_cap && e[fs.dense_presence_word] != 0;
     const unsigned m = __ballot_sync(0xffffffffu, occ);
-    if (!m) continue;
-    unsigned long long base = 0;
-    if (lane == 0) base = atomicAdd(out_count, (unsigned long long)__popc(m));
-    base = __shfl_sync(0xffffffffu, base, 0);
+    if (lane == 0) s_cnt[warp] = __popc(m);
+    __syncthreads();
+    if (threadIdx.x == 0) {
+      unsigned t = 0;
+      for (int w = 0; w < 8; w++) t += s_cnt[w];
+      s_base = t ? atomicAdd(out_count, (unsigned long long)t) : 0;
+    }
+    __syncthreads();
+    unsigned long long base = s_base;
+    for (unsigned w = 0; w < warp; w++) base += s_cnt[w];
+    __syncthreads();
     if (!occ) continue;
     const unsigned long long at = base + __popc(m & lanemask_lt());
     for (int c = 0; c < emit.ncols; c++) {
@@ -781,17 +790,4 @@
   return 1;
 }
 
-__global__ void __launch_bounds__(256) dense_count_kernel(const FastSpec fs, unsigned long long* out) {
-  unsigned long long c = 0;
-  for (uint64_t i = blockIdx.x * (uint64_t)blockDim.x + threadIdx.x; i < fs.dense_cap; i += (uint64_t)gridDim.x * blockDim.x)
-    c += fs.dense_tab[i * fs.dense_stride + fs.dense_presence_word] != 0;
-#pragma unroll
-  for (int d = 16; d > 0; d >>= 1) c += __shfl_xor_sync(0xffffffffu, c, d);
-  if ((threadIdx.x & 31) == 0 && c) atomicAdd(out, c);
-}
-int launch_dense_count(const FastSpec& fs, unsigned long long* d_out, cudaStream_t s) {
-  dense_count_kernel<<<fast_grid(((int64_t)fs.dense_cap + 255) / 256), 256, 0, s>>>(fs, d_out);
-  return 1;
-}
-
-}
+}
diff --git a/blaze_b200/csrc/kernels_fast.cuh b/blaze_b200/csrc/kernels_fast.cuh
--- a/blaze_b200/csrc/kernels_fast.cuh
+++ b/blaze_b200/csrc/kernels_fast.cuh
@@ -79,15 +79,12 @@
 
 int launch_agg_tile_wide(const ColTable& cols, const TileAggSpec& ts, const AggLayout& lay, const AggTable& tab, int64_t row_begin, int64_t n, cudaStream_t s);
 int launch_tile_wide_init(const TileAggSpec& ts, cudaStream_t s);
-int launch_tile_wide_count(const TileAggSpec& ts, unsigned long long* d_out, cudaStream_t s);
 int launch_tile_wide_normalise(const TileAggSpec& ts, cudaStream_t s);
 int launch_tile_wide_emit(const TileAggSpec& ts, const AggLayout& lay, const EmitTable& emit, unsigned long long* d_out_count, cudaStream_t s);
 
 int launch_agg_tile_dense(const ColTable& cols, const FastSpec& fs, const AggLayout& lay, const AggTable& tab, int64_t row_begin, int64_t n, cudaStream_t s);
 int launch_agg_fast_update(const ColTable& cols, const FastSpec& fs, const AggLayout& lay, const AggTable& tab, int64_t row_begin, int64_t n, cudaStream_t s);
-int launch_key_skew_probe(const DevCol* key_cols, const uint8_t* phys, int nkeys, int64_t n, unsigned* d_hist , cudaStream_t s);
-int launch_key_range(const DevCol& col, int phys, int64_t n, long long* d_out, cudaStream_t s);
+int launch_key_stats(const DevCol* key_cols, const uint8_t* phys, int nkeys, int64_t n, bool skew, unsigned long long* d_out, unsigned* d_hist, cudaStream_t s);
 int launch_agg_emit_dense(const FastSpec& fs, const EmitTable& emit, const DenseEmitMap& map, unsigned long long* d_out_count, cudaStream_t s);
-int launch_dense_count(const FastSpec& fs, unsigned long long* d_out, cudaStream_t s);
 
 }
diff --git a/blaze_b200/csrc/kernels_tile.cu b/blaze_b200/csrc/kernels_tile.cu
--- a/blaze_b200/csrc/kernels_tile.cu
+++ b/blaze_b200/csrc/kernels_tile.cu
@@ -403,17 +403,6 @@
   return ts.flavour == TF_MIN_S64 ? w == 0 : ts.flavour == TF_ADD_F64 ? as_f64(w) != 0.0 : w != 0;
 }
 __device__ __forceinline__ bool tw_present(const TileAggSpec& ts, const unsigned long long* e) { return tw_marked(ts, e[ts.presence_word]); }
-__global__ void __launch_bounds__(256) tile_wide_count_kernel(const TileAggSpec ts, unsigned long long* out) {
-  unsigned long long c = 0;
-  for (uint64_t i = blockIdx.x * (uint64_t)blockDim.x + threadIdx.x; i < ts.dense_cap; i += (uint64_t)gridDim.x * blockDim.x) c += tw_present(ts, ts.dense_tab + i * ts.G);
-#pragma unroll
-  for (int d = 16; d > 0; d >>= 1) c += __shfl_xor_sync(0xffffffffu, c, d);
-  if ((threadIdx.x & 31) == 0 && c) atomicAdd(out, c);
-}
-int launch_tile_wide_count(const TileAggSpec& ts, unsigned long long* d_out, cudaStream_t s) {
-  tile_wide_count_kernel<<<tile_grid(tile_wide_count_kernel, ((int64_t)ts.dense_cap + 16383) / 16384), 256, 0, s>>>(ts, d_out);
-  return 1;
-}
 __global__ void __launch_bounds__(256) tile_wide_normalise_kernel(const TileAggSpec ts) {
   for (uint64_t i = blockIdx.x * (uint64_t)blockDim.x + threadIdx.x; i < ts.dense_cap; i += (uint64_t)gridDim.x * blockDim.x) {
     unsigned long long* e = ts.dense_tab + i * ts.G + ts.dec_word;
diff --git a/blaze_b200/csrc/stages.cu b/blaze_b200/csrc/stages.cu
--- a/blaze_b200/csrc/stages.cu
+++ b/blaze_b200/csrc/stages.cu
@@ -69,11 +69,37 @@
   return d;
 }
 
-static DevMemP upload_program(const CompiledProgram& cp, cudaStream_t s) {
+class PinnedSlots {
+  std::mutex mu_; std::vector<unsigned long long*> free_;
+  const size_t slot_bytes_, page_bytes_;
+ public:
+  explicit PinnedSlots(size_t slot_bytes) : slot_bytes_(slot_bytes), page_bytes_(std::max<size_t>(4096, 8 * slot_bytes)) {}
+  unsigned long long* get() {
+    std::lock_guard<std::mutex> l(mu_);
+    if (free_.empty()) {
+      unsigned long long* page = nullptr;
+      B200Q_CUDA(cudaMallocHost((void**)&page, page_bytes_));
+      for (size_t i = 0; i < page_bytes_ / slot_bytes_; i++) free_.push_back(page + i * (slot_bytes_ / 8));
+    }
+    unsigned long long* p = free_.back(); free_.pop_back(); return p;
+  }
+  void put(unsigned long long* p) { std::lock_guard<std::mutex> l(mu_); free_.push_back(p); }
+};
+static PinnedSlots& pinned_slots() { static PinnedSlots* p = new PinnedSlots(64); return *p; }
+static PinnedSlots& pinned_programs() { static PinnedSlots* p = new PinnedSlots((sizeof(VmProgram) + 255) & ~(size_t)255); return *p; }
+
+struct PinnedProgram {
+  unsigned long long* h = nullptr;
+  PinnedProgram() = default;
+  PinnedProgram(const PinnedProgram&) = delete;
+  PinnedProgram& operator=(const PinnedProgram&) = delete;
+  ~PinnedProgram() { if (h) pinned_programs().put(h); }
+};
+static DevMemP upload_program(const CompiledProgram& cp, cudaStream_t s, PinnedProgram& host) {
   DevMemP d = DevMem::alloc(sizeof(VmProgram), s);
-  const VmProgram p = relocated_program(cp, d->ptr);
-  B200Q_CUDA(cudaMemcpyAsync(d->ptr, &p, sizeof(VmProgram), cudaMemcpyHostToDevice, s));
-  B200Q_CUDA(cudaStreamSynchronize(s));
+  if (!host.h) host.h = pinned_programs().get();
+  *(VmProgram*)host.h = relocated_program(cp, d->ptr);
+  B200Q_CUDA(cudaMemcpyAsync(d->ptr, host.h, sizeof(VmProgram), cudaMemcpyHostToDevice, s));
   return d;
 }
 
@@ -86,6 +112,7 @@
 class FilterProjectStage : public Stage {
   CompiledProgram cp_;
   DevMemP d_prog_;
+  PinnedProgram prog_host_;
   bool has_filters_;
   bool identity_ = false;
   bool lean_possible_ = false;
@@ -147,7 +174,7 @@
     used_input_cols = cp_.used_cols;
     for (int c : out_src_) if (c >= 0 && std::find(used_input_cols.begin(), used_input_cols.end(), c) == used_input_cols.end()) used_input_cols.push_back(c);
     if (!cx.conf.force_generic_kernels && !varlen_ && !cp_.has_strings) detect_lean(filters, outs);
-    d_prog_ = upload_program(cp_, cx.stream);
+    d_prog_ = upload_program(cp_, cx.stream, prog_host_);
   }
 
   void push(OpContext& cx, DevBatch& in, std::vector<DevBatch>& outs) override {
@@ -354,28 +381,13 @@
   return true;
 }
 
-class PinnedSlots {
-  std::mutex mu_; std::vector<unsigned long long*> free_; 
- public:
-  unsigned long long* get() {
-    std::lock_guard<std::mutex> l(mu_);
-    if (free_.empty()) {
-      unsigned long long* page = nullptr;
-      B200Q_CUDA(cudaMallocHost((void**)&page, 4096));
-      for (int i = 0; i < 4096 / 32; i++) free_.push_back(page + i * 4);
-    }
-    unsigned long long* p = free_.back(); free_.pop_back(); return p;
-  }
-  void put(unsigned long long* p) { std::lock_guard<std::mutex> l(mu_); free_.push_back(p); }
-};
-static PinnedSlots& pinned_slots() { static PinnedSlots* p = new PinnedSlots(); return *p; }
-
 class AggStage : public Stage {
   PlanNode node_;
   std::vector<ExprP> filters_;
   std::vector<ExprP> vm_outs_;
   CompiledProgram cp_;
   DevMemP d_prog_;
+  PinnedProgram prog_host_;
   AggLayout lay_{};
   bool merge_mode_ = false, columnar_ = false, final_ = false;
   int n_in_ = 0;
@@ -388,7 +400,7 @@
   DevMemP d_sets_;
 
   DevMemP keys_, accs_, counters_, deferred_[2];
-  uint64_t capacity_ = 0;
+  uint64_t capacity_ = 0, initial_capacity_ = 0;
   int64_t deferred_cap_ = 0;
   int64_t ngroups_ = 0;
 
@@ -672,7 +684,7 @@
     if (merge_mode_ && !columnar_) used_input_cols.push_back(n_in_ - 1);
     std::sort(used_input_cols.begin(), used_input_cols.end());
     used_input_cols.erase(std::unique(used_input_cols.begin(), used_input_cols.end()), used_input_cols.end());
-    d_prog_ = upload_program(cp_, cx.stream);
+    d_prog_ = upload_program(cp_, cx.stream, prog_host_);
     if (multi) {
       d_sets_ = DevMem::alloc(sizeof(AggSetDesc) * sets_.size(), cx.stream);
       B200Q_CUDA(cudaMemcpyAsync(d_sets_->ptr, sets_.data(), sizeof(AggSetDesc) * sets_.size(), cudaMemcpyHostToDevice, cx.stream));
@@ -691,12 +703,12 @@
       }
     }
 
-    capacity_ = std::max<uint64_t>(1ULL << 20, (uint64_t)((double)std::max<int64_t>(cx.conf.agg_initial_groups, 1) * AGG_SLOTS_PER_GROUP));
-    if (capacity_ >= (1ULL << 32)) throw PlanError(B200Q_ERR_UNSUPPORTED, "agg_initial_groups too large");
-    alloc_table(cx, capacity_, keys_, accs_, counters_);
+    initial_capacity_ = std::max<uint64_t>(1ULL << 20, (uint64_t)((double)std::max<int64_t>(cx.conf.agg_initial_groups, 1) * AGG_SLOTS_PER_GROUP));
+    if (initial_capacity_ >= (1ULL << 32)) throw PlanError(B200Q_ERR_UNSUPPORTED, "agg_initial_groups too large");
+    check_table_budget(cx, (unsigned __int128)initial_capacity_ * (lay_.kstride + lay_.astride) * 8, "hash table");
+    counters_ = DevMem::alloc(64, cx.stream, true);
+    if (!(dense_possible_ || wide_possible_)) alloc_hashed(cx);
     if (lay_.nkeys == 0) seed_global_group(cx);
-    B200Q_CUDA(cudaStreamSynchronize(cx.stream));
-    cx.m.table_capacity = (int64_t)capacity_;
   }
 
 
@@ -911,20 +923,17 @@
   bool dense_range(OpContext& cx, const ColTable& ct, int64_t n, int nkeys, const int8_t* key_col, const uint8_t* key_phys, int entry_words,
                    bool probe_skew, DenseRange& dr) {
     const int64_t sample = std::min<int64_t>(n, 1 << 22);
-    DevMemP d = DevMem::alloc(64, cx.stream);
-    { const long long init[8] = {INT64_MAX, INT64_MIN, 0, INT64_MAX, INT64_MIN, 0, 0, 0};
-      B200Q_CUDA(cudaMemcpyAsync(d->ptr, init, 64, cudaMemcpyHostToDevice, cx.stream)); }
-    for (int k = 0; k < nkeys; k++) cx.m.launches += launch_key_range(ct.col[key_col[k]], key_phys[k], sample, (long long*)d->ptr + 3 * k, cx.stream);
-    DevMemP hist;
-    if (probe_skew) {
-      hist = DevMem::alloc((65536 + 1) * 4, cx.stream, true);
-      DevCol kc[2] = {ct.col[key_col[0]], ct.col[key_col[nkeys == 2 ? 1 : 0]]};
-      cx.m.launches += launch_key_skew_probe(kc, key_phys, nkeys, sample, (unsigned*)hist->ptr, cx.stream);
-    }
-    long long hr[6] = {0}; unsigned mx = 0;
-    B200Q_CUDA(cudaMemcpyAsync(hr, d->ptr, 48, cudaMemcpyDeviceToHost, cx.stream));
-    if (probe_skew) B200Q_CUDA(cudaMemcpyAsync(&mx, (unsigned*)hist->ptr + 65536, 4, cudaMemcpyDeviceToHost, cx.stream));
+    DevMemP d = DevMem::alloc(64 + (probe_skew ? 65536 * 4 : 0), cx.stream, true);
+    const DevCol kc[2] = {ct.col[key_col[0]], ct.col[key_col[nkeys == 2 ? 1 : 0]]};
+    cx.m.launches += launch_key_stats(kc, key_phys, nkeys, sample, probe_skew, (unsigned long long*)d->ptr, (unsigned*)((unsigned long long*)d->ptr + 8), cx.stream);
+    ensure_snaps();
+    unsigned long long* hw = snap_[0].h;
+    B200Q_CUDA(cudaMemcpyAsync(hw, d->ptr, 56, cudaMemcpyDeviceToHost, cx.stream));
     B200Q_CUDA(cudaStreamSynchronize(cx.stream));
+    constexpr unsigned long long SIGN = 0x8000000000000000ULL;
+    long long hr[6];
+    for (int k = 0; k < 2; k++) { hr[3 * k] = (long long)(~hw[3 * k] ^ SIGN); hr[3 * k + 1] = (long long)(hw[3 * k + 1] ^ SIGN); hr[3 * k + 2] = (long long)hw[3 * k + 2]; }
+    const unsigned long long mx = hw[6];
     long long nonnull = 0;
     for (int k = 0; k < nkeys; k++) {
       const long long* h = hr + 3 * k;
@@ -941,7 +950,7 @@
     if (entries > budget || entries > ((uint64_t)1 << 26)) return false;
     if (cx.conf.agg_max_table_bytes > 0 && entries * entry_words * 8 > (unsigned __int128)cx.conf.agg_max_table_bytes) return false;
     dr.entries = (uint64_t)entries;
-    dr.hot = probe_skew && dr.entries * entry_words > 4096 && (uint64_t)mx * 256 > (uint64_t)sample;
+    dr.hot = probe_skew && dr.entries * entry_words > 4096 && mx * 256 > (uint64_t)sample;
     return true;
   }
 
@@ -1041,11 +1050,15 @@
       throw ExecError(B200Q_ERR_UNSUPPORTED, std::string("aggregate ") + what + " of " + std::to_string((unsigned long long)bytes) + " bytes exceeds the HBM budget (agg_max_table_bytes = " +
                                                  std::to_string(budget) + "): the table cannot spill on the GPU, fall back to the host path (agg_table.rs:540-588)");
   }
-  void alloc_table(OpContext& cx, uint64_t cap, DevMemP& keys, DevMemP& accs, DevMemP& counters) {
+  void alloc_slots(OpContext& cx, uint64_t cap, DevMemP& keys, DevMemP& accs) {
     check_table_budget(cx, (unsigned __int128)cap * (lay_.kstride + lay_.astride) * 8, "hash table");
     keys = DevMem::alloc((size_t)cap * lay_.kstride * 8, cx.stream, true);
     accs = DevMem::alloc((size_t)cap * lay_.astride * 8, cx.stream);
-    counters = DevMem::alloc(64, cx.stream, true);
+  }
+  void alloc_hashed(OpContext& cx) {
+    alloc_slots(cx, initial_capacity_, keys_, accs_);
+    capacity_ = initial_capacity_;
+    cx.m.table_capacity = (int64_t)capacity_;
   }
 
   void seed_global_group(OpContext& cx) {
@@ -1070,18 +1083,20 @@
 
   AggTable table_view(int deferred_idx) const {
     AggTable t{};
-    t.keys = (unsigned long long*)keys_->ptr; t.accs = (unsigned long long*)accs_->ptr; t.capacity = capacity_; t.max_groups = load_limit(capacity_);
+    if (capacity_) { t.keys = (unsigned long long*)keys_->ptr; t.accs = (unsigned long long*)accs_->ptr; }
+    t.capacity = capacity_; t.max_groups = load_limit(capacity_);
     t.counters = (unsigned long long*)counters_->ptr;
     t.deferred = deferred_[deferred_idx] ? (uint32_t*)deferred_[deferred_idx]->ptr : nullptr;
     return t;
   }
 
   void grow(OpContext& cx, uint64_t min_groups) {
+    if (capacity_ == 0) { alloc_hashed(cx); return; }
     uint64_t cap = capacity_;
     do cap <<= 1; while (load_limit(cap) < min_groups);
     if (cap >= (1ULL << 32)) throw ExecError(B200Q_ERR_UNSUPPORTED, "aggregate hash table beyond 2^32 slots");
-    DevMemP nkeys, naccs, ncounters;
-    alloc_table(cx, cap, nkeys, naccs, ncounters);
+    DevMemP nkeys, naccs, ncounters = DevMem::alloc(64, cx.stream, true);
+    alloc_slots(cx, cap, nkeys, naccs);
     AggTable oldt = table_view(0);
     AggTable newt{}; newt.keys = (unsigned long long*)nkeys->ptr; newt.accs = (unsigned long long*)naccs->ptr; newt.capacity = cap; newt.max_groups = load_limit(cap); newt.counters = (unsigned long long*)ncounters->ptr;
     cx.m.launches += launch_agg_rehash(lay_, oldt, newt, cx.stream);
@@ -1198,7 +1213,10 @@
       const int c = cp_.used_cols[i];
       ct.col[i] = dev_col_of(c < n_in_ ? in.cols[c] : state_cols[c - n_in_]);
     }
-    if (!dense_decided_) { if (wide_possible_) decide_wide(cx, ct, n); else decide_dense(cx, ct, n); }
+    if (!dense_decided_) {
+      if (wide_possible_) decide_wide(cx, ct, n); else decide_dense(cx, ct, n);
+      if (capacity_ == 0 && !fs_.dense && !wide_possible_) alloc_hashed(cx);
+    }
     update_rows(cx, ct, n);
     rows_pushed_ += (uint64_t)n;
   }
@@ -1232,25 +1250,24 @@
 
   void finish(OpContext& cx, std::vector<DevBatch>& outs) override {
     const bool wide = wide_possible_ && ws_.dense_tab;
+    const bool dense = fs_.dense || wide;
     ensure_snaps();
     unsigned long long* hs = snap_[0].h;
-    DevMemP dc;
-    if (fs_.dense || wide) {
-      dc = DevMem::alloc(8, cx.stream, true);
-      if (wide) cx.m.launches += launch_tile_wide_normalise(ws_, cx.stream);
-      cx.m.launches += fs_.dense ? launch_dense_count(fs_, (unsigned long long*)dc->ptr, cx.stream) : launch_tile_wide_count(ws_, (unsigned long long*)dc->ptr, cx.stream);
-      B200Q_CUDA(cudaMemcpyAsync(hs + 3, dc->ptr, 8, cudaMemcpyDeviceToHost, cx.stream));
-    } else hs[3] = 0;
-    B200Q_CUDA(cudaMemcpyAsync(hs, counters_->ptr, 24, cudaMemcpyDeviceToHost, cx.stream));
-    B200Q_CUDA(cudaStreamSynchronize(cx.stream));
-    check_device_error_flags((int)hs[2]);
-    ngroups_ = (int64_t)hs[0];
-    const int64_t g = ngroups_ + (int64_t)hs[3];
-    cx.m.num_groups = g;
+    int64_t g;
+    if (dense) {
+      g = (int64_t)std::min<uint64_t>(fs_.dense ? fs_.dense_cap : ws_.dense_cap, rows_pushed_) + ngroups_;
+    } else {
+      B200Q_CUDA(cudaMemcpyAsync(hs, counters_->ptr, 24, cudaMemcpyDeviceToHost, cx.stream));
+      B200Q_CUDA(cudaStreamSynchronize(cx.stream));
+      check_device_error_flags((int)hs[2]);
+      ngroups_ = (int64_t)hs[0];
+      g = ngroups_;
+      cx.m.num_groups = g;
+    }
     if (g == 0) return;
     EmitTable et{}; et.ncols = (int)emit_.size();
     if (et.ncols > EMIT_MAX_COLS) throw ExecError(B200Q_ERR_UNSUPPORTED, "too many output columns");
-    DevBatch ob; ob.num_rows = g;
+    DevBatch ob;
     std::vector<DevMemP> valid_bytes(emit_.size()), bool_bytes(emit_.size());
     for (size_t i = 0; i < emit_.size(); i++) {
       EmitCol ec = emit_[i].ec; const FieldDef& f = emit_[i].field;
@@ -1262,9 +1279,22 @@
       ob.cols.push_back(c);
     }
     DevMemP out_count = DevMem::alloc(8, cx.stream, true);
-    cx.m.launches += launch_agg_emit(lay_, table_view(0), et, (unsigned long long*)out_count->ptr, cx.stream);
+    if (capacity_) cx.m.launches += launch_agg_emit(lay_, table_view(0), et, (unsigned long long*)out_count->ptr, cx.stream);
     if (fs_.dense) cx.m.launches += launch_agg_emit_dense(fs_, et, dmap_, (unsigned long long*)out_count->ptr, cx.stream);
-    if (wide) cx.m.launches += launch_tile_wide_emit(ws_, lay_, et, (unsigned long long*)out_count->ptr, cx.stream);
+    if (wide) {
+      cx.m.launches += launch_tile_wide_normalise(ws_, cx.stream);
+      cx.m.launches += launch_tile_wide_emit(ws_, lay_, et, (unsigned long long*)out_count->ptr, cx.stream);
+    }
+    if (dense) {
+      B200Q_CUDA(cudaMemcpyAsync(hs + 3, out_count->ptr, 8, cudaMemcpyDeviceToHost, cx.stream));
+      B200Q_CUDA(cudaMemcpyAsync(hs, counters_->ptr, 24, cudaMemcpyDeviceToHost, cx.stream));
+      B200Q_CUDA(cudaStreamSynchronize(cx.stream));
+      check_device_error_flags((int)hs[2]);
+      g = (int64_t)hs[3];
+      cx.m.num_groups = g;
+      if (g == 0) return;
+    }
+    ob.num_rows = g;
     for (size_t i = 0; i < emit_.size(); i++) {
       if (valid_bytes[i]) cx.m.launches += launch_pack_valid((const uint8_t*)valid_bytes[i]->ptr, (uint32_t*)ob.cols[i].validity->ptr, g, cx.stream);
       if (bool_bytes[i]) cx.m.launches += launch_pack_valid((const uint8_t*)bool_bytes[i]->ptr, (uint32_t*)ob.cols[i].values->ptr, g, cx.stream);
```

Result: no change. 82.17 billion, median of 6 (+0.6%).
